# AUTOMATIC1111/stable-diffusion-webui

Measured on AMD Instinct MI355X. Metric: images/sec SD1.5 512x512 20-step Euler-a, batch 8 per GPU, higher is better.
Workload: dtype f16

## Files before the change

include/sdmi.h:

```cpp
#ifndef SDMI_H
#define SDMI_H

#include <stdint.h>

#ifdef __cplusplus
extern "C" {
#endif

#define SDMI_VERSION 100

enum { SDMI_F16 = 0, SDMI_F32 = 1 };

typedef struct sdmi_engine sdmi_engine;

int sdmi_version(void);
const char* sdmi_last_error(void);
int sdmi_device_ok(void);


int64_t sdmi_attention_workspace_bytes(int B, int H, int M, int D);
int sdmi_attention(const void* q, const void* k, const void* v, void* out,
                   int B, int H, int N, int M, int D,
                   int ldq, int ldk, int ldv, int ldo, float scale,
                   void* workspace, int64_t workspace_bytes, void* stream);

int64_t sdmi_attention_wide_workspace_bytes(int B, int N, int M, int D);
int sdmi_attention_wide(const void* q, const void* k, const void* v, void* out,
                        int B, int N, int M, int D,
                        int ldq, int ldk, int ldv, int ldo, float scale,
                        void* workspace, int64_t workspace_bytes, void* stream);

int sdmi_attention_vt(const void* q, const void* k, const void* vt, void* out,
                      int B, int H, int N, int M, int D,
                      int ldq, int ldk, int vt_ld, int ldo, float scale, int force_generic, void* stream);

typedef struct sdmi_conv_desc {
    const void* a0;
    const void* a1;
    const void* w;
    const void* bias;
    const void* rowbias;
    const void* resid;
    void* out;
    int32_t c0, c1, lda0, lda1;
    int32_t B, Hi, Wi, Ho, Wo;
    int32_t taps;
    int32_t stride;
    int32_t pad;
    int32_t up;
    int32_t N;
    int32_t n_real;
    int32_t ldo, ldr;
    int32_t flags;
    float alpha;
    int32_t batch;
    int64_t a_bs, w_bs, o_bs, r_bs;
    int32_t force_generic;
    int32_t reserved;
    void* splitk_workspace;
    int64_t splitk_workspace_bytes;
} sdmi_conv_desc;

enum {
    SDMI_EP_OUT_F32  = 1,
    SDMI_EP_GEGLU    = 2,
    SDMI_EP_NCHW     = 4,
    SDMI_EP_BIAS_ROW = 8,
    SDMI_EP_WRAP = 128,
    SDMI_EP_TRANSPOSE = 64
};
int sdmi_conv_gemm(const sdmi_conv_desc* d, void* stream);
int64_t sdmi_conv_splitk_workspace_bytes(int M, int N, int K, int batch);

int sdmi_pack_conv_weight(const void* w_oihw, int dtype, void* out_f16, int O, int I, int kh, int kw,
                          int O_pad, int I_pad, int geglu, void* stream);

int sdmi_groupnorm(const void* x0, const void* x1, int c0, int c1, const void* gamma_f32, const void* beta_f32,
                   void* out_f16, int B, int HW, int groups, float eps, int silu,
                   void* workspace_f32, int64_t workspace_bytes, void* stream);
int64_t sdmi_groupnorm_workspace_bytes(int B, int HW, int groups);

int sdmi_layernorm(const void* x, const void* gamma_f32, const void* beta_f32, void* out_f16,
                   int64_t rows, int C, float eps, void* stream);

int64_t sdmi_rowchain_ff_pack_bytes(int C, int hidden);
int sdmi_rowchain_ff_pack(const void* w1_f16, const void* b1_f32_or_null, const void* w2_f16, void* packs, int C, int hidden,
                          void* stream);
int sdmi_rowchain_ff(const void* x_f16, void* out_f16, const void* ln_gamma_f32, const void* ln_beta_f32, const void* packs,
                     const void* b2_f32_or_null, int64_t rows, int C, int hidden, float eps, void* stream);


int sdmi_philox_randn(void* out_f32, int64_t n, uint64_t seed, uint32_t offset, void* stream);

int sdmi_slerp(void* out_f32, const void* low_f32, const void* high_f32, float val, int C, int H, int W, void* scratch_f32,
               void* stream);


int sdmi_cfg_prepare_input(const void* x_f32, const void* c_in_f32, void* x_in, int out_dtype,
                           int B, int reps, int64_t chw, void* stream);

int sdmi_cfg_prepare_concat(const void* x_f32, const void* c_in_f32, const void* c_concat_f32, void* x_in, int out_dtype,
                            int B, int reps, int C, int Cc, int64_t hw, uint32_t zero_reps, void* stream);

int sdmi_cfg_combine(const void* x_f32, const void* eps_f32, const void* c_out_f32, float cond_scale, int mode,
                     const void* mask_f32, const void* nmask_f32, const void* init_latent_f32,
                     void* denoised_f32, int B, int64_t chw, void* stream);

int sdmi_cfg_combine_affine(const void* x_f32, const void* out_f32, const void* c_out_f32, const void* c_skip_f32,
                            float cond_scale, const void* mask_f32, const void* nmask_f32, const void* init_latent_f32,
                            void* denoised_f32, int B, int64_t chw, void* stream);

int sdmi_euler_step(void* x_f32, const void* denoised_f32, const void* noise_f32_or_null,
                    float sigma, float sigma_down, float sigma_up, float s_noise, int64_t n, void* stream);

int sdmi_dpmpp2m_step(void* x_f32, const void* denoised_f32, const void* old_denoised_f32_or_null,
                      float ratio, float em1, float c1, float c2, int64_t n, void* stream);

int sdmi_ddim_step(void* x_f32, const void* e_t_f32, const void* noise_f32_or_null, void* pred_x0_f32_or_null,
                   float a_t, float a_prev, float sigma_t, float sqrt_one_minus_at, int64_t n, void* stream);

int sdmi_axpby(void* y_f32, const void* x_f32, float a, const void* z_f32_or_null, float b, int64_t n, void* stream);

int sdmi_lincomb(void* out_f32, const void* const* terms_f32, const float* coefs, int n_terms, int64_t n, void* stream);

int sdmi_dpm_error_partials(const void* x_low_f32, const void* x_high_f32, const void* x_prev_f32, float atol, float rtol,
                            void* partial256_f32, int64_t n, void* stream);

int sdmi_latent_resize(const void* in_f32, void* out_f32, int planes, int hi, int wi, int ho, int wo, int mode, void* stream);

int sdmi_mask_blend(void* x_f32, const void* init_f32, const void* mask_f32, const void* nmask_f32, int64_t n, void* stream);

int sdmi_image_to_u8(const void* img_f32_nchw, void* out_u8_nhwc, int B, int C, int H, int W, void* stream);

typedef struct sdmi_unet_config {
    int32_t in_channels, out_channels, model_channels;
    int32_t num_levels;
    int32_t channel_mult[8];
    int32_t num_res_blocks;
    int32_t attn_level[8];
    int32_t transformer_depth[8];
    int32_t num_heads;
    int32_t num_head_channels;
    int32_t context_dim;
    int32_t adm_in_channels;
    int32_t reserved[4];
} sdmi_unet_config;

typedef struct sdmi_vae_config {
    int32_t ch, num_levels;
    int32_t ch_mult[8];
    int32_t num_res_blocks, in_channels, out_ch, z_channels;
    float scale_factor;
    int32_t reserved[4];
} sdmi_vae_config;

sdmi_engine* sdmi_engine_create(int device);
void sdmi_engine_destroy(sdmi_engine* e);

int sdmi_unet_configure(sdmi_engine* e, const sdmi_unet_config* cfg);
int sdmi_unet_load_tensor(sdmi_engine* e, const char* key, const void* data, int dtype, int ndim,
                          const int64_t* shape, int on_device);
int sdmi_unet_finalize(sdmi_engine* e);

int sdmi_unet_update_weight(sdmi_engine* e, const char* key, const void* data, int dtype, int ndim,
// ... 77 lines not shown
```

stable-diffusion-webui_amd/_lib.py:

```python
from __future__ import annotations

import ctypes as C
import os
import re

_HERE = os.path.dirname(os.path.abspath(__file__))
LIB_PATH = os.environ.get("SDMI_LIB") or os.path.join(_HERE, "lib", "libsdmi.so")
HEADER_PATH = os.path.join(os.path.dirname(_HERE), "include", "sdmi.h")

F16, F32 = 0, 1
EP_OUT_F32, EP_GEGLU, EP_NCHW, EP_BIAS_ROW = 1, 2, 4, 8
EP_TRANSPOSE = 64
EP_WRAP = 128


class SdmiError(RuntimeError):
    pass


class ConvDesc(C.Structure):
    _fields_ = [
        ("a0", C.c_void_p), ("a1", C.c_void_p), ("w", C.c_void_p), ("bias", C.c_void_p), ("rowbias", C.c_void_p),
        ("resid", C.c_void_p), ("out", C.c_void_p),
        ("c0", C.c_int32), ("c1", C.c_int32), ("lda0", C.c_int32), ("lda1", C.c_int32),
        ("B", C.c_int32), ("Hi", C.c_int32), ("Wi", C.c_int32), ("Ho", C.c_int32), ("Wo", C.c_int32),
        ("taps", C.c_int32), ("stride", C.c_int32), ("pad", C.c_int32), ("up", C.c_int32),
        ("N", C.c_int32), ("n_real", C.c_int32), ("ldo", C.c_int32), ("ldr", C.c_int32),
        ("flags", C.c_int32), ("alpha", C.c_float), ("batch", C.c_int32),
        ("a_bs", C.c_int64), ("w_bs", C.c_int64), ("o_bs", C.c_int64), ("r_bs", C.c_int64),
        ("force_generic", C.c_int32), ("reserved", C.c_int32),
        ("splitk_workspace", C.c_void_p), ("splitk_workspace_bytes", C.c_int64),
    ]


class UNetConfigC(C.Structure):
    _fields_ = [
        ("in_channels", C.c_int32), ("out_channels", C.c_int32), ("model_channels", C.c_int32),
        ("num_levels", C.c_int32), ("channel_mult", C.c_int32 * 8), ("num_res_blocks", C.c_int32),
        ("attn_level", C.c_int32 * 8), ("transformer_depth", C.c_int32 * 8),
        ("num_heads", C.c_int32), ("num_head_channels", C.c_int32), ("context_dim", C.c_int32),
        ("adm_in_channels", C.c_int32), ("reserved", C.c_int32 * 4),
    ]


class VAEConfigC(C.Structure):
    _fields_ = [
        ("ch", C.c_int32), ("num_levels", C.c_int32), ("ch_mult", C.c_int32 * 8),
        ("num_res_blocks", C.c_int32), ("in_channels", C.c_int32), ("out_ch", C.c_int32), ("z_channels", C.c_int32),
        ("scale_factor", C.c_float), ("reserved", C.c_int32 * 4),
    ]


class ClipConfigC(C.Structure):
    _fields_ = [("vocab_size", C.c_int32), ("max_positions", C.c_int32), ("hidden", C.c_int32), ("layers", C.c_int32),
                ("heads", C.c_int32), ("intermediate", C.c_int32), ("act", C.c_int32), ("eps", C.c_float)]


def declared_symbols() -> list:
    src = open(HEADER_PATH).read()
    src = re.sub(r"/\*.*?\*/", "", src, flags=re.S)
    return sorted(set(re.findall(r"\b(sdmi_[a-z0-9_]+)\s*\(", src)))


if not os.path.exists(LIB_PATH):
    raise ImportError(
        f"{LIB_PATH} is missing: build it with `python -c 'import __graft_entry__ as g; g.build()'` "
        "(hipcc --offload-arch=gfx950). There is no CPU fallback for the MI355X engine.")

lib = C.CDLL(LIB_PATH)

_vp, _i, _i64, _f, _u32 = C.c_void_p, C.c_int, C.c_int64, C.c_float, C.c_uint32
_SIGS = {
    "sdmi_version": (C.c_int, []),
    "sdmi_last_error": (C.c_char_p, []),
    "sdmi_device_ok": (C.c_int, []),
    "sdmi_attention_workspace_bytes": (_i64, [_i, _i, _i, _i]),
    "sdmi_attention": (_i, [_vp, _vp, _vp, _vp, _i, _i, _i, _i, _i, _i, _i, _i, _i, _f, _vp, _i64, _vp]),
    "sdmi_attention_wide_workspace_bytes": (_i64, [_i, _i, _i, _i]),
    "sdmi_attention_wide": (_i, [_vp, _vp, _vp, _vp, _i, _i, _i, _i, _i, _i, _i, _i, _f, _vp, _i64, _vp]),
    "sdmi_attention_vt": (_i, [_vp, _vp, _vp, _vp, _i, _i, _i, _i, _i, _i, _i, _i, _i, _f, _i, _vp]),
    "sdmi_conv_gemm": (_i, [C.POINTER(ConvDesc), _vp]),
    "sdmi_conv_splitk_workspace_bytes": (_i64, [_i, _i, _i, _i]),
    "sdmi_bench_conv_gemm": (_i, [C.POINTER(ConvDesc), _i, C.POINTER(C.c_float), _vp]),
    "sdmi_pack_conv_weight": (_i, [_vp, _i, _vp, _i, _i, _i, _i, _i, _i, _i, _vp]),
    "sdmi_groupnorm": (_i, [_vp, _vp, _i, _i, _vp, _vp, _vp, _i, _i, _i, _f, _i, _vp, _i64, _vp]),
    "sdmi_groupnorm_workspace_bytes": (_i64, [_i, _i, _i]),
    "sdmi_layernorm": (_i, [_vp, _vp, _vp, _vp, _i64, _i, _f, _vp]),
    "sdmi_rowchain_ff_pack_bytes": (_i64, [_i, _i]),
    "sdmi_rowchain_ff_pack": (_i, [_vp, _vp, _vp, _vp, _i, _i, _vp]),
    "sdmi_rowchain_ff": (_i, [_vp, _vp, _vp, _vp, _vp, _vp, _i64, _i, _i, _f, _vp]),
    "sdmi_philox_randn": (_i, [_vp, _i64, C.c_uint64, C.c_uint32, _vp]),
    "sdmi_slerp": (_i, [_vp, _vp, _vp, _f, _i, _i, _i, _vp, _vp]),
    "sdmi_cfg_prepare_input": (_i, [_vp, _vp, _vp, _i, _i, _i, _i64, _vp]),
    "sdmi_cfg_prepare_concat": (_i, [_vp, _vp, _vp, _vp, _i, _i, _i, _i, _i, _i64, _u32, _vp]),
    "sdmi_cfg_combine": (_i, [_vp, _vp, _vp, _f, _i, _vp, _vp, _vp, _vp, _i, _i64, _vp]),
    "sdmi_cfg_combine_affine": (_i, [_vp, _vp, _vp, _vp, _f, _vp, _vp, _vp, _vp, _i, _i64, _vp]),
    "sdmi_euler_step": (_i, [_vp, _vp, _vp, _f, _f, _f, _f, _i64, _vp]),
    "sdmi_dpmpp2m_step": (_i, [_vp, _vp, _vp, _f, _f, _f, _f, _i64, _vp]),
    "sdmi_ddim_step": (_i, [_vp, _vp, _vp, _vp, _f, _f, _f, _f, _i64, _vp]),
    "sdmi_axpby": (_i, [_vp, _vp, _f, _vp, _f, _i64, _vp]),
    "sdmi_dpm_error_partials": (_i, [_vp, _vp, _vp, _f, _f, _vp, _i64, _vp]),
    "sdmi_lincomb": (_i, [_vp, C.POINTER(_vp), C.POINTER(_f), _i, _i64, _vp]),
    "sdmi_mask_blend": (_i, [_vp, _vp, _vp, _vp, _i64, _vp]),
    "sdmi_latent_resize": (_i, [_vp, _vp, _i, _i, _i, _i, _i, _i, _vp]),
    "sdmi_image_to_u8": (_i, [_vp, _vp, _i, _i, _i, _i, _vp]),
    "sdmi_engine_create": (_vp, [_i]),
    "sdmi_engine_destroy": (None, [_vp]),
    "sdmi_unet_configure": (_i, [_vp, C.POINTER(UNetConfigC)]),
    "sdmi_unet_load_tensor": (_i, [_vp, C.c_char_p, _vp, _i, _i, C.POINTER(C.c_int64), _i]),
    "sdmi_unet_finalize": (_i, [_vp]),
    "sdmi_clip_configure": (_i, [_vp, _i, C.POINTER(ClipConfigC)]),
    "sdmi_clip_load_tensor": (_i, [_vp, _i, C.c_char_p, _vp, _i, _i, C.POINTER(C.c_int64), _i]),
    "sdmi_clip_finalize": (_i, [_vp, _i]),
    "sdmi_clip_forward": (_i, [_vp, _i, _vp, _vp, _i, _i, _i, _i, _vp, _vp, _vp]),
    "sdmi_unet_update_weight": (_i, [_vp, C.c_char_p, _vp, _i, _i, C.POINTER(C.c_int64), _i]),
    "sdmi_unet_hypernet_clear": (_i, [_vp]),
    "sdmi_unet_hypernet_begin": (_i, [_vp, _f]),
    "sdmi_unet_hypernet_linear": (_i, [_vp, _i, _i, _vp, _vp, _i, _i, _i, _i]),
    "sdmi_unet_hypernet_act": (_i, [_vp, _i, _i, _i]),
    "sdmi_unet_hypernet_layernorm": (_i, [_vp, _i, _i, _vp, _vp, _i, _i, _i]),
    "sdmi_unet_update_vector": (_i, [_vp, C.c_char_p, _vp, _i, _i64, _i]),
    "sdmi_lora_merge": (_i, [_vp, _vp, _i, _vp, _i, _vp, _i, _i, _i, _i, _f, _vp]),
    "sdmi_weight_hadamard": (_i, [_vp, _vp, _vp, _vp, _f, _i64, _vp]),
    "sdmi_weight_kron": (_i, [_vp, _vp, _vp, _vp, _i, _i, _i, _i, _i, _f, _vp]),
    "sdmi_weight_ia3": (_i, [_vp, _vp, _vp, _i, _i, _i, _f, _vp]),
    "sdmi_weight_dora": (_i, [_vp, _vp, _vp, _vp, _i, _i, _i, _f, _vp]),
    "sdmi_vae_configure": (_i, [_vp, C.POINTER(VAEConfigC)]),
    "sdmi_vae_load_tensor": (_i, [_vp, C.c_char_p, _vp, _i, _i, C.POINTER(C.c_int64), _i]),
    "sdmi_vae_finalize": (_i, [_vp]),
    "sdmi_unet_set_context": (_i, [_vp, _vp, _i, _i, _i, _vp]),
    "sdmi_unet_set_context_cached": (_i, [_vp, _vp, _i, _i, _i, _vp]),
    "sdmi_unet_forward": (_i, [_vp, _vp, _vp, _vp, _vp, _vp, _i, _i, _i, _i, _i, _vp]),
    "sdmi_unet_set_control": (_i, [_vp, _vp, _vp, _i, _i]),
    "sdmi_unet_forward_ex": (_i, [_vp, _vp, _vp, _vp, _vp, _vp, _i, _i, _i, _i, _i, _i, _vp]),
    "sdmi_vae_decode": (_i, [_vp, _vp, _i, _vp, _i, _i, _i, _vp]),
    "sdmi_vae_encode": (_i, [_vp, _vp, _i, _vp, _i, _i, _i, _vp]),
    "sdmi_debug_set": (_i, [C.c_char_p, _i]),
    "sdmi_debug_set_str": (_i, [C.c_char_p, C.c_char_p]),
    "sdmi_profile_begin": (_i, []),
    "sdmi_profile_end": (_i, [C.c_char_p, _i]),
    "sdmi_engine_arena_bytes": (_i64, [_vp]),
    "sdmi_engine_set_option": (_i, [_vp, C.c_char_p, _i]),
    "sdmi_engine_tap_count": (_i, [_vp]),
    "sdmi_engine_tap_info": (_i, [_vp, _i, C.c_char_p, _i, C.POINTER(C.c_int64)]),
    "sdmi_engine_tap_read": (_i, [_vp, _i, _vp, _vp]),
}
for _name, (_res, _args) in _SIGS.items():
    _fn = getattr(lib, _name)
    _fn.restype = _res
    _fn.argtypes = _args


def last_error() -> str:
    return (lib.sdmi_last_error() or b"").decode("utf-8", "replace")


def check(rc: int, what: str = "sdmi call"):
    if rc != 0:
        raise SdmiError(f"{what} failed: {last_error()}")


def device_ok() -> bool:
    return bool(lib.sdmi_device_ok())


def require_device():
    if not device_ok():
        raise SdmiError("no gfx950 (MI355X) device visible to HIP: the engine has no CPU path")


# ... 17 lines not shown
```

stable-diffusion-webui_amd/csrc/capi.cpp:

```cpp
#include "engine.h"
#include "prof.h"
#include <cstring>

namespace sdmi {
extern int g_vae_attn_rows;
int unet_forward(sdmi_engine* e, const void* x, const void* t, const void* ctx, const void* y, void* out, int io_dtype,
                 int Bn, int h, int w, int L, hipStream_t s);
int vae_decode(sdmi_engine* e, const void* z, int io_dtype, float* out, int B, int h, int w, hipStream_t s);
int vae_encode(sdmi_engine* e, const void* x, int io_dtype, float* out, int B, int H, int W, hipStream_t s);
int engine_load_unet_tensor(sdmi_engine* e, const char* key, const void* data, int dtype, int ndim, const int64_t* shape, int on_device);
int engine_load_vae_tensor(sdmi_engine* e, const char* key, const void* data, int dtype, int ndim, const int64_t* shape, int on_device);
int engine_unet_finalize(sdmi_engine* e);
int engine_clip_configure(sdmi_engine* e, int slot, const sdmi_clip_config* cfg);
int engine_clip_load_tensor(sdmi_engine* e, int slot, const char* key, const void* data, int dtype, int ndim, const int64_t* shape, int on_device);
int engine_clip_finalize(sdmi_engine* e, int slot);
int engine_clip_forward(sdmi_engine* e, int slot, const int* tokens, const float* inputs_embeds, int B, int L, int skip,
                        int apply_final_ln, float* out, float* pooled, hipStream_t s);
int engine_unet_update_weight(sdmi_engine* e, const char* key, const void* data, int dtype, int ndim, const int64_t* shape, int on_device);
int engine_vae_finalize(sdmi_engine* e);
int engine_hypernet_clear(sdmi_engine* e);
int engine_hypernet_begin(sdmi_engine* e, float multiplier);
int engine_hypernet_linear(sdmi_engine* e, int dim, int which, const void* w, const void* b, int dtype, int out_f, int in_f, int on_device);
int engine_hypernet_act(sdmi_engine* e, int dim, int which, int act);
int engine_hypernet_layernorm(sdmi_engine* e, int dim, int which, const void* g, const void* b, int dtype, int n, int on_device);
// ... 48 lines not shown
                   int ldk, int ldv, int ldo, float scale, void* workspace, int64_t workspace_bytes, void* stream) {
    API_GUARD_BEGIN
    SDMI_REQUIRE(workspace && workspace_bytes >= sdmi_attention_workspace_bytes(B, H, M, D), "attention workspace too small");
    const int mpad = (M + 63) / 64 * 64;
    if (launch_transpose_v((const half_t*)v, (half_t*)workspace, B, H, M, D, ldv, mpad, (hipStream_t)stream)) return 1;
    return sdmi_attention_vt(q, k, workspace, out, B, H, N, M, D, ldq, ldk, mpad, ldo, scale, 0, stream);
    API_GUARD_END
}

static constexpr int kWideRows = 4096;
int64_t sdmi_attention_wide_workspace_bytes(int B, int N, int M, int D) {
    if (B <= 0 || N <= 0 || M <= 0 || D <= 0) return 0;
    const int64_t mpad = (M + 63) / 64 * 64;
    const int64_t rows = N < kWideRows ? N : kWideRows;
    return (int64_t)B * D * mpad * (int64_t)sizeof(half_t) + rows * mpad * (int64_t)(sizeof(float) + sizeof(half_t));
}

int sdmi_attention_wide(const void* q, const void* k, const void* v, void* out, int B, int N, int M, int D, int ldq, int ldk,
                        int ldv, int ldo, float scale, void* workspace, int64_t workspace_bytes, void* stream) {
    API_GUARD_BEGIN
    SDMI_REQUIRE(q && k && v && out && B > 0 && N > 0 && M > 0, "sdmi_attention_wide: null pointer or empty problem");
    SDMI_REQUIRE(D > 0 && D % 64 == 0 && D <= 1024, "sdmi_attention_wide: D must be a multiple of 64, at most 1024");
    SDMI_REQUIRE(ldq % 8 == 0 && ldk % 8 == 0 && ldo % 8 == 0, "sdmi_attention_wide: row strides must be multiples of 8 elements");
    SDMI_REQUIRE(ldq >= D && ldk >= D && ldv >= D && ldo >= D, "sdmi_attention_wide: row strides must be at least D");
    SDMI_REQUIRE(workspace && workspace_bytes >= sdmi_attention_wide_workspace_bytes(B, N, M, D), "attention workspace too small");
    hipStream_t s = (hipStream_t)stream;
    const int mpad = (M + 63) / 64 * 64;
    const int rows_max = N < kWideRows ? N : kWideRows;
    half_t* vt = (half_t*)workspace;
    float* S = (float*)(vt + (size_t)B * D * mpad);
    half_t* P = (half_t*)(S + (size_t)rows_max * mpad);
    if (launch_transpose_v((const half_t*)v, vt, B, 1, M, D, ldv, mpad, s)) return 1;
    for (int b = 0; b < B; ++b)
        for (int r0 = 0; r0 < N; r0 += kWideRows) {
            const int rows = N - r0 < kWideRows ? N - r0 : kWideRows;
            GemmP p{};
            p.a0 = (const half_t*)q + ((size_t)b * N + r0) * ldq; p.c0 = D; p.cin = D; p.lda0 = ldq;
            p.w = (const half_t*)k + (size_t)b * M * ldk; p.ldw = ldk;
            p.out = S;
            p.Hi = rows; p.Wi = 1; p.Ho = rows; p.Wo = 1; p.taps = 1; p.stride = 1;
            p.M = rows; p.N = mpad; p.n_valid = M; p.K = D; p.ldo = mpad; p.rows_per_batch = rows; p.n_real = mpad;
            p.flags = EP_OUT_F32;
            p.alpha = scale;
            if (launch_gemm(p, 1, false, true, s)) return 1;
            if (launch_softmax_rows(S, P, rows, M, mpad, mpad, s)) return 1;
            GemmP g{};
            g.a0 = P; g.c0 = mpad; g.cin = mpad; g.lda0 = mpad;
            g.w = vt + (size_t)b * D * mpad; g.ldw = mpad;
            g.out = (half_t*)out + ((size_t)b * N + r0) * ldo;
            g.Hi = rows; g.Wi = 1; g.Ho = rows; g.Wo = 1; g.taps = 1; g.stride = 1;
            g.M = rows; g.N = D; g.K = mpad; g.ldo = ldo; g.rows_per_batch = rows; g.n_real = D;
            g.alpha = 1.f;
            if (launch_gemm(g, 1, false, true, s)) return 1;
        }
    return 0;
    API_GUARD_END
}

static int desc_to_p(const sdmi_conv_desc* d, GemmP* p) {
    SDMI_REQUIRE(d != nullptr, "null descriptor");
    *p = GemmP{};
    p->a0 = (const half_t*)d->a0; p->a1 = (const half_t*)d->a1; p->w = (const half_t*)d->w;
    p->bias = (const float*)d->bias; p->rowbias = (const float*)d->rowbias; p->resid = (const half_t*)d->resid;
    p->out = d->out;
    p->c0 = d->c0; p->c1 = d->a1 ? d->c1 : 0; p->cin = p->c0 + p->c1;
    p->lda0 = d->lda0 ? d->lda0 : d->c0; p->lda1 = d->lda1 ? d->lda1 : d->c1;
    p->Hi = d->Hi; p->Wi = d->Wi; p->Ho = d->Ho; p->Wo = d->Wo;
    p->taps = d->taps; p->stride = d->stride ? d->stride : 1; p->pad = d->pad; p->up = d->up;
    SDMI_REQUIRE(p->taps == 1 || p->taps == 9, "taps must be 1 or 9");
    p->M = d->B * d->Ho * d->Wo; p->N = d->N; p->K = p->taps * p->cin;
    p->ldo = d->ldo; p->ldr = d->ldr; p->ldw = p->K; p->ldrb = d->N;
    p->rows_per_batch = d->Ho * d->Wo;
    p->n_real = d->n_real ? d->n_real : d->N;
    p->flags = d->flags;
    p->alpha = d->alpha == 0.f ? 1.f : d->alpha;
    p->a_bs = d->a_bs; p->w_bs = d->w_bs; p->o_bs = d->o_bs; p->r_bs = d->r_bs;
    const size_t need = gemm_splitk_ws_bytes(p->M, p->N, p->K, d->batch > 0 ? d->batch : 1);
    if (d->splitk_workspace && need && (size_t)d->splitk_workspace_bytes >= need) p->splitk_ws = (float*)d->splitk_workspace;
    return 0;
}

int64_t sdmi_conv_splitk_workspace_bytes(int M, int N, int K, int batch) { return (int64_t)gemm_splitk_ws_bytes(M, N, K, batch); }

int sdmi_conv_gemm(const sdmi_conv_desc* d, void* stream) {
    API_GUARD_BEGIN
    GemmP p;
    if (desc_to_p(d, &p)) return 1;
    const char* env = getenv("SDMI_NO_GLDS");
    return launch_gemm(p, d->batch > 0 ? d->batch : 1, d->force_generic == 1, !(env && env[0] == '1') && d->force_generic != 2,
                       (hipStream_t)stream);
    API_GUARD_END
}

int sdmi_bench_conv_gemm(const sdmi_conv_desc* d, int iters, float* ms_out, void* stream) {
    API_GUARD_BEGIN
    GemmP p;
    if (desc_to_p(d, &p)) return 1;
    hipStream_t s = (hipStream_t)stream;
    hipEvent_t e0, e1;
    SDMI_CHECK_HIP(hipEventCreate(&e0));
    SDMI_CHECK_HIP(hipEventCreate(&e1));
    const bool glds = d->force_generic != 2;
    for (int i = 0; i < 2; ++i)
        if (launch_gemm(p, d->batch > 0 ? d->batch : 1, d->force_generic == 1, glds, s)) return 1;
    SDMI_CHECK_HIP(hipEventRecord(e0, s));
    for (int i = 0; i < iters; ++i)
        if (launch_gemm(p, d->batch > 0 ? d->batch : 1, d->force_generic == 1, glds, s)) return 1;
    SDMI_CHECK_HIP(hipEventRecord(e1, s));
    SDMI_CHECK_HIP(hipEventSynchronize(e1));
    float ms = 0.f;
    SDMI_CHECK_HIP(hipEventElapsedTime(&ms, e0, e1));
    *ms_out = ms / (float)iters;
    (void)hipEventDestroy(e0);
    (void)hipEventDestroy(e1);
    return 0;
    API_GUARD_END
}

int sdmi_pack_conv_weight(const void* w, int dtype, void* out, int O, int I, int kh, int kw, int O_pad, int I_pad, int geglu,
                          void* stream) {
    API_GUARD_BEGIN
    return launch_pack_conv_weight(w, dtype, (half_t*)out, O, I, kh, kw, O_pad, I_pad, geglu, (hipStream_t)stream);
    API_GUARD_END
}

int64_t sdmi_groupnorm_workspace_bytes(int B, int HW, int groups) { return groupnorm_ws_bytes(B, HW, groups); }

int sdmi_groupnorm(const void* x0, const void* x1, int c0, int c1, const void* gamma, const void* beta, void* out, int B, int HW,
                   int groups, float eps, int silu, void* ws, int64_t ws_bytes, void* stream) {
    API_GUARD_BEGIN
    SDMI_REQUIRE(ws && ws_bytes >= groupnorm_ws_bytes(B, HW, groups), "groupnorm workspace too small");
    return launch_groupnorm((const half_t*)x0, (const half_t*)x1, c0, x1 ? c1 : 0, (const float*)gamma, (const float*)beta,
                            (half_t*)out, B, HW, groups, eps, silu != 0, (float*)ws, (hipStream_t)stream);
    API_GUARD_END
}

int sdmi_layernorm(const void* x, const void* gamma, const void* beta, void* out, int64_t rows, int C, float eps, void* stream) {
    API_GUARD_BEGIN
    return launch_layernorm((const half_t*)x, (const float*)gamma, (const float*)beta, (half_t*)out, rows, C, eps, (hipStream_t)stream);
    API_GUARD_END
}

int64_t sdmi_rowchain_ff_pack_bytes(int C, int hidden) { return (int64_t)rowchain_ff_pack_bytes(C, hidden); }
int sdmi_rowchain_ff_pack(const void* w1, const void* b1, const void* w2, void* packs, int C, int hidden, void* stream) {
    API_GUARD_BEGIN
    SDMI_REQUIRE(w1 && w2 && packs, "null argument");
    return launch_rowchain_ff_pack((const half_t*)w1, (const float*)b1, (const half_t*)w2, packs, C, hidden, false, (hipStream_t)stream);
    API_GUARD_END
}
int sdmi_rowchain_ff(const void* x, void* out, const void* g, const void* b, const void* packs, const void* b2, int64_t rows, int C,
                     int hidden, float eps, void* stream) {
    API_GUARD_BEGIN
    SDMI_REQUIRE(x && out && g && b && packs, "null argument");
    return launch_rowchain_ff((const half_t*)x, (half_t*)out, (const float*)g, (const float*)b, packs, (const float*)b2, (long)rows, C,
                              hidden, eps, (hipStream_t)stream);
    API_GUARD_END
}


int sdmi_philox_randn(void* out, int64_t n, uint64_t seed, uint32_t offset, void* stream) {
    API_GUARD_BEGIN
    return launch_philox((float*)out, n, seed, offset, (hipStream_t)stream);
    API_GUARD_END
}

int sdmi_slerp(void* out, const void* low, const void* high, float val, int C, int H, int W, void* scratch, void* stream) {
    API_GUARD_BEGIN
    SDMI_REQUIRE(out && low && high && scratch && C > 0 && H > 0 && W > 0, "bad arguments");
    return launch_slerp((float*)out, (const float*)low, (const float*)high, val, C, H, W, (float*)scratch, (hipStream_t)stream);
    API_GUARD_END
}

int sdmi_cfg_prepare_input(const void* x, const void* c_in, void* x_in, int out_dtype, int B, int reps, int64_t chw, void* stream) {
    API_GUARD_BEGIN
    return launch_cfg_prepare((const float*)x, (const float*)c_in, x_in, out_dtype, B, reps, chw, (hipStream_t)stream);
    API_GUARD_END
}

int sdmi_cfg_prepare_concat(const void* x, const void* c_in, const void* c_concat, void* x_in, int out_dtype, int B, int reps,
                            int C, int Cc, int64_t hw, uint32_t zero_reps, void* stream) {
    API_GUARD_BEGIN
    SDMI_REQUIRE(x && c_concat && x_in, "null pointer");
    SDMI_REQUIRE(B > 0 && reps > 0 && reps <= 32 && C > 0 && Cc > 0 && hw > 0, "bad sizes");
    return launch_cfg_prepare_concat((const float*)x, (const float*)c_in, (const float*)c_concat, x_in, out_dtype, B, reps, C, Cc, hw,
                                     zero_reps, (hipStream_t)stream);
    API_GUARD_END
}

int sdmi_cfg_combine(const void* x, const void* eps, const void* c_out, float cond_scale, int mode, const void* mask,
                     const void* nmask, const void* init_latent, void* den, int B, int64_t chw, void* stream) {
    API_GUARD_BEGIN
    SDMI_REQUIRE(mode == 1 || (x && c_out), "sigma-space combine needs x and c_out");
    return launch_cfg_combine((const float*)x, (const float*)eps, (const float*)c_out, cond_scale, mode, (const float*)mask,
                              (const float*)nmask, (const float*)init_latent, (float*)den, B, chw, (hipStream_t)stream);
    API_GUARD_END
}

int sdmi_euler_step(void* x, const void* den, const void* noise, float sigma, float sigma_down, float sigma_up, float s_noise,
                    int64_t n, void* stream) {
    API_GUARD_BEGIN
    return launch_euler_step((float*)x, (const float*)den, (const float*)noise, sigma, sigma_down, sigma_up, s_noise, n,
                             (hipStream_t)stream);
    API_GUARD_END
}

int sdmi_dpmpp2m_step(void* x, const void* den, const void* old, float ratio, float em1, float c1, float c2, int64_t n,
                      void* stream) {
    API_GUARD_BEGIN
    return launch_dpmpp2m_step((float*)x, (const float*)den, (const float*)old, ratio, em1, c1, c2, n, (hipStream_t)stream);
    API_GUARD_END
}

int sdmi_ddim_step(void* x, const void* e_t, const void* noise, void* pred_x0, float a_t, float a_prev, float sigma_t,
                   float sqrt_one_minus_at, int64_t n, void* stream) {
    API_GUARD_BEGIN
    return launch_ddim_step((float*)x, (const float*)e_t, (const float*)noise, (float*)pred_x0, a_t, a_prev, sigma_t,
                            sqrt_one_minus_at, n, (hipStream_t)stream);
    API_GUARD_END
}

int sdmi_dpm_error_partials(const void* x_low, const void* x_high, const void* x_prev, float atol, float rtol, void* partial256_f32,
                            int64_t n, void* stream) {
// ... 206 lines not shown
    e->vae.cfg = *cfg;
    e->vae.ready = false;
    return 0;
    API_GUARD_END
}
int sdmi_vae_load_tensor(sdmi_engine* e, const char* key, const void* data, int dtype, int ndim, const int64_t* shape,
                         int on_device) {
    API_GUARD_BEGIN
    return engine_load_vae_tensor(e, key, data, dtype, ndim, shape, on_device);
    API_GUARD_END
}
int sdmi_vae_finalize(sdmi_engine* e) {
    API_GUARD_BEGIN
    return engine_vae_finalize(e);
    API_GUARD_END
}

int sdmi_unet_set_context(sdmi_engine* e, const void* context, int io_dtype, int Bn, int L, void* stream) {
    API_GUARD_BEGIN
    return engine_set_context(e, context, io_dtype, Bn, L, (hipStream_t)stream);
    API_GUARD_END
}
int sdmi_unet_set_context_cached(sdmi_engine* e, const void* context, int io_dtype, int Bn, int L, void* stream) {
    API_GUARD_BEGIN
    return engine_set_context(e, context, io_dtype, Bn, L, (hipStream_t)stream, true);
    API_GUARD_END
}
int sdmi_unet_forward(sdmi_engine* e, const void* x, const void* timesteps, const void* context, const void* y, void* out,
                      int io_dtype, int Bn, int h, int w, int L, void* stream) {
    API_GUARD_BEGIN
    return unet_forward(e, x, timesteps, context, y, out, io_dtype, Bn, h, w, L, (hipStream_t)stream);
    API_GUARD_END
}
int sdmi_unet_set_control(sdmi_engine* e, const void* const* tensors, const int64_t* numel, int n, int only_mid_control) {
    API_GUARD_BEGIN
    SDMI_REQUIRE(e != nullptr && n >= 0 && (n == 0 || (tensors && numel)), "null argument");
    e->control.assign(tensors, tensors + n);
    e->control_numel.assign(numel, numel + n);
    e->only_mid_control = only_mid_control != 0;
    for (int i = 0; i < n; ++i) SDMI_REQUIRE(tensors[i] != nullptr, "null control tensor");
    return 0;
    API_GUARD_END
}
int sdmi_unet_forward_ex(sdmi_engine* e, const void* x, const void* timesteps, const void* context, const void* y, void* out,
                         int io_dtype, int Bn, int h, int w, int L, int call_flags, void* stream) {
    API_GUARD_BEGIN
    SDMI_REQUIRE(e != nullptr, "null engine");
    struct Restore {
        sdmi_engine* e; bool uni, pairs, derive;
        ~Restore() { e->uniform_t = uni; e->cfg_pairs = pairs; e->auto_promises = derive; }
    } restore{e, e->uniform_t, e->cfg_pairs, e->auto_promises};
    e->uniform_t = (call_flags & SDMI_CALL_UNIFORM_T) != 0;
    e->cfg_pairs = (call_flags & SDMI_CALL_CFG_PAIRS) != 0;
    e->auto_promises = (call_flags & SDMI_CALL_DERIVE) != 0;
    return unet_forward(e, x, timesteps, context, y, out, io_dtype, Bn, h, w, L, (hipStream_t)stream);
    API_GUARD_END
}
int sdmi_vae_decode(sdmi_engine* e, const void* z, int io_dtype, void* out, int B, int h, int w, void* stream) {
    API_GUARD_BEGIN
    return vae_decode(e, z, io_dtype, (float*)out, B, h, w, (hipStream_t)stream);
    API_GUARD_END
}
int sdmi_vae_encode(sdmi_engine* e, const void* x, int io_dtype, void* out, int B, int H, int W, void* stream) {
    API_GUARD_BEGIN
    return vae_encode(e, x, io_dtype, (float*)out, B, H, W, (hipStream_t)stream);
    API_GUARD_END
}

int sdmi_debug_set(const char* name, int value) {
    API_GUARD_BEGIN
    SDMI_REQUIRE(name != nullptr, "null name");
    const std::string n(name);
    if (n == "gemm_cfg") g_force_gemm_cfg = value;
    else if (n == "gemm_shortk_cfg") g_shortk_gemm_cfg = value;
    else if (n == "vae_attn_rows") g_vae_attn_rows = value;
    else if (n == "gemm_shortk_maxk") g_shortk_max_k = value;
    else if (n == "gemm_geglu_cfg") g_geglu_gemm_cfg = value;
    else if (n == "vt_mode") g_vt_mode = value;
    else if (n == "tile_order") g_tile_order = value;
    else if (n == "conv_korder") g_conv_korder = value < 0 ? g_conv_korder_default : value;
    else if (n == "small_linear_lds") g_small_linear_lds = value;
    else if (n == "gn_fuse") g_gn_fuse = value;
    else if (n == "gn_small") g_gn_small = value;
    else if (n == "ep_wide") g_ep_wide = value;
    else if (n == "attn_kvt") g_attn_kvt = value;
    else if (n == "attn_occ") g_attn_occ = value;
    else if (n == "attn_lds_pad") g_attn_lds_pad = value;
    else if (n == "attn_fold_min_m") g_attn_fold_min_m = value;
    else if (n == "attn_tau") g_attn_tau = value;
    else if (n == "attn_dbg_lo") g_attn_dbg = (g_attn_dbg & 0xFFFFFFFF00000000ull) | (unsigned)value;
    else if (n == "attn_dbg_hi") g_attn_dbg = (g_attn_dbg & 0xFFFFFFFFull) | ((unsigned long long)(unsigned)value << 32);
    else if (n == "gemm_split") g_force_gemm_split = value;
    else if (n == "gemm_pipe") g_gemm_pipe = value < 0 ? g_gemm_pipe_default : value;
    else if (n == "gemm_lin") g_gemm_lin = value < 0 ? 1 : value;
    else if (n == "gn_apply_blocks") g_gn_apply_blocks = value < 0 ? 0 : value;
    else if (n == "gn_band_elems") g_gn_band_elems = value < 0 ? 0 : value;
    else if (n == "gemm_dbgflags") g_gemm_dbgflags = value & 0x1F00;
    else if (n == "gemm_dbg_lo") g_gemm_dbg = (g_gemm_dbg & 0xFFFFFFFF00000000ull) | (unsigned)value;
    else if (n == "gemm_dbg_hi") g_gemm_dbg = (g_gemm_dbg & 0xFFFFFFFFull) | ((unsigned long long)(unsigned)value << 32);
    else { set_error("unknown debug knob " + n); return 1; }
    return 0;
    API_GUARD_END
}

int sdmi_debug_set_str(const char* name, const char* value) {
    API_GUARD_BEGIN
    SDMI_REQUIRE(name != nullptr, "null name");
    if (std::string(name) == "gemm_override") {
        SDMI_REQUIRE(gemm_set_override(value) == 0, "gemm_override: expected M,N,K,taps,kind:cfg:split;...");
        return 0;
    }
    set_error(std::string("unknown debug knob ") + name);
    return 1;
    API_GUARD_END
}

int sdmi_profile_begin(void) {
    prof_begin();
    return 0;
}
int sdmi_profile_end(char* json_out, int capacity) {
    const std::string s = prof_end();
    if (!json_out || capacity <= (int)s.size()) {
        set_error("profile buffer too small");
        return 1;
    }
    std::memcpy(json_out, s.c_str(), s.size() + 1);
    return 0;
}

int64_t sdmi_engine_arena_bytes(sdmi_engine* e) { return e ? (int64_t)e->arena.cap : 0; }

int sdmi_engine_set_option(sdmi_engine* e, const char* name, int value) {
    API_GUARD_BEGIN
    SDMI_REQUIRE(e && name, "null argument");
    const std::string n(name);
    if (n == "force_generic") e->force_generic = value != 0;
    else if (n == "glds") e->use_glds = value != 0;
    else if (n == "trace") { e->trace = value != 0; e->taps.clear(); }
    else if (n == "tiling") e->tiling = value != 0;
    else if (n == "uniform_t") e->uniform_t = value != 0;
    else if (n == "cfg_pairs") e->cfg_pairs = value != 0;
    else if (n == "auto_promises") e->auto_promises = value != 0;
    else if (n == "ln_fold") e->ln_fold = value;
    else if (n == "fuse_rows") e->fuse_rows = value;
    else if (n == "residual_fp32") e->residual_fp32 = value != 0;
    else if (n == "arena_reuse") e->arena_reuse = value;
    else if (n == "streams") { if (value < 1 || value > 8) { sdmi::set_error("streams must be 1..8"); return 1; } e->n_streams = value; }
    else if (n == "vae_range_extend") e->vae_stream_scale = value ? 1.0f / 64.0f : 1.0f;
    else { set_error("unknown option " + n); return 1; }
    return 0;
    API_GUARD_END
}

int sdmi_engine_tap_count(sdmi_engine* e) { return e ? (int)e->taps.size() : 0; }
int sdmi_engine_tap_info(sdmi_engine* e, int index, char* name_out, int capacity, int64_t* dims_bhwc) {
    API_GUARD_BEGIN
    SDMI_REQUIRE(e && name_out && dims_bhwc && index >= 0 && index < (int)e->taps.size(), "bad tap index / null argument");
    const auto& t = e->taps[index];
    SDMI_REQUIRE((int)t.name.size() < capacity, "tap name buffer too small");
    std::memcpy(name_out, t.name.c_str(), t.name.size() + 1);
    dims_bhwc[0] = t.B; dims_bhwc[1] = t.H; dims_bhwc[2] = t.W; dims_bhwc[3] = t.C;
    return 0;
    API_GUARD_END
}
int sdmi_engine_tap_read(sdmi_engine* e, int index, void* out_f16_nhwc, void* stream) {
// ... 11 lines not shown
```

stable-diffusion-webui_amd/csrc/common.h:

```cpp
#pragma once
#include <hip/hip_runtime.h>
#include <stdint.h>
#include <string>

typedef _Float16 half_t;
typedef _Float16 h8 __attribute__((ext_vector_type(8)));
typedef _Float16 h4 __attribute__((ext_vector_type(4)));
typedef _Float16 h2 __attribute__((ext_vector_type(2)));
typedef float f4 __attribute__((ext_vector_type(4)));
typedef float f16v __attribute__((ext_vector_type(16)));

namespace sdmi {

#ifndef SDMI_GELU_SIG
#define SDMI_GELU_SIG 1
#endif
__device__ __forceinline__ float geglu_gate(float val, float g) {
    const float gc = fminf(fmaxf(g, -10.0f), 10.0f);
    const float g2 = gc * gc;
    float p = fmaf(1.01426306e-3f, g2, -0.106775724f);
    p = fmaf(p, g2, -2.30112135f);
    const float e = __builtin_amdgcn_exp2f(p * gc);
    return (val * g) * __builtin_amdgcn_rcpf(1.0f + e);
}
// ... 13 lines not shown
#define SDMI_REQUIRE(cond, msg)                                                                    \
    do {                                                                                           \
        if (!(cond)) {                                                                             \
            ::sdmi::set_error(std::string("requirement failed: ") + #cond + " — " + (msg));        \
            return 1;                                                                              \
        }                                                                                          \
    } while (0)

static inline int cdiv(int64_t a, int64_t b) { return (int)((a + b - 1) / b); }

struct PerDeviceOnce {
    int level[64] = {};
    bool need(int want = 1) {
        int d = 0;
        if (hipGetDevice(&d) != hipSuccess) d = 0;
        d &= 63;
        if (level[d] >= want) return false;
        level[d] = want;
        return true;
    }
};

constexpr int kZeroPageHalfs = 16384;
const half_t* zero_page();

struct GemmP {
    const half_t* a0;
    const half_t* a1;
    const half_t* w;
    const float* bias;
    const float* rowbias;
    const half_t* resid;
    void* out;
    const half_t* zero;
    int c0, c1, cin;
    int lda0, lda1;
    int Hi, Wi, Ho, Wo;
    int taps, stride, pad, up;
    int M, N, K;
    int ldo, ldr;
    int ldw;
    int ldrb;
    int rows_per_batch;
    int n_real;
    int n_valid;
    int flags;
    float alpha;
    long a_bs, w_bs, o_bs, r_bs;
    float* splitk_ws;
    int splitk;
    int splitk_steps;
    long long* dbg;
    float* stats_out;
    int stats_cpg;
    int stats_nchunk;
    int korder;
    int tile_order;
    float bias_scale;
    const int* gate;
    const float* ln_stats;
    const float* ln_s;
    int ln_np;
    float ln_inv_c, ln_eps;
    float* lnp_out;
    int lnp_np;
};

enum { EP_OUT_F32 = 1, EP_GEGLU = 2, EP_NCHW = 4, EP_BIAS_ROW = 8,
       EP_QUICK_GELU = 16, EP_GELU = 32,
       EP_TRANSPOSE = 64,
       EP_WRAP = 128,
       EP_DBG_NO_BAR_A = 0x100, EP_DBG_NO_BAR_B = 0x200, EP_DBG_NO_GLDS = 0x400, EP_DBG_NO_VMWAIT = 0x800,
       EP_DBG_NO_DSREAD = 0x1000,
       EP_LNFOLD = 0x4000,
       EP_HILO = 0x8000,
       EP_NARROW = 0x2000
     };

__host__ __device__ inline half_t* gemm_out_lo(const GemmP& p) {
    return (p.flags & EP_HILO) ? reinterpret_cast<half_t*>(const_cast<float*>(p.ln_stats)) : nullptr;
}
__host__ __device__ inline const half_t* gemm_resid_lo(const GemmP& p) { return (p.flags & EP_HILO) ? reinterpret_cast<const half_t*>(p.ln_s) : nullptr; }

int launch_gemm(const GemmP& p, int batch, bool force_generic, bool use_glds, hipStream_t s, int* stats_nchunk_out = nullptr,
                int* lnp_np_out = nullptr);
extern int g_ep_wide;
extern int g_small_linear_lds;
extern int g_gn_small;
extern int g_gn_fuse;
size_t gemm_splitk_ws_bytes(int M, int N, int K, int batch);
int gemm_set_override(const char* spec);
extern int g_force_gemm_cfg;
extern int g_shortk_gemm_cfg;
extern int g_shortk_max_k;
extern int g_geglu_gemm_cfg;
extern int g_conv_korder;
extern int g_conv_korder_default;
extern int g_tile_order;
extern int g_vt_mode;
extern long g_gn_band_elems;
extern int g_gn_apply_blocks;
extern int g_gemm_lin;
extern int g_gemm_pipe;
extern int g_gemm_pipe_default;
extern int g_force_gemm_split;
extern int g_attn_kvt;
extern int g_attn_occ;
extern int g_attn_lds_pad;
extern int g_attn_fold_min_m;
extern int g_attn_tau;
extern unsigned long long g_attn_dbg;
extern int g_gemm_dbgflags;
extern unsigned long long g_gemm_dbg;

struct AttnP {
    const half_t* q;
    const half_t* k;
    const half_t* vt;
    half_t* out;
    int B, H, N, M, D;
    int ldq, ldk, vt_ld, ldo;
    float scale_log2;
    int causal;
    long long* dbg;
    float tau;
};
int launch_attention(const AttnP& p, bool force_generic, hipStream_t s);
int launch_transpose_v(const half_t* v, half_t* vt, int B, int H, int M, int D, int ldv, int Mpad, hipStream_t s);

bool rowchain_supports(int C);
size_t rowchain_ff_pack_bytes(int C, int hidden);
int launch_rowchain_ff_pack(const half_t* w1, const float* b1, const half_t* w2, void* packs, int C, int hidden, bool permuted,
                            hipStream_t s);
int launch_rowchain_ff(const half_t* x, half_t* out, const float* gamma, const float* beta, const void* packs, const float* bias_out,
                       long rows, int C, int hidden, float eps, hipStream_t s);

int launch_groupnorm(const half_t* x0, const half_t* x1, int c0, int c1, const float* gamma, const float* beta,
                     half_t* out, int B, int HW, int groups, float eps, bool silu, float* ws, hipStream_t s, int pre_nchunk = 0,
                     const half_t* x0_lo = nullptr, const half_t* x1_lo = nullptr);
int64_t groupnorm_ws_bytes(int B, int HW, int groups);
int launch_layernorm(const half_t* x, const float* gamma, const float* beta, half_t* out, int64_t rows, int C,
                     float eps, hipStream_t s, const half_t* x_lo = nullptr);
int launch_ln_rowstats(const half_t* x, float* stats, int64_t rows, int C, float eps, hipStream_t s);
int launch_ln_fold_weights(const half_t* w, const float* gamma, const float* beta, const float* bias, half_t* wf, float* s_out,
                           float* c_out, int n_rows, int K, int C, hipStream_t s);

int launch_philox(float* out, int64_t n, uint64_t seed, uint32_t offset, hipStream_t s);
int launch_cfg_prepare(const float* x, const float* c_in, void* xin, int out_dtype, int B, int reps, int64_t chw, hipStream_t s);
int launch_slerp(float* out, const float* low, const float* high, float val, int C, int H, int W, float* scratch, hipStream_t s);
int launch_weight_hadamard(float* out, const float* w, const float* a, const float* b, float scale, int64_t n, hipStream_t s);
int launch_weight_kron(float* out, const float* w, const float* w1, const float* w2, int r1, int c1, int r2, int c2, int k, float scale,
                       hipStream_t s);
int launch_weight_ia3(float* out, const float* w, const float* v, int rows, int cols, int on_input, float scale, hipStream_t s);
int launch_weight_dora(float* out, const float* w, const float* delta, const float* dora_scale, int rows, int cin, int k, float mult,
                       hipStream_t s);
int launch_cfg_prepare_concat(const float* x, const float* c_in, const float* cond, void* xin, int out_dtype, int B, int reps,
                              int C, int Cc, int64_t hw, unsigned zero_reps, hipStream_t s);
int launch_cfg_combine(const float* x, const float* eps, const float* c_out, float cond_scale, int mode,
                       const float* mask, const float* nmask, const float* init_latent, float* den, int B,
                       int64_t chw, hipStream_t s);
int launch_euler_step(float* x, const float* den, const float* noise, float sigma, float sigma_down, float sigma_up,
                      float s_noise, int64_t n, hipStream_t s);
int launch_dpmpp2m_step(float* x, const float* den, const float* old, float ratio, float em1, float c1, float c2,
                        int64_t n, hipStream_t s);
int launch_ddim_step(float* x, const float* e, const float* noise, float* pred_x0, float a_t, float a_prev,
                     float sigma_t, float somat, int64_t n, hipStream_t s);
int launch_axpby(float* y, const float* x, float a, const float* z, float b, int64_t n, hipStream_t s);
int launch_dpm_error(const float* lo, const float* hi, const float* prev, float atol, float rtol, float* partial256, int64_t n,
                     hipStream_t s);
int launch_lincomb(float* out, const float* const* terms, const float* coefs, int n_terms, int64_t n, hipStream_t s);
int launch_lora_merge(float* out, const void* w, int w_dtype, const void* up, int up_dtype, const void* down, int down_dtype,
                      int rows, int cols, int rank, float scale, hipStream_t s);
int launch_clip_embed(const int* tokens, const void* tok_emb, int tok_dtype, const float* pos_emb, const float* inputs_embeds,
                      half_t* out, int B, int L, int C, int vocab, hipStream_t s);
int launch_clip_pool(const int* tokens, const half_t* hidden, float* pooled, int B, int L, int C, hipStream_t s);
int launch_latent_resize(const float* in, float* out, int planes, int hi, int wi, int ho, int wo, int mode, hipStream_t s);
int launch_cfg_combine_affine(const float* x, const float* out, const float* c_out, const float* c_skip, float cond_scale,
                              const float* mask, const float* nmask, const float* init_latent, float* den, int B, int64_t chw,
                              hipStream_t s);
int launch_act_f16(half_t* x, int64_t n, int kind, hipStream_t s);
int launch_axpy_f16(half_t* y, const half_t* x, const half_t* h, float a, int64_t n, hipStream_t s);
int launch_silu_f32(const float* x, float* y, int64_t n, hipStream_t s);
int launch_mask_blend(float* x, const float* init, const float* mask, const float* nmask, int64_t n, hipStream_t s);
int launch_image_to_u8(const float* img, uint8_t* out, int B, int C, int H, int W, hipStream_t s);

int launch_nchw_to_nhwc(const void* x, int dtype, half_t* out, int B, int C, int HW, int cpad, float scale,
                        const float* mix_w, const float* mix_b, hipStream_t s, bool lo_ch = false);
int launch_add_nchw_residual(const half_t* src, const half_t* src_lo, const void* ctrl, int dtype, half_t* dst, half_t* dst_lo, int B, int C,
                             int HW, hipStream_t s);
int launch_copy_out(const float* src, void* dst, int dtype, int64_t n, hipStream_t s);
int launch_convert_to_f16(const void* src, int dtype, half_t* dst, int64_t n, hipStream_t s);
int launch_convert_to_f32(const void* src, int dtype, float* dst, int64_t n, hipStream_t s);
int launch_ctx_compare(const void* src, int dtype, const half_t* cached, int B, int L, int Lpad, int C, int* gate, hipStream_t s);
int launch_ctx_update_gated(const void* src, int dtype, half_t* cached, int B, int L, int Lpad, int C, const int* gate, hipStream_t s);
int launch_timestep_embedding(const void* t, int dtype, float* out, int B, int dim, hipStream_t s);
int launch_small_linear(const float* a, const half_t* w, const float* bias, const float* add, float* out, int B,
                        int N, int K, int lda, int ldo, bool silu_in, bool silu_out, hipStream_t s);
int launch_softmax_rows(const float* in, half_t* out, int64_t rows, int cols, int ldi, int ldo, hipStream_t s);
int launch_pack_conv_weight(const void* w, int dtype, half_t* out, int O, int I, int kh, int kw, int O_pad,
                            int I_pad, int geglu, hipStream_t s);
int launch_pack_bias(const void* b, int dtype, float* out, int O, int O_pad, int geglu, hipStream_t s);

}
```

stable-diffusion-webui_amd/csrc/engine.cpp:

```cpp
#include "engine.h"

#include <algorithm>
#include <cmath>
#include <cstring>

namespace sdmi {

static thread_local std::string g_err;
void set_error(const std::string& m) { g_err = m; }
const char* get_error() { return g_err.c_str(); }

const half_t* zero_page() {
    static thread_local int cached_dev = -1;
    static thread_local half_t* cached = nullptr;
    static std::map<int, half_t*> pages;
    int dev = 0;
    if (hipGetDevice(&dev) != hipSuccess) return nullptr;
    if (dev == cached_dev) return cached;
    auto it = pages.find(dev);
    if (it == pages.end()) {
        void* p = nullptr;
        if (hipMalloc(&p, kZeroPageHalfs * sizeof(half_t)) != hipSuccess) return nullptr;
        if (hipMemset(p, 0, kZeroPageHalfs * sizeof(half_t)) != hipSuccess) return nullptr;
        it = pages.emplace(dev, (half_t*)p).first;
    }
    cached_dev = dev;
    cached = it->second;
    return cached;
}

static inline int rup(int x, int m) { return (x + m - 1) / m * m; }

struct Run {
    sdmi_engine* e;
    hipStream_t s;
    bool dry;
    Arena* ar;
    int b0 = 0, Btot = 0;
    Run(sdmi_engine* e_, hipStream_t s_, bool dry_, Arena* ar_ = nullptr, int b0_ = 0, int Btot_ = 0)
        : e(e_), s(s_), dry(dry_), ar(ar_ ? ar_ : &e_->arena), b0(b0_), Btot(Btot_) {}
    half_t* H(size_t n) { return (half_t*)ar->take(n * sizeof(half_t)); }
    bool acc() const { return e->residual_fp32 && !e->force_generic && e->use_glds; }
    half_t* S(size_t n) { return H(acc() ? 2 * n : n); }
    half_t* lo(const half_t* p, size_t n) const { return (acc() && p) ? const_cast<half_t*>(p) + n : nullptr; }
    bool reuse() const { return e->arena_reuse && !e->trace && !e->ln_fold && !acc(); }
    float* F(size_t n) { return (float*)ar->take(n * sizeof(float)); }
    void tap(const std::string& name, const half_t* p, int B, int H, int W, int C) {
        if (!dry && e->trace) e->taps.push_back({name, p, B, H, W, C});
    }
    const half_t* st_tensor = nullptr;
    float* st_ws = nullptr;
    int st_nchunk = 0;
    bool lnp_want = false;
    const half_t* lnp_tensor = nullptr;
    float* lnp_ws = nullptr;
    int lnp_np = 0;
};

#define TRY(x)                  \
    do {                        \
        if ((x) != 0) return 1; \
    } while (0)

static int dev_alloc(sdmi_engine* e, void** p, size_t bytes) {
    SDMI_CHECK_HIP(hipMalloc(p, std::max<size_t>(bytes, 256)));
    (e->alloc_sink ? *e->alloc_sink : e->owned).push_back(*p);
    return 0;
}

static const RawTensor* find_raw(const std::map<std::string, RawTensor>& m, const std::string& k) {
    auto it = m.find(k);
    return it == m.end() ? nullptr : &it->second;
}

static int pack_stack(sdmi_engine* e, const std::map<std::string, RawTensor>& m, const std::vector<std::string>& names,
                      bool pad64, bool geglu, ConvW* out, bool dup_in = false) {
    int cin = -1, taps = -1, total = 0;
    bool any_bias = false;
    for (auto& n : names) {
        const RawTensor* w = find_raw(m, n + ".weight");
        SDMI_REQUIRE(w != nullptr, "missing weight " + n + ".weight");
        SDMI_REQUIRE(w->shape.size() == 2 || w->shape.size() == 4, "weight must be 2-D or 4-D: " + n);
        const int I = (int)w->shape[1];
        const int t = w->shape.size() == 4 ? (int)(w->shape[2] * w->shape[3]) : 1;
        SDMI_REQUIRE(cin < 0 || (cin == I && taps == t), "stacked weights disagree in shape: " + n);
        cin = I; taps = t;
        total += (int)w->shape[0];
        if (find_raw(m, n + ".bias")) any_bias = true;
    }
    SDMI_REQUIRE(taps == 1 || taps == 9, "only 1x1 and 3x3 kernels");
    out->cin = cin;
    out->cin_pad = pad64 ? rup(cin, 64) : cin;
    out->cout = total;
    out->n_pad = pad64 ? rup(total, 64) : total;
    out->taps = taps;
    out->geglu = geglu;
    SDMI_REQUIRE(names.size() == 1 || (total == out->n_pad), "stacked outputs must be multiples of 64");
    const size_t wn = (size_t)out->n_pad * taps * out->cin_pad;
    TRY(dev_alloc(e, (void**)&out->w, wn * sizeof(half_t)));
    SDMI_CHECK_HIP(hipMemset(out->w, 0, wn * sizeof(half_t)));
    if (any_bias) {
        TRY(dev_alloc(e, (void**)&out->b, (size_t)out->n_pad * sizeof(float)));
        SDMI_CHECK_HIP(hipMemset(out->b, 0, (size_t)out->n_pad * sizeof(float)));
    }
    int row = 0;
    for (size_t i = 0; i < names.size(); ++i) {
        const RawTensor* w = find_raw(m, names[i] + ".weight");
        const int O = (int)w->shape[0];
        const int Opad = (names.size() == 1) ? out->n_pad : O;
        const int kh = taps == 9 ? 3 : 1;
        const int pflags = (geglu ? 1 : 0) | ((dup_in && 2 * cin <= out->cin_pad) ? 2 : 0);
        TRY(launch_pack_conv_weight(w->ptr, w->dtype, out->w + (size_t)row * taps * out->cin_pad, O, cin, kh, kh, Opad,
                                    out->cin_pad, pflags, 0));
        if (e->recording_unet_sites)
            e->unet_sites[names[i] + ".weight"].push_back({out->w + (size_t)row * taps * out->cin_pad, O, cin, kh, Opad,
                                                           out->cin_pad, pflags});
        const RawTensor* b = find_raw(m, names[i] + ".bias");
        if (b) TRY(launch_pack_bias(b->ptr, b->dtype, out->b + row, O, Opad, geglu ? 1 : 0, 0));
        if (b && e->recording_unet_sites) e->unet_vec_sites[names[i] + ".bias"].push_back({out->b + row, O, Opad, geglu ? 1 : 0});
        row += Opad;
    }
    return 0;
}
static int pack_one(sdmi_engine* e, const std::map<std::string, RawTensor>& m, const std::string& name, bool pad64,
                    bool geglu, ConvW* out, bool dup_in = false) {
    return pack_stack(e, m, {name}, pad64, geglu, out, dup_in);
}
static int pack_norm(sdmi_engine* e, const std::map<std::string, RawTensor>& m, const std::string& name, NormW* out) {
    const RawTensor* g = find_raw(m, name + ".weight");
    const RawTensor* b = find_raw(m, name + ".bias");
    SDMI_REQUIRE(g && b, "missing norm " + name);
    const int c = (int)g->shape[0];
    out->c = c;
    TRY(dev_alloc(e, (void**)&out->g, c * sizeof(float)));
    TRY(dev_alloc(e, (void**)&out->b, c * sizeof(float)));
    TRY(launch_convert_to_f32(g->ptr, g->dtype, out->g, c, 0));
    TRY(launch_convert_to_f32(b->ptr, b->dtype, out->b, c, 0));
    if (e->recording_unet_sites) {
        e->unet_vec_sites[name + ".weight"].push_back({out->g, c, c, 0});
// ... 144 lines not shown
            L.kind = UNetLayer::DOWN;
            TRY(pack_one(e, m, "input_blocks." + std::to_string(idx) + ".0.op", true, false, &L.conv));
            blk.push_back(L);
            u.input.push_back(blk);
            chans.push_back(ch);
            ++idx;
        }
    }
    TRY(add_res("middle_block.0", ch, ch, ch, 0, &u.middle));
    TRY(add_st("middle_block.1", ch, nlev - 1, &u.middle));
    TRY(add_res("middle_block.2", ch, ch, ch, 0, &u.middle));
    idx = 0;
    for (int level = nlev - 1; level >= 0; --level) {
        for (int i = 0; i <= c.num_res_blocks; ++i) {
            std::vector<UNetLayer> blk;
            const int ich = chans.back();
            chans.pop_back();
            const int cout = mc * c.channel_mult[level];
            const std::string base = "output_blocks." + std::to_string(idx);
            TRY(add_res(base + ".0", ch + ich, cout, ch, ich, &blk));
            ch = cout;
            int li = 1;
            if (c.attn_level[level]) { TRY(add_st(base + "." + std::to_string(li), ch, level, &blk)); ++li; }
            if (level && i == c.num_res_blocks) {
                UNetLayer L;
                L.kind = UNetLayer::UP;
                TRY(pack_one(e, m, base + "." + std::to_string(li) + ".conv", true, false, &L.conv));
                blk.push_back(L);
            }
            u.output.push_back(blk);
            ++idx;
        }
    }
    TRY(pack_norm(e, m, "out.0", &u.out_norm));
    TRY(pack_one(e, m, "out.2", true, false, &u.out_conv));
    TRY(pack_stack(e, m, emb_names, false, false, &u.emb_all));
    u.emb_cols = emb_cols;
    SDMI_CHECK_HIP(hipDeviceSynchronize());
    u.ready = true;
    return 0;
}

struct ConvArgs {
    const half_t* a0 = nullptr;
    const half_t* a1 = nullptr;
    int c0 = 0, c1 = 0;
    int B = 1, Hi = 1, Wi = 1, Ho = 1, Wo = 1;
    int stride = 1, pad = 0, up = 0;
    const float* rowbias = nullptr;
    int ldrb = 0;
    const half_t* resid = nullptr;
    const half_t* resid_lo = nullptr;
    half_t* out_lo = nullptr;
    int ldr = 0;
    void* out = nullptr;
    int ldo = 0;
    int flags = 0;
    int n_real = 0;
    float alpha = 1.f;
    float bias_scale = 1.f;
    int batch = 1;
    long a_bs = 0, w_bs = 0, o_bs = 0, r_bs = 0;
    const int* gate = nullptr;
    int stats_C = 0;
    bool no_split = false;
    float* stats_ws_pre = nullptr;
};

static int run_conv(Run& r, const ConvW& W, const ConvArgs& a) {
    float* splitk_ws = nullptr;
    if (!(a.flags & EP_NCHW) && !W.geglu && !a.no_split) {
        const size_t wsb = gemm_splitk_ws_bytes(a.B * a.Ho * a.Wo, W.n_pad, W.taps * (a.c0 + a.c1), a.batch);
        if (wsb) splitk_ws = r.F(wsb / sizeof(float));
    }
    float* stats_ws = nullptr;
    if (a.stats_C > 0 && W.n_pad == a.stats_C && a.stats_C % 32 == 0) stats_ws = a.stats_ws_pre ? a.stats_ws_pre : r.F((size_t)a.B * 64 * 32 * 2);
    r.st_tensor = nullptr; r.st_nchunk = 0;
    float* lnp_ws = nullptr;
    const bool want_lnp = r.lnp_want && W.taps == 1 && !W.geglu && !(a.flags & (EP_NCHW | EP_OUT_F32 | EP_TRANSPOSE));
    r.lnp_want = false;
    if (want_lnp) lnp_ws = r.F((size_t)a.B * a.Ho * a.Wo * (W.n_pad / 64) * 2);
    r.lnp_tensor = nullptr; r.lnp_np = 0;
    if (r.dry) return 0;
    GemmP p{};
    p.splitk_ws = splitk_ws;
    p.lnp_out = lnp_ws;
    p.a0 = a.a0; p.a1 = a.a1; p.w = W.w; p.bias = W.b; p.rowbias = a.rowbias; p.resid = a.resid; p.out = a.out;
    p.c0 = a.c0; p.c1 = a.c1; p.cin = a.c0 + a.c1; p.lda0 = a.c0; p.lda1 = a.c1;
    SDMI_REQUIRE(p.cin == W.cin_pad, "conv input channels do not match the packed weight");
    p.Hi = a.Hi; p.Wi = a.Wi; p.Ho = a.Ho; p.Wo = a.Wo;
    p.taps = W.taps; p.stride = a.stride; p.pad = a.pad; p.up = a.up;
    p.M = a.B * a.Ho * a.Wo; p.N = W.n_pad; p.K = W.taps * p.cin;
    p.ldo = a.ldo; p.ldr = a.ldr; p.ldw = p.K; p.ldrb = a.ldrb;
    p.rows_per_batch = a.Ho * a.Wo;
    p.n_real = a.n_real ? a.n_real : W.n_pad;
    p.flags = a.flags | (W.geglu ? EP_GEGLU : 0);
    if (a.out_lo || a.resid_lo) {
        p.flags |= EP_HILO;
        p.ln_stats = reinterpret_cast<const float*>(a.out_lo);
        p.ln_s = reinterpret_cast<const float*>(a.resid_lo);
    }
    if (r.e->tiling && W.taps == 9 && a.pad == 1) p.flags |= EP_WRAP;
    p.alpha = a.alpha;
    p.bias_scale = a.bias_scale;
    p.a_bs = a.a_bs; p.w_bs = a.w_bs; p.o_bs = a.o_bs; p.r_bs = a.r_bs;
    p.gate = a.gate;
    int nchunk = 0;
    if (stats_ws) { p.stats_out = stats_ws; p.stats_cpg = a.stats_C / 32; }
    int lnp_np = 0;
    TRY(launch_gemm(p, a.batch, r.e->force_generic, r.e->use_glds, r.s, &nchunk, &lnp_np));
    if (nchunk > 0) { r.st_tensor = (const half_t*)a.out; r.st_ws = stats_ws; r.st_nchunk = nchunk; }
    if (lnp_np > 0) { r.lnp_tensor = (const half_t*)a.out; r.lnp_ws = lnp_ws; r.lnp_np = lnp_np; }
    return 0;
}

static int run_linear(Run& r, const ConvW& W, const half_t* a, int rows, const half_t* resid, half_t* out, int ldo, float ss = 1.f,
                      bool no_split = false, const half_t* resid_lo = nullptr, half_t* out_lo = nullptr) {
    ConvArgs c;
    c.resid_lo = resid_lo; c.out_lo = out_lo;
    c.alpha = ss; c.bias_scale = ss;
    c.no_split = no_split;
    c.a0 = a; c.c0 = W.cin_pad;
    c.B = 1; c.Hi = rows; c.Wi = 1; c.Ho = rows; c.Wo = 1;
    c.resid = resid; c.ldr = ldo; c.out = out; c.ldo = ldo;
    return run_conv(r, W, c);
}

static int run_gn(Run& r, const NormW& n, const half_t* x0, const half_t* x1, int c0, int c1, int B, int HW, float eps,
                  bool silu, half_t* out, const half_t* x0_lo = nullptr, const half_t* x1_lo = nullptr) {
    float* ws = r.F(groupnorm_ws_bytes(B, HW, 32) / sizeof(float));
    if (r.dry) return 0;
    SDMI_REQUIRE(n.c == c0 + c1, "GroupNorm channel mismatch");
    if (x1 == nullptr && r.st_nchunk > 0 && r.st_tensor == x0)
        return launch_groupnorm(x0, nullptr, c0, 0, n.g, n.b, out, B, HW, 32, eps, silu, r.st_ws, r.s, r.st_nchunk, x0_lo, nullptr);
    return launch_groupnorm(x0, x1, c0, c1, n.g, n.b, out, B, HW, 32, eps, silu, ws, r.s, 0, x0_lo, x1_lo);
}
static int run_ln(Run& r, const NormW& n, const half_t* x, int64_t rows, half_t* out, const half_t* x_lo = nullptr) {
    if (r.dry) return 0;
    return launch_layernorm(x, n.g, n.b, out, rows, n.c, 1e-5f, r.s, x_lo);
}

struct LnStats { const float* ptr = nullptr; int np = 0; };
static int run_ln_stats(Run& r, const NormW& n, const half_t* x, int64_t rows, LnStats* out) {
    float* own = r.F((size_t)rows * 2);
    if (r.dry) { out->ptr = own; out->np = 0; return 0; }
    if (r.lnp_tensor == x && r.lnp_np > 0) { out->ptr = r.lnp_ws; out->np = r.lnp_np; return 0; }
    out->ptr = own; out->np = 0;
    return launch_ln_rowstats(x, own, rows, n.c, 1e-5f, r.s);
}
static int ensure_ln_fold(sdmi_engine* e, const ConvW& W, const NormW& n, hipStream_t s) {
    if (W.w_ln && W.fold_epoch == e->weights_epoch) return 0;
    SDMI_REQUIRE(W.taps == 1 && n.c <= W.cin_pad, "LayerNorm fold: linear layers only");
    if (!W.w_ln) {
        void* p = nullptr;
        SDMI_CHECK_HIP(hipMalloc(&p, (size_t)W.n_pad * W.cin_pad * sizeof(half_t))); e->owned.push_back(p); W.w_ln = (half_t*)p;
        SDMI_CHECK_HIP(hipMalloc(&p, (size_t)W.n_pad * sizeof(float))); e->owned.push_back(p); W.s_ln = (float*)p;
        SDMI_CHECK_HIP(hipMalloc(&p, (size_t)W.n_pad * sizeof(float))); e->owned.push_back(p); W.c_ln = (float*)p;
    }
    TRY(launch_ln_fold_weights(W.w, n.g, n.b, W.b, W.w_ln, W.s_ln, W.c_ln, W.n_pad, W.cin_pad, n.c, s));
    W.fold_epoch = e->weights_epoch;
    return 0;
}
static int run_linear_ln(Run& r, const ConvW& W, const NormW& n, const half_t* x, const LnStats& stats, int rows, half_t* out, int ldo) {
    if (!r.dry) TRY(ensure_ln_fold(r.e, W, n, r.s));
    float* splitk_ws = nullptr;
    if (!W.geglu) {
        const size_t wsb = gemm_splitk_ws_bytes(rows, W.n_pad, W.cin_pad, 1);
        if (wsb) splitk_ws = r.F(wsb / sizeof(float));
    }
    r.st_tensor = nullptr; r.st_nchunk = 0;
    if (r.dry) return 0;
    GemmP p{};
    p.splitk_ws = splitk_ws;
    p.a0 = x; p.w = W.w_ln; p.bias = W.c_ln; p.out = out;
    p.c0 = W.cin_pad; p.cin = W.cin_pad; p.lda0 = W.cin_pad;
    p.Hi = rows; p.Wi = 1; p.Ho = rows; p.Wo = 1;
    p.taps = 1; p.stride = 1; p.pad = 0; p.up = 0;
    p.M = rows; p.N = W.n_pad; p.K = W.cin_pad;
    p.ldo = ldo; p.ldw = p.K;
    p.rows_per_batch = rows; p.n_real = W.n_pad;
    p.flags = EP_LNFOLD | (W.geglu ? EP_GEGLU : 0);
    p.alpha = 1.f; p.bias_scale = 1.f;
    p.ln_stats = stats.ptr; p.ln_np = stats.np; p.ln_inv_c = 1.0f / (float)n.c; p.ln_eps = 1e-5f; p.ln_s = W.s_ln;
    return launch_gemm(p, 1, false, true, r.s);
}
static int run_vt_ln(Run& r, const ConvW& Wv, const NormW& n, const half_t* x, const LnStats& stats, int B, int tokens, int tokens_pad,
                     half_t* vt) {
    if (r.dry) return 0;
    TRY(ensure_ln_fold(r.e, Wv, n, r.s));
    GemmP p{};
    const int C = Wv.n_pad, K = Wv.cin_pad;
    p.a0 = x; p.c0 = K; p.cin = K; p.lda0 = K;
    p.w = Wv.w_ln; p.ldw = K;
    p.bias = Wv.c_ln;
    p.out = vt;
    p.Hi = tokens; p.Wi = 1; p.Ho = tokens; p.Wo = 1;
    p.taps = 1; p.stride = 1; p.pad = 0; p.up = 0;
    p.M = B * tokens; p.N = C; p.K = K; p.n_valid = C;
    p.ldo = tokens_pad; p.rows_per_batch = tokens; p.n_real = C;
    p.flags = EP_TRANSPOSE | EP_LNFOLD;
    p.alpha = 1.f; p.bias_scale = 1.f;
    p.ln_stats = stats.ptr; p.ln_np = stats.np; p.ln_inv_c = 1.0f / (float)n.c; p.ln_eps = 1e-5f; p.ln_s = Wv.s_ln;
    return launch_gemm(p, 1, false, true, r.s);
}

static int run_res(Run& r, const ResW& w, const half_t* x0, const half_t* x1, int c0, int c1, int B, int H, int Wd,
                   float eps, const float* embs, int emb_ld, half_t** out, float ss = 1.f, half_t* out_buf = nullptr, bool hilo = false,
                   size_t lo_rows = 0) {
    const int HW = H * Wd;
    const size_t M = (size_t)B * HW;
    const size_t LR = lo_rows ? lo_rows : M;
    const bool reuse = r.reuse();
    half_t* o_pre = reuse ? r.H(M * w.cout) : nullptr;
    float* st_pre = (reuse && ss == 1.f && w.cout % 32 == 0) ? r.F((size_t)B * 64 * 32 * 2) : nullptr;
    const size_t mk = r.ar->mark();
    const bool acc = hilo && r.acc() && ss == 1.f;
    const half_t* x0_lo = acc ? r.lo(x0, LR * c0) : nullptr;
    const half_t* x1_lo = (acc && x1) ? r.lo(x1, LR * c1) : nullptr;
    half_t* t1 = r.H(M * w.cin);
    TRY(run_gn(r, w.n1, x0, x1, c0, c1, B, HW, eps * ss * ss, true, t1, x0_lo, x1_lo));
    half_t* h1 = acc ? r.S(M * w.cout) : r.H(M * w.cout);
    {
        ConvArgs c;
        c.a0 = t1; c.c0 = w.cin; c.B = B; c.Hi = H; c.Wi = Wd; c.Ho = H; c.Wo = Wd; c.pad = 1;
        if (embs) { c.rowbias = embs + w.emb_off; c.ldrb = emb_ld; }
        c.out = h1; c.ldo = w.cout;
        c.out_lo = acc ? r.lo(h1, M * w.cout) : nullptr;
        c.stats_C = w.cout;
        TRY(run_conv(r, w.c1, c));
    }
    half_t* t2 = r.H(M * w.cout);
    TRY(run_gn(r, w.n2, h1, nullptr, w.cout, 0, B, HW, eps, true, t2, acc ? r.lo(h1, M * w.cout) : nullptr));
    const half_t* resid = x0;
    const half_t* resid_lo = x0_lo;
    if (w.has_skip) {
        half_t* sk = acc ? r.S(M * w.cout) : r.H(M * w.cout);
        ConvArgs c;
        c.a0 = x0; c.a1 = x1; c.c0 = c0; c.c1 = c1; c.B = B; c.Hi = H; c.Wi = Wd; c.Ho = H; c.Wo = Wd;
        c.out = sk; c.ldo = w.cout;
        c.resid_lo = nullptr;
        c.out_lo = acc ? r.lo(sk, M * w.cout) : nullptr;
        c.bias_scale = ss;
        TRY(run_conv(r, w.skip, c));
        resid = sk;
        resid_lo = c.out_lo;
    } else {
        SDMI_REQUIRE(x1 == nullptr, "identity skip with a concatenated input");
    }
    half_t* o = out_buf ? out_buf : (reuse ? o_pre : (acc ? r.S(M * w.cout) : r.H(M * w.cout)));
    {
        ConvArgs c;
        c.a0 = t2; c.c0 = w.cout; c.B = B; c.Hi = H; c.Wi = Wd; c.Ho = H; c.Wo = Wd; c.pad = 1;
        c.resid = resid; c.ldr = w.cout; c.out = o; c.ldo = w.cout;
        c.resid_lo = resid_lo; c.out_lo = acc ? r.lo(o, (out_buf ? LR : M) * w.cout) : nullptr;
        c.alpha = ss; c.bias_scale = ss;
        c.stats_C = ss == 1.f ? w.cout : 0;
        c.stats_ws_pre = st_pre;
        TRY(run_conv(r, w.c2, c));
    }
    if (reuse) r.ar->rewind(mk);
    *out = o;
    return 0;
}

static int run_attn(Run& r, const half_t* q, const half_t* k, const half_t* vt, half_t* out, int B, int H, int N, int M,
                    int D, int ldq, int ldk, int vt_ld, int ldo) {
    if (r.dry) return 0;
    AttnP p{};
    p.q = q; p.k = k; p.vt = vt; p.out = out;
    p.B = B; p.H = H; p.N = N; p.M = M; p.D = D;
    p.ldq = ldq; p.ldk = ldk; p.vt_ld = vt_ld; p.ldo = ldo;
    p.scale_log2 = (1.0f / sqrtf((float)D)) * 1.4426950408889634f;
    return launch_attention(p, r.e->force_generic, r.s);
}

static int run_vt(Run& r, const ConvW& Wv, const half_t* x, int ldx, int B, int tokens, int tokens_pad, half_t* vt,
                  bool bias_row, const int* gate = nullptr) {
    if (r.dry) return 0;
    GemmP p{};
    const int C = Wv.n_pad, K = Wv.cin_pad;
    if (g_vt_mode == 1 && tokens == tokens_pad && tokens % 4 == 0 && ldx == K && gate == nullptr) {
        p.a0 = x; p.c0 = K; p.cin = K; p.lda0 = ldx;
        p.w = Wv.w; p.ldw = K;
        p.bias = bias_row ? Wv.b : nullptr;
        p.out = vt;
        p.Hi = tokens; p.Wi = 1; p.Ho = tokens; p.Wo = 1;
        p.taps = 1; p.stride = 1; p.pad = 0; p.up = 0;
        p.M = B * tokens; p.N = C; p.K = K; p.n_valid = C;
        p.ldo = tokens_pad; p.rows_per_batch = tokens; p.n_real = C;
        p.flags = EP_TRANSPOSE;
        p.alpha = 1.f;
        return launch_gemm(p, 1, r.e->force_generic, r.e->use_glds, r.s);
    }
    p.a0 = Wv.w; p.c0 = K; p.cin = K; p.lda0 = K;
    p.w = x; p.ldw = ldx;
    p.bias = bias_row ? Wv.b : nullptr;
    p.out = vt;
    p.Hi = C; p.Wi = 1; p.Ho = C; p.Wo = 1;
    p.taps = 1; p.stride = 1; p.pad = 0; p.up = 0;
    p.M = C; p.N = tokens_pad; p.K = K; p.n_valid = tokens;
    p.ldo = tokens_pad; p.rows_per_batch = C; p.n_real = tokens_pad;
    p.flags = bias_row ? EP_BIAS_ROW : 0;
    p.alpha = 1.f;
    p.a_bs = 0; p.w_bs = (long)tokens * ldx;
    p.o_bs = (long)C * tokens_pad;
    p.gate = gate;
    return launch_gemm(p, B, r.e->force_generic, r.e->use_glds, r.s);
}

static bool hn_has_dim(const sdmi_engine* e, int dim) {
    for (const auto& n : e->hypernets)
        if (n.by_dim.count(dim)) return true;
    return false;
}

template <typename Alloc>
static int run_hn(Run& r, int dim, int which, const half_t* x, size_t rows, Alloc alloc, bool no_split, const half_t** out) {
    const half_t* cur = x;
    for (const HnNet& net : r.e->hypernets) {
        auto it = net.by_dim.find(dim);
        if (it == net.by_dim.end()) continue;
        const HnModule& mod = which ? it->second.second : it->second.first;
        const half_t* h = cur;
        int width = dim;
        half_t* y = nullptr;
        for (size_t i = 0; i < mod.ops.size(); ++i) {
            const HnOp& op = mod.ops[i];
            const bool last = i + 1 == mod.ops.size();
            if (op.kind == 0) {
                SDMI_REQUIRE(op.lin.cin_pad == width || r.dry, "hypernetwork layer widths do not chain");
                half_t* t = alloc(rows * (size_t)op.lin.n_pad);
                if (last) {
                    SDMI_REQUIRE(op.lin.n_pad == dim, "hypernetwork output width must equal its input width");
                    TRY(run_linear(r, op.lin, h, (int)rows, cur, t, op.lin.n_pad, net.multiplier, no_split));
                    y = t;
                } else {
                    TRY(run_linear(r, op.lin, h, (int)rows, nullptr, t, op.lin.n_pad, 1.f, no_split));
                }
                h = t;
                width = op.lin.n_pad;
            } else if (op.kind == 1) {
                if (!r.dry) TRY(launch_act_f16(const_cast<half_t*>(h), (int64_t)rows * width, op.act, r.s));
            } else {
                half_t* t = alloc(rows * (size_t)width);
                if (!r.dry) TRY(launch_layernorm(h, op.ln.g, op.ln.b, t, (int64_t)rows, width, 1e-5f, r.s));
                h = t;
            }
        }
        if (y == nullptr) {
            SDMI_REQUIRE(width == dim, "hypernetwork output width must equal its input width");
            y = alloc(rows * (size_t)dim);
            if (!r.dry) TRY(launch_axpy_f16(y, cur, h, net.multiplier, (int64_t)rows * dim, r.s));
        }
        cur = y;
    }
    *out = cur;
    return 0;
}

static int run_st(Run& r, const STW& st, const half_t* x, int B, int H, int Wd, int L, half_t** out,
                  const std::string& name = std::string(), int Bh = 0) {
    sdmi_engine* e = r.e;
    const int C = st.ch, HW = H * Wd;
    const size_t M = (size_t)B * HW;
    int B1 = Bh > 0 ? Bh : B;
    size_t M1 = (size_t)B1 * HW;
    const int Npad = rup(HW, 64);
    const bool reuse = r.reuse();
    half_t* o_pre = reuse ? r.H(M * C) : nullptr;
    half_t* cur_pre = reuse ? r.H(M * C) : nullptr;
    half_t* pp[2] = {reuse ? r.H(M * C) : nullptr, (reuse && st.blocks.size() > 1) ? r.H(M * C) : nullptr};
    const size_t mk = r.ar->mark();
    const bool acc = r.acc();
    const size_t MC = M * C;
    half_t* n0 = r.H(M * C);
    TRY(run_gn(r, st.norm, x, nullptr, C, 0, B1, HW, 1e-6f, false, n0, r.lo(x, MC)));
    half_t* cur = reuse ? cur_pre : r.S(M * C);
    const bool fold_any = e->ln_fold && !acc && !hn_has_dim(e, C) && !e->force_generic && e->use_glds && g_vt_mode == 1 && HW == Npad && HW % 4 == 0;
    r.lnp_want = fold_any && e->ln_fold >= 2;
    TRY(run_linear(r, st.proj_in, n0, (int)M1, nullptr, cur, C, 1.f, false, nullptr, r.lo(cur, MC)));
    if (reuse) r.ar->rewind(mk);
    int bi = 0, blk = 0;
    for (const TBlockW& b : st.blocks) {
        const std::string bname = name + ".transformer_blocks." + std::to_string(bi++);
        const bool fold = fold_any;
        half_t* a1 = nullptr;
        if (fold) {
            LnStats st1;
            TRY(run_ln_stats(r, b.ln1, cur, M, &st1));
            half_t* qk = r.H(M * 2 * C);
            TRY(run_linear_ln(r, b.qk1, b.ln1, cur, st1, (int)M, qk, 2 * C));
            half_t* vt = r.H((size_t)B * C * Npad);
            TRY(run_vt_ln(r, b.v1, b.ln1, cur, st1, B, HW, Npad, vt));
            a1 = r.H(M * C);
            TRY(run_attn(r, qk, qk + C, vt, a1, B, st.heads, HW, HW, st.dhead, 2 * C, 2 * C, Npad, C));
        }
        half_t* n1 = fold ? nullptr : r.H(M * C);
        if (!fold) TRY(run_ln(r, b.ln1, cur, M1, n1, r.lo(cur, MC)));
        if (fold) {
        } else if (!hn_has_dim(e, C)) {
            half_t* qk = r.H(M * 2 * C);
            TRY(run_linear(r, b.qk1, n1, (int)M1, nullptr, qk, 2 * C));
            half_t* vt = r.H((size_t)B * C * Npad);
            TRY(run_vt(r, b.v1, n1, C, B1, HW, Npad, vt, false));
            a1 = r.H(M * C);
            TRY(run_attn(r, qk, qk + C, vt, a1, B1, st.heads, HW, HW, st.dhead, 2 * C, 2 * C, Npad, C));
        } else {
            auto alloc = [&](size_t n) { return r.H(n); };
            const half_t *xk = nullptr, *xv = nullptr;
            TRY(run_hn(r, C, 0, n1, M, alloc, false, &xk));
            TRY(run_hn(r, C, 1, n1, M, alloc, false, &xv));
            ConvW wq = b.qk1, wk = b.qk1;
            wq.n_pad = wk.n_pad = C; wq.cout = wk.cout = C;
            wk.w = b.qk1.w + (size_t)C * b.qk1.cin_pad;
            if (b.qk1.b) wk.b = b.qk1.b + C;
            half_t* q = r.H(M * C);
            half_t* k = r.H(M * C);
            TRY(run_linear(r, wq, n1, (int)M, nullptr, q, C));
            TRY(run_linear(r, wk, xk, (int)M, nullptr, k, C));
            half_t* vt = r.H((size_t)B * C * Npad);
            TRY(run_vt(r, b.v1, xv, C, B, HW, Npad, vt, false));
            a1 = r.H(M * C);
            TRY(run_attn(r, q, k, vt, a1, B, st.heads, HW, HW, st.dhead, C, C, Npad, C));
        }
        half_t* x1 = r.S(M * C);
        r.lnp_want = fold && e->ln_fold >= 2;
        TRY(run_linear(r, b.o1, a1, (int)M1, cur, x1, C, 1.f, false, r.lo(cur, MC), r.lo(x1, MC)));
        if (B1 != B) {
            if (!r.dry) SDMI_CHECK_HIP(hipMemcpyAsync(x1 + M1 * C, x1, M1 * C * sizeof(half_t), hipMemcpyDeviceToDevice, r.s));
            if (!r.dry && acc) SDMI_CHECK_HIP(hipMemcpyAsync(x1 + MC + M1 * C, x1 + MC, M1 * C * sizeof(half_t), hipMemcpyDeviceToDevice, r.s));
            B1 = B; M1 = M;
        }
        r.tap(bname + ".attn1+x", x1, B, H, Wd, C);
        const bool chain_ok = !fold && !acc && !e->force_generic && e->use_glds && rowchain_supports(C) && HW % 128 == 0 && e->n_streams <= 1;
        half_t* x2 = nullptr;
        {
        half_t* q2 = nullptr;
        if (fold) {
            LnStats st2;
            TRY(run_ln_stats(r, b.ln2, x1, M, &st2));
            q2 = r.H(M * C);
            TRY(run_linear_ln(r, b.q2, b.ln2, x1, st2, (int)M, q2, C));
        } else {
            half_t* n2 = r.H(M * C);
            TRY(run_ln(r, b.ln2, x1, M, n2, r.lo(x1, MC)));
            q2 = r.H(M * C);
            TRY(run_linear(r, b.q2, n2, (int)M, nullptr, q2, C));
        }
        half_t* a2 = r.H(M * C);
        if (!r.dry) {
            SDMI_REQUIRE(e->ctx_valid && e->ctx_B == (r.Btot ? r.Btot : B), "context not set for this batch size");
            AttnP p{};
            p.q = q2; p.out = a2;
            p.k = e->ctx_k[b.ctx_slot] + (size_t)r.b0 * e->ctx_L * C;
            p.vt = e->ctx_vt[b.ctx_slot] + (size_t)r.b0 * C * e->ctx_Lpad;
            p.B = B; p.H = st.heads; p.N = HW; p.M = e->ctx_L; p.D = st.dhead;
            p.ldq = C; p.ldk = C; p.vt_ld = e->ctx_Lpad; p.ldo = C;
            p.scale_log2 = (1.0f / sqrtf((float)st.dhead)) * 1.4426950408889634f;
            TRY(launch_attention(p, e->force_generic, r.s));
        }
        x2 = r.S(M * C);
        r.lnp_want = fold && e->ln_fold >= 2;
        TRY(run_linear(r, b.o2, a2, (int)M, x1, x2, C, 1.f, false, r.lo(x1, MC), r.lo(x2, MC)));
        }
        r.tap(bname + ".attn2+x", x2, B, H, Wd, C);
        half_t* x3 = reuse ? pp[blk & 1] : r.S(M * C);
        if (chain_ok && (e->fuse_rows & 2) && b.ff1.geglu && b.ff1.n_pad % 64 == 0 && b.ff2.cin_pad * 2 == b.ff1.n_pad && b.ff1.cin_pad == C &&
            b.ff2.n_pad == C) {
            if (!r.dry) {
                const int hidden = b.ff2.cin_pad;
                if (!b.ff_packs) {
                    void* pk = nullptr;
                    SDMI_CHECK_HIP(hipMalloc(&pk, rowchain_ff_pack_bytes(C, hidden)));
                    e->owned.push_back(pk);
                    b.ff_packs = (char*)pk;
                }
                if (b.ff_epoch != e->weights_epoch) {
                    TRY(launch_rowchain_ff_pack(b.ff1.w, b.ff1.b, b.ff2.w, b.ff_packs, C, hidden, true, r.s));
                    b.ff_epoch = e->weights_epoch;
                }
                TRY(launch_rowchain_ff(x2, x3, b.ln3.g, b.ln3.b, b.ff_packs, b.ff2.b, (long)M, C, hidden, 1e-5f, r.s));
            }
        } else {
        half_t* g = nullptr;
        if (fold) {
            LnStats st3;
            TRY(run_ln_stats(r, b.ln3, x2, M, &st3));
            g = r.H(M * 4 * C);
            TRY(run_linear_ln(r, b.ff1, b.ln3, x2, st3, (int)M, g, 4 * C));
        } else {
            half_t* n3 = r.H(M * C);
            TRY(run_ln(r, b.ln3, x2, M, n3, r.lo(x2, MC)));
            g = r.H(M * 4 * C);
            TRY(run_linear(r, b.ff1, n3, (int)M, nullptr, g, 4 * C));
        }
        r.lnp_want = fold && e->ln_fold >= 2;
        TRY(run_linear(r, b.ff2, g, (int)M, x2, x3, C, 1.f, false, r.lo(x2, MC), r.lo(x3, MC)));
        }
        r.tap(bname, x3, B, H, Wd, C);
        cur = x3;
        ++blk;
        if (reuse) r.ar->rewind(mk);
    }
    half_t* o = reuse ? o_pre : r.S(M * C);
    TRY(run_linear(r, st.proj_out, cur, (int)M, x, o, C, 1.f, false, r.lo(x, MC), r.lo(o, MC)));
    *out = o;
    (void)L;
    return 0;
}

static void ctx_free(sdmi_engine* e) {
    for (void* p : e->ctx_owned) (void)hipFree(p);
    e->ctx_owned.clear(); e->ctx_k.clear(); e->ctx_vt.clear();
    e->ctx_f16 = nullptr; e->ctx_valid = false;
}

static void collect_st(const UNetW& u, std::vector<const STW*>* out) {
    for (auto& blk : u.input) for (auto& L : blk) if (L.kind == UNetLayer::ST) out->push_back(&L.st);
    for (auto& L : u.middle) if (L.kind == UNetLayer::ST) out->push_back(&L.st);
    for (auto& blk : u.output) for (auto& L : blk) if (L.kind == UNetLayer::ST) out->push_back(&L.st);
}

static int unet_set_context(sdmi_engine* e, const void* ctx, int dtype, int Bn, int L, hipStream_t s, bool conditional = false) {
    UNetW& u = e->unet;
    SDMI_REQUIRE(u.ready, "unet not finalized");
    const int cd = u.cfg.context_dim;
    const int Lpad = rup(L, 64);
    const int* gate = nullptr;
    if (conditional && e->ctx_valid && e->ctx_B == Bn && e->ctx_L == L && !e->ctx_k.empty() && !hn_has_dim(e, cd)) {
        if (!e->ctx_gate) {
            SDMI_CHECK_HIP(hipMalloc((void**)&e->ctx_gate, 256));
            e->owned.push_back(e->ctx_gate);
        }
// ... 5 lines not shown
        SDMI_CHECK_HIP(hipStreamSynchronize(s));
        ctx_free(e);
        void* p = nullptr;
        SDMI_CHECK_HIP(hipMalloc(&p, (size_t)Bn * Lpad * cd * sizeof(half_t)));
        e->ctx_owned.push_back(p);
        e->ctx_f16 = (half_t*)p;
        SDMI_CHECK_HIP(hipMemsetAsync(p, 0, (size_t)Bn * Lpad * cd * sizeof(half_t), s));
        std::vector<const STW*> sts;
        collect_st(u, &sts);
        e->ctx_k.assign(u.n_ctx_slots, nullptr);
        e->ctx_vt.assign(u.n_ctx_slots, nullptr);
        for (const STW* st : sts)
            for (const TBlockW& b : st->blocks) {
                SDMI_CHECK_HIP(hipMalloc(&p, (size_t)Bn * L * st->ch * sizeof(half_t)));
                e->ctx_owned.push_back(p);
                e->ctx_k[b.ctx_slot] = (half_t*)p;
                SDMI_CHECK_HIP(hipMalloc(&p, (size_t)Bn * st->ch * Lpad * sizeof(half_t)));
                e->ctx_owned.push_back(p);
                e->ctx_vt[b.ctx_slot] = (half_t*)p;
            }
        e->ctx_B = Bn; e->ctx_L = L; e->ctx_Lpad = Lpad;
    }
    if (gate) {
        TRY(launch_ctx_update_gated(ctx, dtype, e->ctx_f16, Bn, L, Lpad, cd, gate, s));
    } else {
        for (int b = 0; b < Bn; ++b) {
            const char* src = (const char*)ctx + (size_t)b * L * cd * (dtype == SDMI_F16 ? 2 : 4);
            TRY(launch_convert_to_f16(src, dtype, e->ctx_f16 + (size_t)b * Lpad * cd, (int64_t)L * cd, s));
        }
    }
    Run r{e, s, false};
    const half_t *ctx_k_src = e->ctx_f16, *ctx_v_src = e->ctx_f16;
    if (hn_has_dim(e, cd)) {
        SDMI_REQUIRE(gate == nullptr, "internal: gated context update with hypernetworks");
        const size_t rows = (size_t)Bn * Lpad;
        for (int pass = 0; pass < 2; ++pass) {
            size_t off = 0;
            const bool dry = pass == 0;
            auto alloc = [&](size_t n) {
                const size_t a = (off + 255) & ~size_t(255);
                off = a + n * sizeof(half_t);
                return (half_t*)(dry ? (char*)0x1000 + a : e->hn_ctx_scratch + a);
            };
            Run rr{e, s, dry};
            TRY(run_hn(rr, cd, 0, e->ctx_f16, rows, alloc, true, &ctx_k_src));
            TRY(run_hn(rr, cd, 1, e->ctx_f16, rows, alloc, true, &ctx_v_src));
            if (dry && off > e->hn_ctx_scratch_bytes) {
                SDMI_CHECK_HIP(hipStreamSynchronize(s));
                if (e->hn_ctx_scratch) (void)hipFree(e->hn_ctx_scratch);
                SDMI_CHECK_HIP(hipMalloc((void**)&e->hn_ctx_scratch, off + 256));
                e->hn_ctx_scratch_bytes = off;
            }
        }
    }
    std::vector<const STW*> sts;
    collect_st(u, &sts);
    for (const STW* st : sts)
        for (const TBlockW& b : st->blocks) {
            ConvArgs c;
            c.a0 = ctx_k_src; c.c0 = cd; c.B = 1; c.Hi = L; c.Wi = 1; c.Ho = L; c.Wo = 1;
            c.out = e->ctx_k[b.ctx_slot]; c.ldo = st->ch;
            c.batch = Bn; c.a_bs = (long)Lpad * cd; c.o_bs = (long)L * st->ch;
            c.gate = gate;
            c.no_split = true;
            TRY(run_conv(r, b.k2, c));
            TRY(run_vt(r, b.v2, ctx_v_src, cd, Bn, Lpad, Lpad, e->ctx_vt[b.ctx_slot], false, gate));
        }
    e->ctx_valid = true;
    return 0;
}

struct Act {
    half_t* p;
    int C, H, W;
};

static int unet_run(Run& r, const void* x, const void* t, const void* y, void* out, int io_dtype, int Bn, int h, int w,
                    int L) {
    sdmi_engine* e = r.e;
    UNetW& u = e->unet;
    const sdmi_unet_config& c = u.cfg;
    const int mc = c.model_channels, ted = mc * 4;
    r.ar->reset();
    float* sinus = r.F((size_t)Bn * mc);
    float* e1 = r.F((size_t)Bn * ted);
    float* emb = r.F((size_t)Bn * ted);
    float* embs = r.F((size_t)Bn * u.emb_cols);
    float* emb_act = r.F((size_t)Bn * ted);
    float* yf = c.adm_in_channels > 0 ? r.F((size_t)Bn * c.adm_in_channels) : nullptr;
    float* l1 = c.adm_in_channels > 0 ? r.F((size_t)Bn * ted) : nullptr;
    const int Be = (r.e->uniform_t && c.adm_in_channels == 0) ? 1 : Bn;
    const int emb_ld = Be == 1 ? 0 : u.emb_cols;
    if (!r.dry) {
        TRY(launch_timestep_embedding(t, io_dtype, sinus, Be, mc, r.s));
        TRY(launch_small_linear(sinus, u.te0.w, u.te0.b, nullptr, e1, Be, ted, mc, mc, ted, false, true, r.s));
        TRY(launch_small_linear(e1, u.te2.w, u.te2.b, nullptr, emb, Be, ted, ted, ted, ted, false, false, r.s));
        if (c.adm_in_channels > 0) {
            SDMI_REQUIRE(y != nullptr, "this UNet needs the vector conditioning y");
            TRY(launch_convert_to_f32(y, io_dtype, yf, (int64_t)Bn * c.adm_in_channels, r.s));
            TRY(launch_small_linear(yf, u.le0.w, u.le0.b, nullptr, l1, Bn, ted, c.adm_in_channels, c.adm_in_channels,
                                    ted, false, true, r.s));
            TRY(launch_small_linear(l1, u.le2.w, u.le2.b, emb, emb, Bn, ted, ted, ted, ted, false, false, r.s));
        }
        TRY(launch_silu_f32(emb, emb_act, (int64_t)Be * ted, r.s));
        TRY(launch_small_linear(emb_act, u.emb_all.w, u.emb_all.b, nullptr, embs, Be, u.emb_cols, ted, ted, u.emb_cols,
                                false, false, r.s));
    }
    const ConvW& cin_w = u.input[0][0].conv;
    half_t* xin = r.H((size_t)Bn * h * w * cin_w.cin_pad);
    const bool xin_lo = r.acc() && io_dtype != SDMI_F16 && 2 * c.in_channels <= cin_w.cin_pad;
    if (!r.dry) TRY(launch_nchw_to_nhwc(x, io_dtype, xin, Bn, c.in_channels, h * w, cin_w.cin_pad, 1.0f, nullptr, nullptr, r.s, xin_lo));

    std::vector<Act> hs;
    Act cur{nullptr, 0, h, w};
    const bool pairs = e->cfg_pairs && c.adm_in_channels == 0 && Bn % 2 == 0 && Bn >= 2 && !e->trace && !e->ln_fold && !r.reuse() &&
                       e->hypernets.empty() && (r.Btot == 0 || r.Btot == Bn);
    const int Bh = Bn / 2;
    bool shared = pairs;
    auto dup = [&](const Act& a) -> int {
        const size_t n = (size_t)Bh * a.H * a.W * a.C;
        if (!r.dry) SDMI_CHECK_HIP(hipMemcpyAsync((half_t*)a.p + n, a.p, n * sizeof(half_t), hipMemcpyDeviceToDevice, r.s));
        if (!r.dry && r.acc())
            SDMI_CHECK_HIP(hipMemcpyAsync((half_t*)a.p + 3 * n, a.p + 2 * n, n * sizeof(half_t), hipMemcpyDeviceToDevice, r.s));
        return 0;
    };
    auto run_block = [&](const std::vector<UNetLayer>& blk, const Act* skip, const std::string& bname) -> int {
        bool first = true;
        int li = 0;
        for (const UNetLayer& Lr : blk) {
            const std::string lname = bname + "." + std::to_string(li++);
            if (shared && (Lr.kind == UNetLayer::DOWN || Lr.kind == UNetLayer::UP || (Lr.kind == UNetLayer::RES && skip && first))) {
                TRY(dup(cur));
                shared = false;
            }
            switch (Lr.kind) {
                case UNetLayer::CONV_IN: {
                    half_t* o = r.S((size_t)Bn * cur.H * cur.W * Lr.conv.n_pad);
                    if (shared) {
                        ConvArgs a;
                        a.a0 = xin; a.c0 = Lr.conv.cin_pad; a.B = Bh; a.Hi = cur.H; a.Wi = cur.W; a.Ho = cur.H; a.Wo = cur.W;
                        a.pad = 1; a.out = o; a.ldo = Lr.conv.n_pad;
                        a.out_lo = r.lo(o, (size_t)Bn * cur.H * cur.W * Lr.conv.n_pad);
                        TRY(run_conv(r, Lr.conv, a));
                        cur = Act{o, Lr.conv.cout, cur.H, cur.W};
                        break;
                    }
                    ConvArgs a;
                    a.a0 = xin; a.c0 = Lr.conv.cin_pad; a.B = Bn; a.Hi = cur.H; a.Wi = cur.W; a.Ho = cur.H; a.Wo = cur.W;
                    a.pad = 1; a.out = o; a.ldo = Lr.conv.n_pad;
                    a.out_lo = r.lo(o, (size_t)Bn * cur.H * cur.W * Lr.conv.n_pad);
                    TRY(run_conv(r, Lr.conv, a));
                    cur = Act{o, Lr.conv.cout, cur.H, cur.W};
                    break;
                }
                case UNetLayer::RES: {
                    half_t* o = nullptr;
                    if (skip && first) {
                        SDMI_REQUIRE(Lr.c0 == cur.C && Lr.c1 == skip->C, "skip concat channel mismatch");
                        SDMI_REQUIRE(cur.H == skip->H && cur.W == skip->W, "skip connection spatial mismatch");
                        TRY(run_res(r, Lr.res, cur.p, skip->p, cur.C, skip->C, Bn, cur.H, cur.W, 1e-5f, embs, emb_ld, &o, 1.f, nullptr, true));
                    } else if (shared) {
                        half_t* full = r.S((size_t)Bn * cur.H * cur.W * Lr.res.cout);
                        TRY(run_res(r, Lr.res, cur.p, nullptr, cur.C, 0, Bh, cur.H, cur.W, 1e-5f, embs, emb_ld, &o, 1.f, full, true,
                                    (size_t)Bn * cur.H * cur.W));
                    } else {
                        TRY(run_res(r, Lr.res, cur.p, nullptr, cur.C, 0, Bn, cur.H, cur.W, 1e-5f, embs, emb_ld, &o, 1.f, nullptr, true));
                    }
                    cur = Act{o, Lr.res.cout, cur.H, cur.W};
                    break;
                }
                case UNetLayer::ST: {
                    half_t* o = nullptr;
                    if (shared) TRY(dup(cur));
                    TRY(run_st(r, Lr.st, cur.p, Bn, cur.H, cur.W, L, &o, lname, shared ? Bh : 0));
                    shared = false;
                    cur.p = o;
                    break;
                }
                case UNetLayer::DOWN: {
                    const int Ho = (cur.H + 2 - 3) / 2 + 1, Wo = (cur.W + 2 - 3) / 2 + 1;
                    half_t* o = r.S((size_t)Bn * Ho * Wo * cur.C);
                    ConvArgs a;
                    a.a0 = cur.p; a.c0 = cur.C; a.B = Bn; a.Hi = cur.H; a.Wi = cur.W; a.Ho = Ho; a.Wo = Wo;
                    a.stride = 2; a.pad = 1; a.out = o; a.ldo = cur.C;
                    a.out_lo = r.lo(o, (size_t)Bn * Ho * Wo * cur.C);
                    TRY(run_conv(r, Lr.conv, a));
                    cur = Act{o, cur.C, Ho, Wo};
                    break;
                }
                case UNetLayer::UP: {
                    const int Ho = cur.H * 2, Wo = cur.W * 2;
                    half_t* o = r.S((size_t)Bn * Ho * Wo * cur.C);
                    ConvArgs a;
                    a.a0 = cur.p; a.c0 = cur.C; a.B = Bn; a.Hi = cur.H; a.Wi = cur.W; a.Ho = Ho; a.Wo = Wo;
                    a.up = 1; a.pad = 1; a.out = o; a.ldo = cur.C;
                    a.out_lo = r.lo(o, (size_t)Bn * Ho * Wo * cur.C);
                    TRY(run_conv(r, Lr.conv, a));
                    cur = Act{o, cur.C, Ho, Wo};
                    break;
                }
            }
            first = false;
            r.tap(lname, cur.p, Bn, cur.H, cur.W, cur.C);
        }
        return 0;
    };
    if (!r.dry) e->taps.clear();
    const bool have_ctl = !e->control.empty();
    const size_t n_ctl = e->control.size();
    if (have_ctl) SDMI_REQUIRE(n_ctl == u.input.size() + 1, "control: one tensor per input block output and one for the middle block");
    auto add_control = [&](Act a, size_t idx, Act* out) -> int {
        const size_t n = (size_t)Bn * a.H * a.W * a.C;
        half_t* o = r.S(n);
        if (!r.dry) {
            const size_t full = (size_t)(r.Btot ? r.Btot : Bn) * a.C * a.H * a.W;
            SDMI_REQUIRE((size_t)e->control_numel[idx] == full, "control tensor " + std::to_string(idx) + " does not have the shape of the activation it is added to");
            const size_t elt = io_dtype == SDMI_F16 ? 2 : 4;
            const char* src = (const char*)e->control[idx] + (size_t)r.b0 * a.C * a.H * a.W * elt;
            TRY(launch_add_nchw_residual(a.p, r.lo(a.p, n), src, io_dtype, o, r.lo(o, n), Bn, a.C, a.H * a.W, r.s));
        }
        *out = Act{o, a.C, a.H, a.W};
        return 0;
    };
    int bidx = 0;
    for (auto& blk : u.input) {
        TRY(run_block(blk, nullptr, "input_blocks." + std::to_string(bidx++)));
        if (shared) TRY(dup(cur));
        Act sk = cur;
        if (have_ctl && !e->only_mid_control) TRY(add_control(cur, hs.size(), &sk));
        hs.push_back(sk);
    }
    shared = false;
    TRY(run_block(u.middle, nullptr, "middle_block"));
    if (have_ctl) TRY(add_control(cur, n_ctl - 1, &cur));
    bidx = 0;
    for (auto& blk : u.output) {
        Act sk = hs.back();
        hs.pop_back();
        TRY(run_block(blk, &sk, "output_blocks." + std::to_string(bidx++)));
    }
    const size_t M = (size_t)Bn * cur.H * cur.W;
    half_t* tn = r.H(M * cur.C);
    TRY(run_gn(r, u.out_norm, cur.p, nullptr, cur.C, 0, Bn, cur.H * cur.W, 1e-5f, true, tn, r.lo(cur.p, M * cur.C)));
    float* eps = r.F((size_t)Bn * c.out_channels * cur.H * cur.W);
    {
        ConvArgs a;
        a.a0 = tn; a.c0 = cur.C; a.B = Bn; a.Hi = cur.H; a.Wi = cur.W; a.Ho = cur.H; a.Wo = cur.W; a.pad = 1;
        a.out = eps; a.flags = EP_NCHW; a.n_real = c.out_channels;
        TRY(run_conv(r, u.out_conv, a));
    }
    if (!r.dry) TRY(launch_copy_out(eps, out, io_dtype, (int64_t)Bn * c.out_channels * cur.H * cur.W, r.s));
    return 0;
}

static int ensure_arena(Arena& ar, size_t need, hipStream_t s) {
    if (need <= ar.cap) return 0;
    SDMI_CHECK_HIP(hipStreamSynchronize(s));
    if (ar.base) SDMI_CHECK_HIP(hipFree(ar.base));
    ar.base = nullptr; ar.cap = 0;
    const size_t cap = need + (need >> 4) + (1 << 20);
    SDMI_CHECK_HIP(hipMalloc((void**)&ar.base, cap));
    ar.cap = cap;
    return 0;
}
static int ensure_arena(sdmi_engine* e, size_t need, hipStream_t s) { return ensure_arena(e->arena, need, s); }

static int unet_forward_slice(sdmi_engine* e, Arena& ar, const void* x, const void* t, const void* y, void* out, int io_dtype,
                              int Bn, int b0, int Btot, int h, int w, int L, hipStream_t s) {
    Run dry(e, s, true, &ar, b0, Btot);
    ar.dry = true; ar.high = 0;
    TRY(unet_run(dry, x, t, y, out, io_dtype, Bn, h, w, L));
    ar.dry = false;
    TRY(ensure_arena(ar, ar.high, s));
    Run run(e, s, false, &ar, b0, Btot);
    return unet_run(run, x, t, y, out, io_dtype, Bn, h, w, L);
}

int unet_forward(sdmi_engine* e, const void* x, const void* t, const void* ctx, const void* y, void* out, int io_dtype,
                 int Bn, int h, int w, int L, hipStream_t s) {
    SDMI_REQUIRE(e->unet.ready, "unet not finalized");
    SDMI_CHECK_HIP(hipSetDevice(e->device));
    const char* cpv = getenv("SDMI_CHECK_PROMISES");
    const bool check_promises = cpv && atoi(cpv) != 0;
    if (check_promises && (e->cfg_pairs || e->uniform_t)) {
        const size_t elt = io_dtype == SDMI_F16 ? 2 : 4;
        SDMI_CHECK_HIP(hipStreamSynchronize(s));
        if (e->uniform_t && Bn > 1) {
            std::vector<char> th((size_t)Bn * elt);
            SDMI_CHECK_HIP(hipMemcpy(th.data(), t, th.size(), hipMemcpyDeviceToHost));
            for (int b = 1; b < Bn; ++b)
                SDMI_REQUIRE(memcmp(th.data(), th.data() + (size_t)b * elt, elt) == 0, "option uniform_t is set but the timesteps of the call differ");
        }
        if (e->cfg_pairs && Bn % 2 == 0 && Bn >= 2) {
            const size_t half_bytes = (size_t)(Bn / 2) * e->unet.cfg.in_channels * h * w * elt;
            std::vector<char> xh(2 * half_bytes), th((size_t)Bn * elt);
            SDMI_CHECK_HIP(hipMemcpy(xh.data(), x, xh.size(), hipMemcpyDeviceToHost));
            SDMI_CHECK_HIP(hipMemcpy(th.data(), t, th.size(), hipMemcpyDeviceToHost));
            SDMI_REQUIRE(memcmp(xh.data(), xh.data() + half_bytes, half_bytes) == 0,
                         "option cfg_pairs is set but rows [Bn/2, Bn) of x do not repeat rows [0, Bn/2)");
            SDMI_REQUIRE(memcmp(th.data(), th.data() + th.size() / 2, th.size() / 2) == 0,
                         "option cfg_pairs is set but the timesteps of the two halves differ");
        }
    }
    struct Restore {
        sdmi_engine* e; bool pairs, uni, on;
        ~Restore() { if (on) { e->cfg_pairs = pairs; e->uniform_t = uni; } }
    } restore{e, e->cfg_pairs, e->uniform_t, e->auto_promises};
    if (e->auto_promises) {
        const size_t elt = io_dtype == SDMI_F16 ? 2 : 4;
        const size_t half_bytes = (size_t)(Bn / 2) * e->unet.cfg.in_channels * h * w * elt;
        std::vector<char> th((size_t)Bn * elt), xh(Bn % 2 == 0 && Bn >= 2 ? 2 * half_bytes : 0);
        SDMI_CHECK_HIP(hipStreamSynchronize(s));
        SDMI_CHECK_HIP(hipMemcpy(th.data(), t, th.size(), hipMemcpyDeviceToHost));
        bool uni = true;
        for (int b = 1; b < Bn && uni; ++b) uni = memcmp(th.data(), th.data() + (size_t)b * elt, elt) == 0;
        bool pairs = uni && !xh.empty();
        if (pairs) {
            SDMI_CHECK_HIP(hipMemcpy(xh.data(), x, xh.size(), hipMemcpyDeviceToHost));
            pairs = memcmp(xh.data(), xh.data() + half_bytes, half_bytes) == 0;
        }
        e->uniform_t = uni;
        e->cfg_pairs = pairs;
    }
    struct ClearControl {
        sdmi_engine* e;
        ~ClearControl() { e->control.clear(); e->control_numel.clear(); e->only_mid_control = false; }
    } clear_control{e};
    if (ctx) TRY(unet_set_context(e, ctx, io_dtype, Bn, L, s));
    const int ns = (e->n_streams > 1 && !e->trace && Bn % e->n_streams == 0) ? e->n_streams : 1;
    SDMI_REQUIRE(!(ns > 1 && e->ln_fold), "engine options ln_fold and streams > 1 cannot be combined");
    if (ns == 1) return unet_forward_slice(e, e->arena, x, t, y, out, io_dtype, Bn, 0, Bn, h, w, L, s);
    const sdmi_unet_config& c = e->unet.cfg;
    while ((int)e->aux_streams.size() < ns - 1) {
// ... 662 lines not shown
```

stable-diffusion-webui_amd/csrc/gemm.hip:

```cpp
#include "common.h"
#include "prof.h"
#include <algorithm>
#include <cmath>
#include <cstdlib>
#include <map>

namespace sdmi {

typedef const __attribute__((address_space(1))) void* gptr_t;
typedef __attribute__((address_space(3))) void* lptr_t;

struct RowInfo {
    int b, yo, xo;
    bool ok;
};

struct GRow {
    int yb, xb;
    int pixbase;
    bool ok;
};

__device__ __forceinline__ float gelu_erf(float g) {
    const float x = fabsf(g) * 0.70710678118654752f;
// ... 2046 lines not shown

int g_force_gemm_split = 0;
int g_shortk_gemm_cfg = [] { const char* e = getenv("SDMI_SHORTK_CFG"); return e ? atoi(e) : -1; }();
int g_shortk_max_k = [] { const char* e = getenv("SDMI_SHORTK_MAXK"); return e ? atoi(e) : 448; }();
int g_geglu_gemm_cfg = [] { const char* e = getenv("SDMI_GEGLU_CFG"); return e ? atoi(e) : -1; }();
int g_conv_korder_default = [] { const char* e = getenv("SDMI_CONV_KORDER"); return e ? atoi(e) : 2; }();
int g_conv_korder = g_conv_korder_default;
int g_ep_wide = [] { const char* e = getenv("SDMI_EP_WIDE"); return e ? atoi(e) : 1; }();
int g_gn_fuse = [] { const char* e = getenv("SDMI_GN_FUSE"); return e ? atoi(e) : 1; }();
int g_tile_order = [] { const char* e = getenv("SDMI_TILE_ORDER"); return e ? atoi(e) : -1; }();
int g_vt_mode = [] { const char* e = getenv("SDMI_VT_MODE"); return e ? atoi(e) : 1; }();
int g_gemm_pipe_default = [] { const char* e = getenv("SDMI_GEMM_PIPE"); return e ? atoi(e) : 4; }();
int g_gemm_pipe = g_gemm_pipe_default;

static bool cfg_valid(int cfg, const GemmP& p) {
    if (cfg < 0 || cfg >= CFG_COUNT) return false;
    if (p.N % kCfgBN[cfg]) return false;
    if (cfg == CFG_256x64) return false;
    if ((p.flags & EP_GEGLU) && (cfg == CFG_256x320 || cfg == CFG_128x320 || cfg == CFG_128x160 || cfg == CFG_256x128 || cfg == CFG_128x160_R4 || cfg == CFG_128x160_R3)) return false;
    if (cfg >= CFG_128x160_R4 && (p.korder || (p.flags & EP_LNFOLD))) return false;
    return true;
}

static const int kCfgOcc[CFG_COUNT] = {2, 2, 4, 3, 1, 1, 1, 3, 1, 2, 1, 1, 2, 1};

static float cfg_score(const GemmP& p, int batch, int cfg, int split) {
    const float tiles = (float)((long)cdiv(p.M, kCfgBM[cfg]) * (p.N / kCfgBN[cfg]) * batch * split);
    const float cus = 256.f, cap = cus * kCfgOcc[cfg];
    float fill;
    if (tiles <= cus) fill = 0.8f * tiles / cus;
    else if (tiles <= cap) fill = 0.8f + 0.2f * (tiles - cus) / (cap - cus + 1e-3f);
    else { const float w = tiles / cap; fill = w / ceilf(w); }
    if (kCfgOcc[cfg] == 1 && tiles <= cus) fill = tiles / cus;
    float score = kCfgEff[cfg] * fill;
    const int ksteps = p.K / 64 / split;
    if (ksteps < 8 && kCfgOcc[cfg] == 1) score *= 0.9f;
    if (split > 1) {
        const double flops = 2.0 * p.M * (double)p.N * p.K * batch;
        const double t_mma = flops / (1.0e15 * (score > 0.05f ? score : 0.05f));
        const double slab_bytes = (double)split * p.M * p.N * batch * 4.0;
        const double bw = slab_bytes < 128.0e6 ? 6.0e12 : 3.0e12;
        const double t_red = 2.0 * slab_bytes / bw + 3.0e-6;
        score = (float)(score * t_mma / (t_mma + t_red));
    }
    return score;
}

struct ShapeKey { int M, N, K, taps, kind; };
struct ShapeChoice { ShapeKey k; int cfg, split; };
static std::vector<ShapeChoice> g_gemm_override;
static const ShapeChoice kTunedShapes[] = {
#include "gemm_tuned_shapes.inc"
    {{0, 0, 0, 0, 0}, -1, 1}
};
int gemm_set_override(const char* spec) {
    g_gemm_override.clear();
    if (!spec) return 0;
    const char* c = spec;
    while (*c) {
        ShapeChoice sc{};
        int n = 0;
        if (sscanf(c, "%d,%d,%d,%d,%d:%d:%d%n", &sc.k.M, &sc.k.N, &sc.k.K, &sc.k.taps, &sc.k.kind, &sc.cfg, &sc.split, &n) != 7) return 1;
        if (sc.split > 8) sc.split = 8;
        g_gemm_override.push_back(sc);
        c += n;
        if (*c == ';') ++c;
    }
    return 0;
}
static const ShapeChoice* find_shape(const GemmP& p) {
    const int base_kind = (p.flags & EP_GEGLU) ? 1 : (p.flags & EP_TRANSPOSE) ? 2 : 0;
    for (int kind : {(p.flags & EP_HILO) ? base_kind + 4 : base_kind, base_kind}) {
        for (const ShapeChoice& sc : g_gemm_override)
            if (sc.k.M == p.M && sc.k.N == p.N && sc.k.K == p.K && sc.k.taps == p.taps && sc.k.kind == kind) return &sc;
        for (const ShapeChoice& sc : kTunedShapes)
            if (sc.cfg >= 0 && sc.k.M == p.M && sc.k.N == p.N && sc.k.K == p.K && sc.k.taps == p.taps && sc.k.kind == kind) return &sc;
    }
    return nullptr;
}

static int pick_cfg(const GemmP& p, int batch, int* split_out, bool allow_split) {
    *split_out = 1;
    if (g_force_gemm_cfg >= 0 && cfg_valid(g_force_gemm_cfg, p)) {
        if (allow_split && g_force_gemm_split > 1 && p.K / 64 / g_force_gemm_split >= 4) *split_out = std::min(g_force_gemm_split, 8);
        return g_force_gemm_cfg;
    }
    if (g_force_gemm_split == 1) allow_split = false;
    if (g_shortk_gemm_cfg >= 0 && p.taps == 1 && p.K <= g_shortk_max_k && !(p.flags & EP_GEGLU) && cfg_valid(g_shortk_gemm_cfg, p))
        return g_shortk_gemm_cfg;
    if (g_geglu_gemm_cfg >= 0 && (p.flags & EP_GEGLU) && cfg_valid(g_geglu_gemm_cfg, p)) return g_geglu_gemm_cfg;
    if (batch == 1) {
        if (const ShapeChoice* sc = find_shape(p)) {
            if (cfg_valid(sc->cfg, p) && (sc->split <= 1 || (allow_split && p.K / 64 / sc->split >= 2))) {
                *split_out = sc->split > 1 ? sc->split : 1;
                return sc->cfg;
            }
        }
    }
    const int cands[] = {CFG_256x320, CFG_256x256, CFG_128x320, CFG_128x128_K32, CFG_128x128, CFG_128x64, CFG_64x64};
    int best = -1;
    float best_score = -1.f;
    const int nk = p.K / 64;
    for (int cfg : cands) {
        if (!cfg_valid(cfg, p)) continue;
        for (int split : {1, 2, 3, 4, 6, 8}) {
            if (split > 1 && (!allow_split || nk / split < 12)) break;
            const float sc = cfg_score(p, batch, cfg, split);
            if (sc > best_score * 1.03f) { best_score = sc; best = cfg; *split_out = split; }
        }
    }
    return best >= 0 ? best : CFG_64x64;
}

size_t gemm_splitk_ws_bytes(int M, int N, int K, int batch) {
    if (K < 64 * 16 || N % 64) return 0;
    if ((long)cdiv(M, 128) * cdiv(N, 128) * batch >= 512) return 0;
    return (size_t)8 * M * N * batch * sizeof(float);
}

int launch_gemm(const GemmP& p_in, int batch, bool force_generic, bool use_glds, hipStream_t s, int* stats_nchunk_out, int* lnp_np_out) {
    GemmP p = p_in;
    p.stats_nchunk = 0;
    p.lnp_np = 0;
    if (stats_nchunk_out) *stats_nchunk_out = 0;
    if (lnp_np_out) *lnp_np_out = 0;
    p.flags |= g_gemm_dbgflags;
    if (p.n_valid <= 0 || p.n_valid > p.N) p.n_valid = p.N;
    if (p.bias_scale == 0.f) p.bias_scale = 1.f;
    p.korder = (p.taps == 9 && g_conv_korder == 1 && !p.up && !(p.flags & EP_WRAP)) ? 1 : 0;
    p.zero = zero_page();
    SDMI_REQUIRE(p.zero != nullptr, "zero page allocation failed");
    SDMI_REQUIRE(p.M > 0 && p.N > 0 && p.K > 0, "empty GEMM");
    SDMI_REQUIRE(p.cin % 8 == 0, "Cin must be a multiple of 8 (pad channels)");
    const double pf_flops = 2.0 * p.M * (double)p.N * p.K * batch;
    const double pf_in = (p.taps == 9 ? (double)p.M / (p.stride * p.stride) * (p.up ? 0.25 : 1.0) : (double)p.M) * p.cin * 2.0;
    const double pf_bytes = (pf_in + (double)p.N * p.K * 2.0 + (double)p.M * p.N * ((p.flags & EP_OUT_F32) ? 4.0 : 2.0)) * batch;
    if (p.flags & EP_LNFOLD) {
        SDMI_REQUIRE(p.ln_stats && p.ln_s && p.taps == 1 && !p.a1 && !p.stats_out && !(p.flags & (EP_NCHW | EP_OUT_F32 | EP_BIAS_ROW)),
                     "EP_LNFOLD: 1x1 / linear layers with fp16 row-major (or transposed) output only");
        SDMI_REQUIRE(!force_generic && use_glds && gemm_mfma_supported(p), "EP_LNFOLD runs on the LDS-direct MFMA kernels only");
    }
    if (force_generic || !gemm_mfma_supported(p)) {
        SDMI_REQUIRE(!(p.flags & EP_HILO), "(hi, lo) stream tensors need the MFMA kernels (shape not supported / force_generic)");
        const bool geglu = p.flags & EP_GEGLU;
        const long total = (long)p.M * (geglu ? p.N / 2 : p.N);
        int blocks = (int)std::min<long>((total + 255) / 256, 65535L * 8);
        ProfScope ps("gemm_generic", pf_flops, pf_bytes, s);
        hipLaunchKernelGGL(gemm_generic_kernel, dim3(blocks, 1, batch), dim3(256), 0, s, p);
        SDMI_CHECK_HIP(hipGetLastError());
        return 0;
    }
    {
        auto al16 = [](const void* q) { return ((uintptr_t)q & 15) == 0; };
        bool wide = g_ep_wide != 0 && al16(p.out) && p.ldo % 8 == 0 && p.o_bs % 8 == 0 && p.N % 8 == 0;
        if (p.resid) wide = wide && al16(p.resid) && p.ldr % 8 == 0 && p.r_bs % 8 == 0;
        if (p.flags & EP_TRANSPOSE) wide = wide && p.rows_per_batch % 8 == 0 && p.M % 8 == 0;
        if (!wide) p.flags |= EP_NARROW;
    }
    const bool hilo = (p.flags & EP_HILO) != 0;
    if (hilo) {
        SDMI_REQUIRE(!force_generic && !(p.flags & (EP_GEGLU | EP_NCHW | EP_TRANSPOSE | EP_OUT_F32 | EP_LNFOLD | EP_BIAS_ROW | EP_QUICK_GELU | EP_GELU)) &&
                         (gemm_resid_lo(p) == nullptr || p.resid != nullptr),
                     "(hi, lo) stream tensors: plain fp16 row-major epilogue on the MFMA kernels only");
        auto al16 = [](const void* q) { return ((uintptr_t)q & 15) == 0; };
        if (!al16(gemm_out_lo(p)) || !al16(gemm_resid_lo(p))) p.flags |= EP_NARROW;
        p.lnp_out = nullptr;
    }
    int split = 1;
    const bool can_split = p.splitk_ws != nullptr && !(p.flags & (EP_GEGLU | EP_NCHW | EP_TRANSPOSE)) && p.N % 4 == 0;
    SDMI_REQUIRE(!(p.flags & EP_TRANSPOSE) || (p.rows_per_batch % 4 == 0 && p.M % 4 == 0 && !(p.flags & (EP_GEGLU | EP_NCHW | EP_OUT_F32 | EP_BIAS_ROW)) &&
                                               !p.resid && !p.rowbias),
                 "EP_TRANSPOSE: rows per image must be a multiple of 4; no residual / GEGLU / fp32 output");
    const int cfg_picked = pick_cfg(p, batch, &split, can_split);
    const int cfg = cfg_picked;
    const bool phase = use_glds && (g_gemm_pipe == 3 || g_gemm_pipe == 4) &&
                       (cfg == CFG_256x320 || cfg == CFG_256x256 || cfg == CFG_256x128 || (cfg == CFG_128x320 && g_gemm_pipe == 4)) && p.n_valid == p.N &&
                       p.cin + 64 <= kZeroPageHalfs &&
                       ((p.taps == 1 && p.stride == 1 && !p.up && p.Ho == p.Hi && p.Wo == p.Wi) ||
                        (p.M / p.rows_per_batch < 128 && (p.up ? 2 : 1) * p.Hi < 2040 && (p.up ? 2 : 1) * p.Wi < 2040 &&
                         p.stride * p.Ho < 2040 && p.stride * p.Wo < 2040));
    const bool dxwalk = g_conv_korder == 2 && phase && p.taps == 9 && p.stride == 1 && p.pad == 1 && !p.up &&
                        !(p.flags & (EP_WRAP | EP_GEGLU | EP_TRANSPOSE | EP_LNFOLD)) && p.Ho == p.Hi && p.Wo == p.Wi && p.Wo % 16 == 0 &&
                        kCfgBM[cfg] % p.Wo == 0 && p.Wi < 2040 && p.Hi < 2040 && !p.lnp_out && !(g_gemm_dbg && p.stats_nchunk == 0);
    if (dxwalk) p.korder = 2;
    if (split > 1) {
        const int nk = p.K / (cfg == CFG_128x128_K32 ? 32 : 64);
        p.splitk_steps = cdiv(nk, split);
        if (dxwalk) p.splitk_steps = cdiv(p.splitk_steps, 3) * 3;
        p.splitk = cdiv(nk, p.splitk_steps);
        if (p.splitk <= 1) { p.splitk = 0; split = 1; }
    } else {
        p.splitk = 0;
    }
    {
        const int BMc = kCfgBM[cfg], BNc = kCfgBN[cfg];
        const long tiles_m = cdiv(p.M, BMc), tiles_n = p.N / BNc;
        const double run = std::max(1.0, (double)tiles_m * tiles_n / 8.0);
        const double a_panel = (double)BMc * p.cin * 2.0 * (p.taps == 9 ? 1.3 : 1.0) / ((p.taps == 9 && p.up) ? 2.0 : 1.0);
        const double w_panel = (double)BNc * p.K * 2.0 / (split > 1 ? split : 1);
        const double n_first = std::ceil(run / tiles_n) * a_panel + std::min<double>(run, tiles_n) * w_panel;
        const double m_first = std::ceil(run / tiles_m) * w_panel + std::min<double>(run, tiles_m) * a_panel;
        p.tile_order = g_tile_order >= 0 ? g_tile_order : (m_first < 0.8 * n_first ? 1 : 0);
        if (tiles_n == 1 || tiles_m == 1) p.tile_order = 0;
    }
    if (p.stats_out && g_gn_fuse && use_glds && split <= 1 && batch == 1 && !(p.flags & (EP_GEGLU | EP_TRANSPOSE | EP_NCHW | EP_OUT_F32 | EP_BIAS_ROW | EP_QUICK_GELU | EP_GELU)) && p.stats_cpg > 0) {
        const int BMc = kCfgBM[cfg], BNc = kCfgBN[cfg];
        if (p.rows_per_batch % BMc == 0 && BNc % p.stats_cpg == 0 && p.N % p.stats_cpg == 0 && p.rows_per_batch / BMc <= 64 &&
            p.M % p.rows_per_batch == 0 && (!hilo || (cfg != CFG_64x64 && cfg != CFG_256x320 && !(p.flags & EP_NARROW)))) {
            p.stats_nchunk = p.rows_per_batch / BMc;
            if (stats_nchunk_out) *stats_nchunk_out = p.stats_nchunk;
        }
    }
    if (p.lnp_out && !hilo && use_glds && split <= 1 && batch == 1 && p.stats_nchunk == 0 &&
        !(p.flags & (EP_NARROW | EP_GEGLU | EP_TRANSPOSE | EP_NCHW | EP_OUT_F32 | EP_BIAS_ROW | EP_QUICK_GELU | EP_GELU | EP_LNFOLD)) &&
        kCfgBM[cfg] % 32 == 0 && cfg != CFG_64x64 && (phase || kCfgBM[cfg] < 256)) {
        p.lnp_np = p.N / kCfgBN[cfg];
        if (lnp_np_out) *lnp_np_out = p.lnp_np;
    }
    std::string pname;
    if (prof_enabled()) {
        pname = std::string(kCfgName[cfg]) + (phase ? "pp" : "") + (split > 1 ? "_splitk" + std::to_string(p.splitk) : "") + (p.taps == 9 ? "_conv3x3" : "_1x1") +
                ((p.flags & EP_GEGLU) ? "_geglu" : "") + ((p.flags & EP_TRANSPOSE) ? "_tr" : "") + ((p.flags & EP_HILO) ? "_hl" : "") + (p.tile_order ? "_mf" : "") + (p.stats_nchunk ? "_gn" : "") + (p.korder == 2 ? "_dx" : "") + " M" + std::to_string(p.M) + " N" + std::to_string(p.N) + " K" + std::to_string(p.K) +
                ((p.flags & EP_LNFOLD) ? " ln" : "") + (batch > 1 ? " x" + std::to_string(batch) : "");
    }
    ProfScope ps(pname.c_str(), pf_flops, pf_bytes, s);
    struct Reduce {
        const GemmP& p; int batch; hipStream_t s; bool on;
        int run() const {
            if (!on) return 0;
            const long total = (long)p.M * (p.N / 4);
            const dim3 grid((unsigned)std::min<long>((total + 255) / 256, 8192));
            if (p.flags & EP_LNFOLD) hipLaunchKernelGGL(splitk_reduce_kernel<true>, grid, dim3(256), 0, s, p, batch);
            else hipLaunchKernelGGL(splitk_reduce_kernel<false>, grid, dim3(256), 0, s, p, batch);
            SDMI_CHECK_HIP(hipGetLastError());
            return 0;
        }
    } reduce{p, batch, s, split > 1};
#define SDMI_CASE(ID, BM, BN, WR, WC, BK)                                                                       \
    case ID:                                                                                                    \
        if (use_glds ? launch_cfg<BM, BN, WR, WC, BK, true>(p, batch, s) : launch_cfg<BM, BN, WR, WC, BK, false>(p, batch, s)) \
            return 1;                                                                                           \
        return reduce.run();
    if (phase) {
        int rc = 1;
        switch (cfg) {
            case CFG_256x320: rc = launch_pingpong<256, 320>(p, batch, s); break;
            case CFG_256x256: rc = launch_pingpong<256, 256>(p, batch, s); break;
            case CFG_256x128: rc = launch_pingpong<256, 128>(p, batch, s); break;
            case CFG_128x320: rc = launch_pingpong<128, 320>(p, batch, s); break;
            default: break;
        }
        if (rc) return 1;
        return reduce.run();
    }
    switch (cfg) {
        SDMI_CASE(CFG_128x128, 128, 128, 2, 2, 64)
        SDMI_CASE(CFG_64x64, 64, 64, 4, 1, 64)
        SDMI_CASE(CFG_128x128_K32, 128, 128, 2, 2, 32)
        SDMI_CASE(CFG_256x256, 256, 256, 4, 2, 64)
        SDMI_CASE(CFG_256x128, 256, 128, 4, 2, 64)
        SDMI_CASE(CFG_256x320, 256, 320, 4, 2, 64)
        SDMI_CASE(CFG_128x64, 128, 64, 4, 1, 64)
        SDMI_CASE(CFG_128x320, 128, 320, 2, 4, 64)
        SDMI_CASE(CFG_128x160, 128, 160, 2, 2, 64)
        case CFG_128x160_R4: if (use_glds ? launch_ring<128, 160, 2, 2, 4>(p, batch, s) : launch_cfg<128, 160, 2, 2, 64, false>(p, batch, s)) return 1; return reduce.run();
        case CFG_128x160_R3: if (use_glds ? launch_ring<128, 160, 2, 2, 3>(p, batch, s) : launch_cfg<128, 160, 2, 2, 64, false>(p, batch, s)) return 1; return reduce.run();
        case CFG_128x128_R4: if (use_glds ? launch_ring<128, 128, 2, 2, 4>(p, batch, s) : launch_cfg<128, 128, 2, 2, 64, false>(p, batch, s)) return 1; return reduce.run();
        case CFG_128x64_R3: if (use_glds ? launch_ring<128, 64, 4, 1, 3>(p, batch, s) : launch_cfg<128, 64, 4, 1, 64, false>(p, batch, s)) return 1; return reduce.run();
    }
#undef SDMI_CASE
    set_error("bad gemm config");
    return 1;
}

}
```

stable-diffusion-webui_amd/csrc/norm.hip:

```cpp
#include "common.h"
#include "prof.h"
#include <algorithm>
#include <cstdio>
#include <cstdlib>

namespace sdmi {

static constexpr int GN_MAX_C = 4096;

template <bool HILO = false>
__global__ __launch_bounds__(256) void gn_stats_kernel(const half_t* x0, const half_t* x1, int c0, int c1, int HW,
                                                       int groups, int rows_per_chunk, float* partial, const half_t* l0 = nullptr,
                                                       const half_t* l1 = nullptr) {
    __shared__ float s_sum[GN_MAX_C];
    __shared__ float s_sq[GN_MAX_C];
    const int C = c0 + c1, VP = C / 8;
    const int chunk = blockIdx.x, b = blockIdx.y, nchunk = gridDim.x;
    const int tid = threadIdx.x;
    const int TP = VP < 256 ? VP : 256;
    const int R = 256 / TP;
    const int p_begin = chunk * rows_per_chunk;
    const int p_end = min(HW, p_begin + rows_per_chunk);
    if (tid < TP * R) {
        const int tr = tid / TP, tc = tid - tr * TP;
        for (int cv = tc; cv < VP; cv += TP) {
            const int c = cv * 8;
            const half_t* src;
            int cc, ld;
            if (c < c0) { src = x0; cc = c; ld = c0; } else { src = x1; cc = c - c0; ld = c1; }
            const half_t* base = src + (long)b * HW * ld + cc;
            [[maybe_unused]] const half_t* lbase = HILO ? (c < c0 ? l0 : l1) + (long)b * HW * ld + cc : nullptr;
            float a[8], q[8], k[8];
#pragma unroll
            for (int e = 0; e < 8; ++e) { a[e] = 0.f; q[e] = 0.f; k[e] = 0.f; }
            int pix = p_begin + tr;
            const int n_t = pix < p_end ? (p_end - pix + R - 1) / R : 0;
            if (pix < p_end) {
                const h8 v = *reinterpret_cast<const h8*>(base + (long)pix * ld);
                h8 lv = {0, 0, 0, 0, 0, 0, 0, 0};
                if constexpr (HILO) lv = *reinterpret_cast<const h8*>(lbase + (long)pix * ld);
#pragma unroll
                for (int e = 0; e < 8; ++e) k[e] = HILO ? (float)v[e] + (float)lv[e] : (float)v[e];
                pix += R;
            }
            for (; pix + 3 * R < p_end; pix += 4 * R) {
                h8 v[4];
#pragma unroll
                for (int u = 0; u < 4; ++u) v[u] = *reinterpret_cast<const h8*>(base + (long)(pix + u * R) * ld);
#pragma unroll
                for (int u = 0; u < 4; ++u) {
                    h8 lv = {0, 0, 0, 0, 0, 0, 0, 0};
                    if constexpr (HILO) lv = *reinterpret_cast<const h8*>(lbase + (long)(pix + u * R) * ld);
#pragma unroll
                    for (int e = 0; e < 8; ++e) { const float f = (HILO ? (float)v[u][e] + (float)lv[e] : (float)v[u][e]) - k[e]; a[e] += f; q[e] = fmaf(f, f, q[e]); }
                }
            }
            for (; pix < p_end; pix += R) {
                const h8 v = *reinterpret_cast<const h8*>(base + (long)pix * ld);
                h8 lv = {0, 0, 0, 0, 0, 0, 0, 0};
                if constexpr (HILO) lv = *reinterpret_cast<const h8*>(lbase + (long)pix * ld);
#pragma unroll
                for (int e = 0; e < 8; ++e) { const float f = (HILO ? (float)v[e] + (float)lv[e] : (float)v[e]) - k[e]; a[e] += f; q[e] = fmaf(f, f, q[e]); }
            }
            const float inv = n_t > 0 ? 1.0f / (float)n_t : 0.f;
#pragma unroll
            for (int e = 0; e < 8; ++e) { s_sum[tr * C + c + e] = fmaf(a[e], inv, k[e]); s_sq[tr * C + c + e] = fmaxf(q[e] - a[e] * a[e] * inv, 0.f); }
        }
    }
    __syncthreads();
    {
        const int g = tid >> 3, l8 = tid & 7;
        const int cpg = C / groups, n = R * cpg;
        const int np = max(p_end - p_begin, 0);
        const float pv = g < groups ? s_sum[g * cpg] : 0.f;
        float a = 0.f;
        if (g < groups)
            for (int i = l8; i < n; i += 8) {
                const int r = i / cpg, c = g * cpg + (i - r * cpg);
                a = fmaf((float)max((np - r + R - 1) / R, 0), s_sum[r * C + c] - pv, a);
            }
        for (int off = 4; off > 0; off >>= 1) a += __shfl_xor(a, off);
        const float mean = np > 0 ? pv + a / ((float)np * (float)cpg) : 0.f;
        float q = 0.f;
        if (g < groups)
            for (int i = l8; i < n; i += 8) {
                const int r = i / cpg, c = g * cpg + (i - r * cpg);
                const float d = s_sum[r * C + c] - mean;
// ... 37 lines not shown
#pragma unroll
    for (int u = 1; u < U; ++u) {
        iv[u] = iv[u - 1] + (unsigned)stride;
        pix_u[u] = pix_u[u - 1] + sp; cv_u[u] = cv_u[u - 1] + sr;
        if (cv_u[u] >= VP) { cv_u[u] -= VP; ++pix_u[u]; }
    }
    const half_t* x0b = x0 + (long)b * HW * c0;
    const half_t* x1b = x1 ? x1 + (long)b * HW * c1 : nullptr;
    [[maybe_unused]] const half_t* l0b = HILO ? l0 + (long)b * HW * c0 : nullptr;
    [[maybe_unused]] const half_t* l1b = (HILO && l1) ? l1 + (long)b * HW * c1 : nullptr;
    half_t* outb = out + (long)b * HW * C;
    h8 v[U];
    [[maybe_unused]] h8 lv[HILO ? U : 1];
    int cs[U];
    bool ok[U];
    auto request = [&]() {
#pragma unroll
        for (int u = 0; u < U; ++u) {
            ok[u] = pix_u[u] < HW;
            const unsigned pix = ok[u] ? (unsigned)pix_u[u] : 0u;
            const int c = (ok[u] ? cv_u[u] : 0) * 8;
            cs[u] = c;
            const half_t* src;
            unsigned cc, ld;
            if (c < c0) { src = x0b; cc = (unsigned)c; ld = (unsigned)c0; } else { src = x1b; cc = (unsigned)(c - c0); ld = (unsigned)c1; }
            v[u] = *reinterpret_cast<const h8*>(src + (__umul24(pix, ld) + cc));
            if constexpr (HILO) lv[u] = *reinterpret_cast<const h8*>((c < c0 ? l0b : l1b) + (__umul24(pix, ld) + cc));
        }
    };
    request();
    {
        const int g = tid >> 3, l8 = tid & 7;
        float n = 0.f, mean = 0.f, m2 = 0.f;
        if (g < groups)
            for (int ch = l8; ch < nchunk; ch += 8) {
                const float* src = partial + (((long)b * nchunk + ch) * groups + g) * 2;
                const int j = ch % chunk_period;
                gn_merge(n, mean, m2, (float)(max(min(chunk_rows, HW - j * chunk_rows), 0) * cpg), src[0], src[1]);
            }
        for (int off = 4; off > 0; off >>= 1) {
            const float nb = __shfl_xor(n, off), mb = __shfl_xor(mean, off), qb = __shfl_xor(m2, off);
            gn_merge(n, mean, m2, nb, mb, qb);
        }
        if (g < groups && l8 == 0) {
            s_mean[g] = mean;
            s_rstd[g] = rsqrtf(m2 / n + eps);
        }
    }
    __syncthreads();
    for (int c = tid; c < C; c += 256) {
        const int g = c / cpg;
        const float sc = s_rstd[g] * gamma[c];
        s_scale[c] = sc;
        s_shift[c] = beta[c] - s_mean[g] * sc;
    }
    __syncthreads();
    while (true) {
#pragma unroll
        for (int u = 0; u < U; ++u) {
            if (!ok[u]) continue;
            const f4 sa = *reinterpret_cast<const f4*>(&s_scale[cs[u]]), sb = *reinterpret_cast<const f4*>(&s_scale[cs[u] + 4]);
            const f4 ha = *reinterpret_cast<const f4*>(&s_shift[cs[u]]), hb = *reinterpret_cast<const f4*>(&s_shift[cs[u] + 4]);
            h8 o;
#pragma unroll
            for (int e = 0; e < 8; ++e) {
                const float sc = e < 4 ? sa[e] : sb[e - 4], sh = e < 4 ? ha[e] : hb[e - 4];
                float y = fmaf(HILO ? (float)v[u][e] + (float)lv[HILO ? u : 0][e] : (float)v[u][e], sc, sh);
                if (silu) y = y * __builtin_amdgcn_rcpf(1.0f + __expf(-y));
                o[e] = (half_t)y;
            }
            *reinterpret_cast<h8*>(outb + iv[u] * 8u) = o;
        }
#pragma unroll
        for (int u = 0; u < U; ++u) {
            iv[u] += (unsigned)(U * stride);
            pix_u[u] += spU; cv_u[u] += srU;
            if (cv_u[u] >= VP) { cv_u[u] -= VP; ++pix_u[u]; }
        }
        if (pix_u[0] >= HW) break;
        request();
    }
}

template <int NVT, bool HILO = false>
__global__ __launch_bounds__(256) void gn_fused_small_kernel(const half_t* x0, const half_t* x1, int c0, int c1, int HW, int groups,
                                                             const float* gamma, const float* beta, half_t* out, float eps, int silu,
                                                             const half_t* l0 = nullptr, const half_t* l1 = nullptr) {
    __shared__ float red[2][4];
    const int C = c0 + c1, cpg = C / groups, VW = cpg / 8;
    const int g = blockIdx.x, b = blockIdx.y, tid = threadIdx.x;
    const int cbase = g * cpg;
    const half_t* x0b = x0 + (long)b * HW * c0;
    const half_t* x1b = x1 ? x1 + (long)b * HW * c1 : nullptr;
    h8 v[NVT];
    [[maybe_unused]] h8 vl[HILO ? NVT : 1];
    [[maybe_unused]] const half_t* l0b = HILO ? l0 + (long)b * HW * c0 : nullptr;
    [[maybe_unused]] const half_t* l1b = (HILO && l1) ? l1 + (long)b * HW * c1 : nullptr;
    int off[NVT], cch[NVT];
    float s = 0.f;
    const int sp = 256 / VW, sr = 256 - sp * VW;
    int pix = tid / VW, vc = tid - pix * VW;
#pragma unroll
    for (int k = 0; k < NVT; ++k) {
        const bool ok = pix < HW;
        const int pp = ok ? pix : 0;
        const int c = cbase + vc * 8;
        off[k] = ok ? pp * C + c : -1;
        cch[k] = c;
        const half_t* src = c < c0 ? x0b + (long)pp * c0 + c : x1b + (long)pp * c1 + (c - c0);
        h8 z = {0, 0, 0, 0, 0, 0, 0, 0};
        v[k] = ok ? *reinterpret_cast<const h8*>(src) : z;
        if constexpr (HILO) {
            const half_t* srcl = c < c0 ? l0b + (long)pp * c0 + c : l1b + (long)pp * c1 + (c - c0);
            vl[k] = ok ? *reinterpret_cast<const h8*>(srcl) : z;
        }
        pix += sp; vc += sr;
        if (vc >= VW) { vc -= VW; ++pix; }
    }
#pragma unroll
    for (int k = 0; k < NVT; ++k)
#pragma unroll
        for (int e = 0; e < 8; ++e) s += HILO ? (float)v[k][e] + (float)vl[HILO ? k : 0][e] : (float)v[k][e];
    for (int o = 32; o > 0; o >>= 1) s += __shfl_xor(s, o);
    if ((tid & 63) == 0) red[0][tid >> 6] = s;
    __syncthreads();
    const float n = (float)cpg * (float)HW;
    const float mean = ((red[0][0] + red[0][1]) + (red[0][2] + red[0][3])) / n;
    float q = 0.f;
#pragma unroll
    for (int k = 0; k < NVT; ++k)
        if (off[k] >= 0) {
#pragma unroll
            for (int e = 0; e < 8; ++e) { const float d = (HILO ? (float)v[k][e] + (float)vl[HILO ? k : 0][e] : (float)v[k][e]) - mean; q = fmaf(d, d, q); }
        }
    for (int o = 32; o > 0; o >>= 1) q += __shfl_xor(q, o);
    if ((tid & 63) == 0) red[1][tid >> 6] = q;
    __syncthreads();
    const float rstd = rsqrtf(((red[1][0] + red[1][1]) + (red[1][2] + red[1][3])) / n + eps);
    half_t* outb = out + (long)b * HW * C;
#pragma unroll
    for (int k = 0; k < NVT; ++k) {
        if (off[k] < 0) continue;
        const int c = cch[k];
        const f4 g0 = *reinterpret_cast<const f4*>(gamma + c), g1 = *reinterpret_cast<const f4*>(gamma + c + 4);
        const f4 b0 = *reinterpret_cast<const f4*>(beta + c), b1 = *reinterpret_cast<const f4*>(beta + c + 4);
        h8 o;
#pragma unroll
        for (int e = 0; e < 8; ++e) {
            const float gm = e < 4 ? g0[e] : g1[e - 4], bt = e < 4 ? b0[e] : b1[e - 4];
            float y = fmaf(((HILO ? (float)v[k][e] + (float)vl[HILO ? k : 0][e] : (float)v[k][e]) - mean) * rstd, gm, bt);
            if (silu) y = y * __builtin_amdgcn_rcpf(1.0f + __expf(-y));
            o[e] = (half_t)y;
        }
        *reinterpret_cast<h8*>(outb + off[k]) = o;
    }
}

int g_gn_apply_blocks = 0;
int g_gn_small = [] { const char* e = getenv("SDMI_GN_SMALL"); return e ? atoi(e) : 1; }();

static inline int gn_chunks(int B, int HW) {
    int n = (1024 + B - 1) / B;
    if (n > HW / 32) n = HW / 32;
    if (n > 64) n = 64;
    if (n < 1) n = 1;
    return n;
}

long g_gn_band_elems = 0;
static inline long gn_band_limit() { return g_gn_band_elems > 0 ? g_gn_band_elems : (1L << 31); }
static inline int gn_row_limit() { return g_gn_band_elems > 0 ? (1 << 30) : (1 << 24); }
static int gn_bands(int HW, int C) {
    if ((long)HW * C < gn_band_limit() && HW < gn_row_limit()) return 1;
    for (int nb = 2; nb <= 8192; nb *= 2)
        if (HW % nb == 0 && (long)(HW / nb) * C < gn_band_limit() && HW / nb < gn_row_limit()) return nb;
    return 0;
}

int64_t groupnorm_ws_bytes(int B, int HW, int groups) {
    int64_t chunks = gn_chunks(B, HW);
    if ((long)HW * GN_MAX_C >= gn_band_limit() || HW >= gn_row_limit()) {
        int nb = 2;
        while (nb < 8192 && !((long)(HW / nb) * GN_MAX_C < gn_band_limit() && HW / nb < gn_row_limit())) nb *= 2;
        chunks = std::max<int64_t>(chunks, (int64_t)nb * 64);
    }
    return (int64_t)B * chunks * groups * 2 * sizeof(float);
}

static int groupnorm_banded(const half_t* x0, const half_t* x1, int c0, int c1, const float* gamma, const float* beta, half_t* out, int B,
                            int HW, int groups, float eps, bool silu, float* ws, hipStream_t s, int nb) {
    const int C = c0 + c1, HWb = HW / nb;
    const int nchunk_b = gn_chunks(1, HWb), rows = cdiv(HWb, nchunk_b), nchunk = nb * nchunk_b;
    SDMI_REQUIRE((int64_t)B * nchunk * groups * 2 * (int64_t)sizeof(float) <= groupnorm_ws_bytes(B, HW, groups),
                 "banded GroupNorm: partial sums exceed the workspace groupnorm_ws_bytes provisions");
    char pname[64];
    snprintf(pname, sizeof pname, "groupnorm_silu_banded B%d HW%d C%d x%d", B, HW, C, nb);
    ProfScope ps(pname, 0.0, 3.0 * B * (double)HW * C * 2.0, s);
    const long per_image = (long)nchunk * groups * 2;
    for (int b = 0; b < B; ++b)
        for (int k = 0; k < nb; ++k) {
            const long row0 = (long)b * HW + (long)k * HWb;
            hipLaunchKernelGGL(gn_stats_kernel<false>, dim3(nchunk_b, 1), dim3(256), 0, s, x0 + row0 * c0, x1 ? x1 + row0 * c1 : nullptr, c0, c1, HWb,
                               groups, rows, ws + b * per_image + (long)k * nchunk_b * groups * 2, nullptr, nullptr);
            SDMI_CHECK_HIP(hipGetLastError());
        }
    const long nvec = (long)HWb * (C / 8);
    const long trips = std::max<long>(1, cdiv(nvec, 2048L * 2048));
    int blocks = (int)std::max<long>(1, cdiv(nvec, 2048 * trips));
    if (g_gn_apply_blocks > 0) blocks = g_gn_apply_blocks;
    const size_t smem = (size_t)2 * C * sizeof(float);
    for (int b = 0; b < B; ++b)
        for (int k = 0; k < nb; ++k) {
            const long row0 = (long)b * HW + (long)k * HWb;
            hipLaunchKernelGGL((gn_apply_kernel<false, 8>), dim3(blocks, 1), dim3(256), smem, s, x0 + row0 * c0, x1 ? x1 + row0 * c1 : nullptr, c0, c1,
                               HWb, groups, nchunk, rows, nchunk_b, ws + b * per_image, gamma, beta, out + row0 * C, eps, silu ? 1 : 0, nullptr, nullptr);
            SDMI_CHECK_HIP(hipGetLastError());
        }
    return 0;
}


int launch_groupnorm(const half_t* x0, const half_t* x1, int c0, int c1, const float* gamma, const float* beta,
                     half_t* out, int B, int HW, int groups, float eps, bool silu, float* ws, hipStream_t s, int pre_nchunk,
                     const half_t* x0_lo, const half_t* x1_lo) {
    const int C = c0 + c1;
    const bool hilo = x0_lo != nullptr;
    SDMI_REQUIRE(!hilo || (x1 == nullptr) == (x1_lo == nullptr), "GroupNorm (hi, lo) input: both sources as pairs");
    SDMI_REQUIRE(C % 8 == 0 && c0 % 8 == 0, "GroupNorm channels must be multiples of 8");
    SDMI_REQUIRE(C <= GN_MAX_C && groups <= 32 && C % groups == 0, "GroupNorm: C <= 4096, groups <= 32, C % groups == 0");
    if (const int nb = gn_bands(HW, C); nb != 1) {
        SDMI_REQUIRE(nb > 1, "GroupNorm: an image of 2^31 elements or more must split into equal power-of-two bands of rows below that limit");
        SDMI_REQUIRE(!hilo && pre_nchunk <= 0, "GroupNorm beyond 2^31 elements per image: fp16 input with its own statistics pass only");
        return groupnorm_banded(x0, x1, c0, c1, gamma, beta, out, B, HW, groups, eps, silu, ws, s, nb);
    }
    char pname[64];
    {
        const int cpg = C / groups;
        const long nv = (long)HW * (cpg / 8);
        if (pre_nchunk <= 0 && g_gn_small && cpg % 8 == 0 && nv <= (hilo ? 6 : 12) * 256) {
            snprintf(pname, sizeof pname, "groupnorm_silu_fused B%d HW%d C%d", B, HW, C);
            ProfScope ps(pname, 0.0, (hilo ? 3.0 : 2.0) * B * (double)HW * C * 2.0, s);
            const dim3 grid(groups, B);
#define SDMI_GNS(NVT, HL) hipLaunchKernelGGL((gn_fused_small_kernel<NVT, HL>), grid, dim3(256), 0, s, x0, x1, c0, c1, HW, groups, gamma, beta, out, eps, silu ? 1 : 0, x0_lo, x1_lo)
            if (hilo) { if (nv <= 2 * 256) SDMI_GNS(2, true); else SDMI_GNS(6, true); }
            else if (nv <= 4 * 256) SDMI_GNS(4, false);
            else SDMI_GNS(12, false);
#undef SDMI_GNS
            SDMI_CHECK_HIP(hipGetLastError());
            return 0;
        }
    }
    const int nchunk = pre_nchunk > 0 ? pre_nchunk : gn_chunks(B, HW);
    const int rows = cdiv(HW, nchunk);
    snprintf(pname, sizeof pname, pre_nchunk > 0 ? "groupnorm_silu_apply B%d HW%d C%d" : "groupnorm_silu B%d HW%d C%d", B, HW, C);
    ProfScope ps(pname, 0.0, (pre_nchunk > 0 ? 2.0 : 3.0) * B * (double)HW * C * 2.0, s);
    if (pre_nchunk <= 0) {
        if (hilo) hipLaunchKernelGGL(gn_stats_kernel<true>, dim3(nchunk, B), dim3(256), 0, s, x0, x1, c0, c1, HW, groups, rows, ws, x0_lo, x1_lo);
        else hipLaunchKernelGGL(gn_stats_kernel<false>, dim3(nchunk, B), dim3(256), 0, s, x0, x1, c0, c1, HW, groups, rows, ws, nullptr, nullptr);
        SDMI_CHECK_HIP(hipGetLastError());
    }
    const long nvec = (long)HW * (C / 8);
    const long cap = std::max(1, 2048 / B);
    const long trips = std::max<long>(1, cdiv(nvec, 2048 * cap));
    int blocks = (int)std::max<long>(1, cdiv(nvec, 2048 * trips));
    if (g_gn_apply_blocks > 0) blocks = g_gn_apply_blocks;
    const size_t smem = (size_t)2 * C * sizeof(float);
    if (hilo)
        hipLaunchKernelGGL((gn_apply_kernel<true, 4>), dim3(blocks, B), dim3(256), smem, s, x0, x1, c0, c1, HW, groups, nchunk, rows, nchunk, ws, gamma,
                           beta, out, eps, silu ? 1 : 0, x0_lo, x1_lo);
    else
        hipLaunchKernelGGL((gn_apply_kernel<false, 8>), dim3(blocks, B), dim3(256), smem, s, x0, x1, c0, c1, HW, groups, nchunk, rows, nchunk, ws, gamma,
                           beta, out, eps, silu ? 1 : 0, nullptr, nullptr);
    SDMI_CHECK_HIP(hipGetLastError());
    return 0;
}

#define LN_VAL(r, k, e) (HILO ? (float)v[r][k][e] + (float)vl[HILO ? (r) : 0][HILO ? (k) : 0][e] : (float)v[r][k][e])
template <int K, int RPW, bool HILO = false>
__global__ __launch_bounds__(256) void layernorm_kernel(const half_t* x, const float* gamma, const float* beta,
                                                        half_t* out, long rows, int C, float eps, const half_t* xlo = nullptr) {
    const int lane = threadIdx.x & 63, wave = threadIdx.x >> 6;
    const long row0 = ((long)blockIdx.x * 4 + wave) * RPW;
    if (row0 >= rows) return;
    const int VP = C / 8;
    const float inv_c = 1.0f / (float)C;
    h8 v[RPW][K];
    [[maybe_unused]] h8 vl[HILO ? RPW : 1][HILO ? K : 1];
    float sum[RPW];
#pragma unroll
    for (int r = 0; r < RPW; ++r) {
        const long row = min(row0 + r, rows - 1);
        const half_t* src = x + row * C;
#pragma unroll
        for (int k = 0; k < K; ++k) {
            const int cv = lane + k * 64;
            h8 z = {0, 0, 0, 0, 0, 0, 0, 0};
            v[r][k] = cv < VP ? *reinterpret_cast<const h8*>(src + cv * 8) : z;
            if constexpr (HILO) vl[r][k] = cv < VP ? *reinterpret_cast<const h8*>(xlo + row * C + cv * 8) : z;
        }
    }
#pragma unroll
    for (int r = 0; r < RPW; ++r) {
        float a = 0.f;
#pragma unroll
        for (int k = 0; k < K; ++k)
#pragma unroll
            for (int e = 0; e < 8; ++e) a += LN_VAL(r, k, e);
        sum[r] = a;
    }
    for (int off = 32; off > 0; off >>= 1)
#pragma unroll
        for (int r = 0; r < RPW; ++r) sum[r] += __shfl_xor(sum[r], off);
    float mean[RPW], sq[RPW];
#pragma unroll
    for (int r = 0; r < RPW; ++r) {
        mean[r] = sum[r] * inv_c;
        float q = 0.f;
#pragma unroll
        for (int k = 0; k < K; ++k) {
            const int cv = lane + k * 64;
            if (cv < VP) {
#pragma unroll
                for (int e = 0; e < 8; ++e) { const float d = LN_VAL(r, k, e) - mean[r]; q = fmaf(d, d, q); }
            }
        }
        sq[r] = q;
// ... 165 lines not shown
```

stable-diffusion-webui_amd/ops.py:

```python
from __future__ import annotations

import ctypes as C
from typing import Optional

import torch

from . import _lib
from ._lib import lib, check, ptr, stream_ptr, ConvDesc, F16, F32, EP_OUT_F32, EP_GEGLU, EP_NCHW, EP_BIAS_ROW


def _rup(x, m):
    return (x + m - 1) // m * m


def attention(q: torch.Tensor, k: torch.Tensor, v: torch.Tensor, heads: int, scale: Optional[float] = None) -> torch.Tensor:
    _lib.require_device()
    assert q.dtype == torch.float16 and k.dtype == torch.float16 and v.dtype == torch.float16
    b, n, c = q.shape
    m = k.shape[1]
    d = c // heads
    q, k, v = [t if t.stride(-1) == 1 and t.stride(0) == t.shape[1] * t.stride(1) else t.contiguous() for t in (q, k, v)]
    out = torch.empty((b, n, c), dtype=torch.float16, device=q.device)
    scale = d ** -0.5 if scale is None else scale
    if heads == 1 and d > 160 and d % 64 == 0:
# ... 30 lines not shown
    check(lib.sdmi_pack_conv_weight(ptr(w), _lib.dtype_code(w), ptr(out), o, i, kh, kw, o_pad, i_pad, 1 if geglu else 0,
                                    stream_ptr()), "pack_conv_weight")
    return out


def pack_bias(b: Optional[torch.Tensor], n_pad: int, geglu: bool = False) -> Optional[torch.Tensor]:
    if b is None:
        return None
    bf = b.float()
    if geglu:
        o = bf.shape[0]
        half = o // 2
        idx = torch.arange(o, device=bf.device)
        g, r = idx // 64, idx % 64
        src = torch.where(r < 32, g * 32 + r, half + g * 32 + (r - 32))
        bf = bf[src]
    out = torch.zeros(n_pad, dtype=torch.float32, device=b.device)
    out[: bf.shape[0]] = bf
    return out


def conv_gemm(a0: torch.Tensor, w_packed: torch.Tensor, *, a1: Optional[torch.Tensor] = None, bias=None, rowbias=None,
              resid=None, taps: int = 9, stride: int = 1, pad: int = 1, up: bool = False, Ho=None, Wo=None,
              geglu: bool = False, out_f32: bool = False, nchw_real: int = 0, bias_row: bool = False, alpha: float = 1.0,
              impl: str = "mfma", transpose: bool = False, wrap: bool = False) -> torch.Tensor:
    _lib.require_device()
    assert a0.dtype == torch.float16 and a0.is_contiguous()
    b, hi, wi, c0 = a0.shape
    c1 = a1.shape[3] if a1 is not None else 0
    n = w_packed.shape[0]
    if Ho is None:
        if up:
            Ho, Wo = 2 * hi, 2 * wi
        elif taps == 9:
            p2 = 2 if pad else 1
            Ho, Wo = (hi + p2 - 3) // stride + 1, (wi + p2 - 3) // stride + 1
        else:
            Ho, Wo = hi, wi
    d = ConvDesc()
    d.a0, d.a1, d.w = a0.data_ptr(), (a1.data_ptr() if a1 is not None else None), w_packed.data_ptr()
    d.bias = bias.data_ptr() if bias is not None else None
    d.rowbias = rowbias.data_ptr() if rowbias is not None else None
    d.resid = resid.data_ptr() if resid is not None else None
    d.c0, d.c1, d.lda0, d.lda1 = c0, c1, c0, c1
    d.B, d.Hi, d.Wi, d.Ho, d.Wo = b, hi, wi, Ho, Wo
    d.taps, d.stride, d.pad, d.up = taps, stride, pad if taps == 9 else 0, 1 if up else 0
    d.N = n
    flags = 0
    n_out = n
    if geglu:
        flags |= EP_GEGLU
        n_out = n // 2
    if bias_row:
        flags |= EP_BIAS_ROW
    if wrap:
        flags |= _lib.EP_WRAP
    if nchw_real:
        flags |= EP_NCHW
        out = torch.empty((b, nchw_real, Ho, Wo), dtype=torch.float32, device=a0.device)
        d.n_real = nchw_real
    elif out_f32:
        flags |= EP_OUT_F32
        out = torch.empty((b, Ho, Wo, n_out), dtype=torch.float32, device=a0.device)
    elif transpose:
        flags |= _lib.EP_TRANSPOSE
        out = torch.empty((b, n_out, Ho * Wo), dtype=torch.float16, device=a0.device)
    else:
        out = torch.empty((b, Ho, Wo, n_out), dtype=torch.float16, device=a0.device)
    d.out = out.data_ptr()
    d.ldo = Ho * Wo if transpose else n_out
    d.ldr = resid.shape[-1] if resid is not None else 0
    d.flags = flags
    d.alpha = alpha
    d.batch = 1
    d.force_generic = {"mfma": 0, "generic": 1, "mfma_reg": 2}[impl]
    wsb = lib.sdmi_conv_splitk_workspace_bytes(b * Ho * Wo, n, taps * (c0 + c1), 1)
    if wsb and not geglu and not nchw_real:
        ws = torch.empty(wsb, dtype=torch.uint8, device=a0.device)
        d.splitk_workspace, d.splitk_workspace_bytes = ws.data_ptr(), wsb
    check(lib.sdmi_conv_gemm(C.byref(d), stream_ptr()), "sdmi_conv_gemm")
    return out


def groupnorm(x0: torch.Tensor, gamma: torch.Tensor, beta: torch.Tensor, *, x1: Optional[torch.Tensor] = None,
              groups: int = 32, eps: float = 1e-5, silu: bool = True) -> torch.Tensor:
    _lib.require_device()
    b, h, w, c0 = x0.shape
    c1 = x1.shape[3] if x1 is not None else 0
    out = torch.empty((b, h, w, c0 + c1), dtype=torch.float16, device=x0.device)
    wsb = lib.sdmi_groupnorm_workspace_bytes(b, h * w, groups)
    ws = torch.empty(max(wsb, 16), dtype=torch.uint8, device=x0.device)
    check(lib.sdmi_groupnorm(ptr(x0), ptr(x1), c0, c1, ptr(gamma.float().contiguous()), ptr(beta.float().contiguous()),
                             ptr(out), b, h * w, groups, float(eps), 1 if silu else 0, ptr(ws), wsb, stream_ptr()), "sdmi_groupnorm")
    return out


def layernorm(x: torch.Tensor, gamma: torch.Tensor, beta: torch.Tensor, eps: float = 1e-5) -> torch.Tensor:
    _lib.require_device()
    c = x.shape[-1]
    x = x.contiguous()
    out = torch.empty_like(x)
    check(lib.sdmi_layernorm(ptr(x), ptr(gamma.float().contiguous()), ptr(beta.float().contiguous()), ptr(out),
                             x.numel() // c, c, float(eps), stream_ptr()), "sdmi_layernorm")
    return out


def rowchain_ff_pack(w1: torch.Tensor, b1, w2: torch.Tensor) -> torch.Tensor:
    _lib.require_device()
    hidden, c = w2.shape[1], w2.shape[0]
    w1, w2 = w1.half().contiguous(), w2.half().contiguous()
    b1 = b1.float().contiguous() if b1 is not None else None
    packs = torch.empty(int(lib.sdmi_rowchain_ff_pack_bytes(c, hidden)), dtype=torch.uint8, device=w1.device)
    check(lib.sdmi_rowchain_ff_pack(ptr(w1), ptr(b1) if b1 is not None else None, ptr(w2), ptr(packs), c, hidden, stream_ptr()),
          "sdmi_rowchain_ff_pack")
    return packs


def rowchain_ff(x: torch.Tensor, gamma, beta, packs: torch.Tensor, b2, hidden: int, eps: float = 1e-5) -> torch.Tensor:
    _lib.require_device()
    c = x.shape[-1]
    x = x.contiguous()
    out = torch.empty_like(x)
    b2 = b2.float().contiguous() if b2 is not None else None
    check(lib.sdmi_rowchain_ff(ptr(x), ptr(out), ptr(gamma.float().contiguous()), ptr(beta.float().contiguous()), ptr(packs),
                               ptr(b2) if b2 is not None else None, x.numel() // c, c, hidden, float(eps), stream_ptr()), "sdmi_rowchain_ff")
    return out


def philox_randn(shape, seed: int, offset: int, device) -> torch.Tensor:
    _lib.require_device()
    out = torch.empty(tuple(shape), dtype=torch.float32, device=device)
    check(lib.sdmi_philox_randn(ptr(out), out.numel(), C.c_uint64(seed & 0xFFFFFFFFFFFFFFFF), C.c_uint32(offset), stream_ptr()),
          "sdmi_philox_randn")
    return out


def lincomb(out: torch.Tensor, terms, coefs) -> torch.Tensor:
    _lib.require_device()
    n = len(terms)
    assert 1 <= n <= 6 and len(coefs) == n
    for t in terms:
        assert t.dtype == torch.float32 and t.is_contiguous() and t.numel() == out.numel()
    assert out.dtype == torch.float32 and out.is_contiguous()
    tarr = (C.c_void_p * n)(*[t.data_ptr() for t in terms])
    carr = (C.c_float * n)(*[float(c) for c in coefs])
    check(lib.sdmi_lincomb(ptr(out), tarr, carr, n, out.numel(), stream_ptr()), "sdmi_lincomb")
    return out


def mask_blend(x: torch.Tensor, init: torch.Tensor, mask: torch.Tensor, nmask: torch.Tensor) -> torch.Tensor:
    _lib.require_device()
    m = mask.to(x.device, torch.float32).expand_as(x).contiguous()
    nm = nmask.to(x.device, torch.float32).expand_as(x).contiguous()
    init = init.to(x.device, torch.float32).expand_as(x).contiguous()
    check(lib.sdmi_mask_blend(ptr(x), ptr(init), ptr(m), ptr(nm), x.numel(), stream_ptr()), "sdmi_mask_blend")
    return x


def latent_resize(x: torch.Tensor, size, mode: str = "bilinear", antialias: bool = False) -> torch.Tensor:
    _lib.require_device()
    x = x.float().contiguous()
    b, c, hi, wi = x.shape
    ho, wo = int(size[0]), int(size[1])
    out = torch.empty((b, c, ho, wo), dtype=torch.float32, device=x.device)
    code = {"nearest": 0, "nearest-exact": 1, "bilinear": 2, "bicubic": 3}[mode]
    if antialias:
# ... 15 lines not shown
```

Baseline: 21.72.

## Fuse split-K reduction of 3x3 convs into following GroupNorm kernel

The split-K reduction pass of a 3x3 conv GEMM is deferred, and when the next op is an eligible GroupNorm on that output, the reduction (alpha, bias, rowbias, residual) is done inside the small fused GroupNorm kernel. When the pre-norm tensor is not needed later, it is not written back at all. This removes one kernel launch and a round trip of the conv output through memory. The cost is deferred-state bookkeeping: every other op entry point must flush the pending reduce first, which is easy to get wrong. The forced split-K selection rule is also relaxed to allow smaller K per split.

```diff
diff --git a/include/sdmi.h b/include/sdmi.h
--- a/include/sdmi.h
+++ b/include/sdmi.h
@@ -80,6 +80,10 @@
                    void* workspace_f32, int64_t workspace_bytes, void* stream);
 int64_t sdmi_groupnorm_workspace_bytes(int B, int HW, int groups);
 
+int sdmi_conv_gemm_groupnorm(const sdmi_conv_desc* d, const void* x1, int c1, const void* gamma_f32, const void* beta_f32, int groups,
+                             float eps, int silu, void* y_f16, void* workspace, int64_t workspace_bytes, int* fused, void* stream);
+int64_t sdmi_conv_gemm_groupnorm_workspace_bytes(int M, int N, int B, int HW, int groups);
+
 int sdmi_layernorm(const void* x, const void* gamma_f32, const void* beta_f32, void* out_f16,
                    int64_t rows, int C, float eps, void* stream);
 
diff --git a/stable-diffusion-webui_amd/_lib.py b/stable-diffusion-webui_amd/_lib.py
--- a/stable-diffusion-webui_amd/_lib.py
+++ b/stable-diffusion-webui_amd/_lib.py
@@ -86,6 +86,8 @@
     "sdmi_groupnorm": (_i, [_vp, _vp, _i, _i, _vp, _vp, _vp, _i, _i, _i, _f, _i, _vp, _i64, _vp]),
     "sdmi_groupnorm_workspace_bytes": (_i64, [_i, _i, _i]),
     "sdmi_layernorm": (_i, [_vp, _vp, _vp, _vp, _i64, _i, _f, _vp]),
+    "sdmi_conv_gemm_groupnorm": (_i, [C.POINTER(ConvDesc), _vp, _i, _vp, _vp, _i, _f, _i, _vp, _vp, _i64, C.POINTER(C.c_int), _vp]),
+    "sdmi_conv_gemm_groupnorm_workspace_bytes": (_i64, [_i, _i, _i, _i, _i]),
     "sdmi_rowchain_ff_pack_bytes": (_i64, [_i, _i]),
     "sdmi_rowchain_ff_pack": (_i, [_vp, _vp, _vp, _vp, _i, _i, _vp]),
     "sdmi_rowchain_ff": (_i, [_vp, _vp, _vp, _vp, _vp, _vp, _i64, _i, _i, _f, _vp]),
diff --git a/stable-diffusion-webui_amd/csrc/capi.cpp b/stable-diffusion-webui_amd/csrc/capi.cpp
--- a/stable-diffusion-webui_amd/csrc/capi.cpp
+++ b/stable-diffusion-webui_amd/csrc/capi.cpp
@@ -154,8 +154,18 @@
 
 int64_t sdmi_conv_splitk_workspace_bytes(int M, int N, int K, int batch) { return (int64_t)gemm_splitk_ws_bytes(M, N, K, batch); }
 
+static SplitKDesc g_api_pend{};
+static hipStream_t g_api_pend_stream = nullptr;
+static int api_flush() {
+    if (g_api_pend.splitk <= 1) return 0;
+    const SplitKDesc d = g_api_pend;
+    g_api_pend.splitk = 0;
+    return launch_splitk_reduce(d, g_api_pend_stream);
+}
+
 int sdmi_conv_gemm(const sdmi_conv_desc* d, void* stream) {
     API_GUARD_BEGIN
+    if (api_flush()) return 1;
     GemmP p;
     if (desc_to_p(d, &p)) return 1;
     const char* env = getenv("SDMI_NO_GLDS");
@@ -201,6 +211,7 @@
 int sdmi_groupnorm(const void* x0, const void* x1, int c0, int c1, const void* gamma, const void* beta, void* out, int B, int HW,
                    int groups, float eps, int silu, void* ws, int64_t ws_bytes, void* stream) {
     API_GUARD_BEGIN
+    if (api_flush()) return 1;
     SDMI_REQUIRE(ws && ws_bytes >= groupnorm_ws_bytes(B, HW, groups), "groupnorm workspace too small");
     return launch_groupnorm((const half_t*)x0, (const half_t*)x1, c0, x1 ? c1 : 0, (const float*)gamma, (const float*)beta,
                             (half_t*)out, B, HW, groups, eps, silu != 0, (float*)ws, (hipStream_t)stream);
@@ -209,7 +220,58 @@
 
 int sdmi_layernorm(const void* x, const void* gamma, const void* beta, void* out, int64_t rows, int C, float eps, void* stream) {
     API_GUARD_BEGIN
+    if (api_flush()) return 1;
     return launch_layernorm((const half_t*)x, (const float*)gamma, (const float*)beta, (half_t*)out, rows, C, eps, (hipStream_t)stream);
+    API_GUARD_END
+}
+
+static size_t cgg_slab_bytes(int64_t M, int64_t N) { return (size_t)8 * M * N * sizeof(float); }
+static size_t cgg_pre_bytes(int64_t M, int64_t N) { return ((size_t)M * N * sizeof(half_t) + 255) / 256 * 256; }
+int64_t sdmi_conv_gemm_groupnorm_workspace_bytes(int M, int N, int B, int HW, int groups) {
+    return (int64_t)(cgg_slab_bytes(M, N) + cgg_pre_bytes(M, N)) + groupnorm_ws_bytes(B, HW, groups);
+}
+
+int sdmi_conv_gemm_groupnorm(const sdmi_conv_desc* d, const void* x1, int c1, const void* gamma, const void* beta, int groups, float eps,
+                             int silu, void* y, void* workspace, int64_t workspace_bytes, int* fused, void* stream) {
+    API_GUARD_BEGIN
+    if (api_flush()) return 1;
+    GemmP p;
+    if (desc_to_p(d, &p)) return 1;
+    hipStream_t s = (hipStream_t)stream;
+    SDMI_REQUIRE(fused != nullptr, "sdmi_conv_gemm_groupnorm: fused must point to an int");
+    *fused = 0;
+    SDMI_REQUIRE(d->batch <= 1 && p.flags == 0, "sdmi_conv_gemm_groupnorm: one batch element, plain fp16 row-major epilogue");
+    SDMI_REQUIRE(d->out == nullptr || d->ldo == d->N, "sdmi_conv_gemm_groupnorm: a kept pre-norm tensor has dense rows (ldo == N)");
+    const int B = d->B, HW = d->Ho * d->Wo;
+    if (x1 == nullptr) c1 = 0;
+    SDMI_REQUIRE(workspace && workspace_bytes >= sdmi_conv_gemm_groupnorm_workspace_bytes(p.M, p.N, B, HW, groups),
+                 "sdmi_conv_gemm_groupnorm: workspace too small");
+    p.splitk_ws = (float*)workspace;
+    half_t* pre = (half_t*)((char*)workspace + cgg_slab_bytes(p.M, p.N));
+    float* gn_ws = (float*)((char*)pre + cgg_pre_bytes(p.M, p.N));
+    const bool keep = d->out != nullptr;
+    if (!keep) { p.out = pre; p.ldo = p.N; }
+    const char* env = getenv("SDMI_NO_GLDS");
+    SplitKDesc pd{};
+    if (launch_gemm(p, 1, d->force_generic == 1, !(env && env[0] == '1') && d->force_generic != 2, s, nullptr, nullptr,
+                    g_gn_splitk_fuse ? &pd : nullptr))
+        return 1;
+    if (gamma == nullptr) {
+        SDMI_REQUIRE(keep, "sdmi_conv_gemm_groupnorm without a norm needs d->out");
+        if (pd.splitk > 1) { g_api_pend = pd; g_api_pend_stream = s; *fused = 1; }
+        return 0;
+    }
+    SDMI_REQUIRE(beta && y, "null argument");
+    if (pd.splitk > 1) {
+        if (groupnorm_splitk_eligible(pd, (const half_t*)x1, c1, B, HW, groups)) {
+            *fused = 1;
+            return launch_groupnorm_splitk(pd, keep, (const half_t*)x1, c1, (const float*)gamma, (const float*)beta, (half_t*)y, B, HW, groups, eps,
+                                           silu != 0, s);
+        }
+        if (launch_splitk_reduce(pd, s)) return 1;
+    }
+    return launch_groupnorm((const half_t*)p.out, (const half_t*)x1, p.N, c1, (const float*)gamma, (const float*)beta, (half_t*)y, B, HW, groups,
+                            eps, silu != 0, gn_ws, s);
     API_GUARD_END
 }
 
@@ -582,6 +644,7 @@
     else if (n == "small_linear_lds") g_small_linear_lds = value;
     else if (n == "gn_fuse") g_gn_fuse = value;
     else if (n == "gn_small") g_gn_small = value;
+    else if (n == "gn_splitk_fuse") g_gn_splitk_fuse = value < 0 ? 1 : value;
     else if (n == "ep_wide") g_ep_wide = value;
     else if (n == "attn_kvt") g_attn_kvt = value;
     else if (n == "attn_occ") g_attn_occ = value;
diff --git a/stable-diffusion-webui_amd/csrc/common.h b/stable-diffusion-webui_amd/csrc/common.h
--- a/stable-diffusion-webui_amd/csrc/common.h
+++ b/stable-diffusion-webui_amd/csrc/common.h
@@ -119,8 +119,24 @@
 }
 __host__ __device__ inline const half_t* gemm_resid_lo(const GemmP& p) { return (p.flags & EP_HILO) ? reinterpret_cast<const half_t*>(p.ln_s) : nullptr; }
 
+struct SplitKDesc {
+    const float* ws;
+    int splitk, M, N, rows_per_batch;
+    float alpha;
+    const float* bias;
+    float bias_scale;
+    const float* rowbias;
+    int ldrb;
+    const half_t* resid;
+    int ldr;
+    half_t* out;
+    int ldo;
+};
+
 int launch_gemm(const GemmP& p, int batch, bool force_generic, bool use_glds, hipStream_t s, int* stats_nchunk_out = nullptr,
-                int* lnp_np_out = nullptr);
+                int* lnp_np_out = nullptr,
+                SplitKDesc* defer = nullptr);
+int launch_splitk_reduce(const SplitKDesc& d, hipStream_t s);
 extern int g_ep_wide;
 extern int g_small_linear_lds;
 extern int g_gn_small;
@@ -176,6 +192,10 @@
                      half_t* out, int B, int HW, int groups, float eps, bool silu, float* ws, hipStream_t s, int pre_nchunk = 0,
                      const half_t* x0_lo = nullptr, const half_t* x1_lo = nullptr);
 int64_t groupnorm_ws_bytes(int B, int HW, int groups);
+extern int g_gn_splitk_fuse;
+bool groupnorm_splitk_eligible(const SplitKDesc& d, const half_t* x1, int c1, int B, int HW, int groups);
+int launch_groupnorm_splitk(const SplitKDesc& d, bool keep, const half_t* x1, int c1, const float* gamma, const float* beta, half_t* out, int B,
+                            int HW, int groups, float eps, bool silu, hipStream_t s);
 int launch_layernorm(const half_t* x, const float* gamma, const float* beta, half_t* out, int64_t rows, int C,
                      float eps, hipStream_t s, const half_t* x_lo = nullptr);
 int launch_ln_rowstats(const half_t* x, float* stats, int64_t rows, int C, float eps, hipStream_t s);
diff --git a/stable-diffusion-webui_amd/csrc/engine.cpp b/stable-diffusion-webui_amd/csrc/engine.cpp
--- a/stable-diffusion-webui_amd/csrc/engine.cpp
+++ b/stable-diffusion-webui_amd/csrc/engine.cpp
@@ -55,6 +55,14 @@
     const half_t* lnp_tensor = nullptr;
     float* lnp_ws = nullptr;
     int lnp_np = 0;
+    bool gn_splitk = false;
+    SplitKDesc pend{};
+    int flush() {
+        if (pend.splitk <= 1) return 0;
+        const SplitKDesc d = pend;
+        pend.splitk = 0;
+        return launch_splitk_reduce(d, s);
+    }
 };
 
 #define TRY(x)                  \
@@ -365,6 +373,7 @@
     if (want_lnp) lnp_ws = r.F((size_t)a.B * a.Ho * a.Wo * (W.n_pad / 64) * 2);
     r.lnp_tensor = nullptr; r.lnp_np = 0;
     if (r.dry) return 0;
+    TRY(r.flush());
     GemmP p{};
     p.splitk_ws = splitk_ws;
     p.lnp_out = lnp_ws;
@@ -391,7 +400,7 @@
     int nchunk = 0;
     if (stats_ws) { p.stats_out = stats_ws; p.stats_cpg = a.stats_C / 32; }
     int lnp_np = 0;
-    TRY(launch_gemm(p, a.batch, r.e->force_generic, r.e->use_glds, r.s, &nchunk, &lnp_np));
+    TRY(launch_gemm(p, a.batch, r.e->force_generic, r.e->use_glds, r.s, &nchunk, &lnp_np, (r.gn_splitk && W.taps == 9) ? &r.pend : nullptr));
     if (nchunk > 0) { r.st_tensor = (const half_t*)a.out; r.st_ws = stats_ws; r.st_nchunk = nchunk; }
     if (lnp_np > 0) { r.lnp_tensor = (const half_t*)a.out; r.lnp_ws = lnp_ws; r.lnp_np = lnp_np; }
     return 0;
@@ -410,16 +419,25 @@
 }
 
 static int run_gn(Run& r, const NormW& n, const half_t* x0, const half_t* x1, int c0, int c1, int B, int HW, float eps,
-                  bool silu, half_t* out, const half_t* x0_lo = nullptr, const half_t* x1_lo = nullptr) {
+                  bool silu, half_t* out, const half_t* x0_lo = nullptr, const half_t* x1_lo = nullptr, bool x0_dead = false) {
     float* ws = r.F(groupnorm_ws_bytes(B, HW, 32) / sizeof(float));
     if (r.dry) return 0;
     SDMI_REQUIRE(n.c == c0 + c1, "GroupNorm channel mismatch");
+    if (r.pend.splitk > 1) {
+        if (r.pend.out == x0 && r.pend.N == c0 && !x0_lo && groupnorm_splitk_eligible(r.pend, x1, c1, B, HW, 32)) {
+            const SplitKDesc d = r.pend;
+            r.pend.splitk = 0;
+            return launch_groupnorm_splitk(d, !x0_dead, x1, c1, n.g, n.b, out, B, HW, 32, eps, silu, r.s);
+        }
+        TRY(r.flush());
+    }
     if (x1 == nullptr && r.st_nchunk > 0 && r.st_tensor == x0)
         return launch_groupnorm(x0, nullptr, c0, 0, n.g, n.b, out, B, HW, 32, eps, silu, r.st_ws, r.s, r.st_nchunk, x0_lo, nullptr);
     return launch_groupnorm(x0, x1, c0, c1, n.g, n.b, out, B, HW, 32, eps, silu, ws, r.s, 0, x0_lo, x1_lo);
 }
 static int run_ln(Run& r, const NormW& n, const half_t* x, int64_t rows, half_t* out, const half_t* x_lo = nullptr) {
     if (r.dry) return 0;
+    TRY(r.flush());
     return launch_layernorm(x, n.g, n.b, out, rows, n.c, 1e-5f, r.s, x_lo);
 }
 
@@ -427,6 +445,7 @@
 static int run_ln_stats(Run& r, const NormW& n, const half_t* x, int64_t rows, LnStats* out) {
     float* own = r.F((size_t)rows * 2);
     if (r.dry) { out->ptr = own; out->np = 0; return 0; }
+    TRY(r.flush());
     if (r.lnp_tensor == x && r.lnp_np > 0) { out->ptr = r.lnp_ws; out->np = r.lnp_np; return 0; }
     out->ptr = own; out->np = 0;
     return launch_ln_rowstats(x, own, rows, n.c, 1e-5f, r.s);
@@ -453,6 +472,7 @@
     }
     r.st_tensor = nullptr; r.st_nchunk = 0;
     if (r.dry) return 0;
+    TRY(r.flush());
     GemmP p{};
     p.splitk_ws = splitk_ws;
     p.a0 = x; p.w = W.w_ln; p.bias = W.c_ln; p.out = out;
@@ -470,6 +490,7 @@
 static int run_vt_ln(Run& r, const ConvW& Wv, const NormW& n, const half_t* x, const LnStats& stats, int B, int tokens, int tokens_pad,
                      half_t* vt) {
     if (r.dry) return 0;
+    TRY(r.flush());
     TRY(ensure_ln_fold(r.e, Wv, n, r.s));
     GemmP p{};
     const int C = Wv.n_pad, K = Wv.cin_pad;
@@ -513,7 +534,7 @@
         TRY(run_conv(r, w.c1, c));
     }
     half_t* t2 = r.H(M * w.cout);
-    TRY(run_gn(r, w.n2, h1, nullptr, w.cout, 0, B, HW, eps, true, t2, acc ? r.lo(h1, M * w.cout) : nullptr));
+    TRY(run_gn(r, w.n2, h1, nullptr, w.cout, 0, B, HW, eps, true, t2, acc ? r.lo(h1, M * w.cout) : nullptr, nullptr, true));
     const half_t* resid = x0;
     const half_t* resid_lo = x0_lo;
     if (w.has_skip) {
@@ -549,6 +570,7 @@
 static int run_attn(Run& r, const half_t* q, const half_t* k, const half_t* vt, half_t* out, int B, int H, int N, int M,
                     int D, int ldq, int ldk, int vt_ld, int ldo) {
     if (r.dry) return 0;
+    TRY(r.flush());
     AttnP p{};
     p.q = q; p.k = k; p.vt = vt; p.out = out;
     p.B = B; p.H = H; p.N = N; p.M = M; p.D = D;
@@ -560,6 +582,7 @@
 static int run_vt(Run& r, const ConvW& Wv, const half_t* x, int ldx, int B, int tokens, int tokens_pad, half_t* vt,
                   bool bias_row, const int* gate = nullptr) {
     if (r.dry) return 0;
+    TRY(r.flush());
     GemmP p{};
     const int C = Wv.n_pad, K = Wv.cin_pad;
     if (g_vt_mode == 1 && tokens == tokens_pad && tokens % 4 == 0 && ldx == K && gate == nullptr) {
@@ -710,6 +733,7 @@
         r.lnp_want = fold && e->ln_fold >= 2;
         TRY(run_linear(r, b.o1, a1, (int)M1, cur, x1, C, 1.f, false, r.lo(cur, MC), r.lo(x1, MC)));
         if (B1 != B) {
+            if (!r.dry) TRY(r.flush());
             if (!r.dry) SDMI_CHECK_HIP(hipMemcpyAsync(x1 + M1 * C, x1, M1 * C * sizeof(half_t), hipMemcpyDeviceToDevice, r.s));
             if (!r.dry && acc) SDMI_CHECK_HIP(hipMemcpyAsync(x1 + MC + M1 * C, x1 + MC, M1 * C * sizeof(half_t), hipMemcpyDeviceToDevice, r.s));
             B1 = B; M1 = M;
@@ -732,6 +756,7 @@
         }
         half_t* a2 = r.H(M * C);
         if (!r.dry) {
+            TRY(r.flush());
             SDMI_REQUIRE(e->ctx_valid && e->ctx_B == (r.Btot ? r.Btot : B), "context not set for this batch size");
             AttnP p{};
             p.q = q2; p.out = a2;
@@ -903,6 +928,9 @@
     const sdmi_unet_config& c = u.cfg;
     const int mc = c.model_channels, ted = mc * 4;
     r.ar->reset();
+    r.gn_splitk = g_gn_splitk_fuse != 0 && !e->trace && !e->force_generic && e->use_glds && !r.acc() && e->n_streams <= 1 &&
+                  (r.Btot == 0 || r.Btot == Bn) && !r.reuse();
+    r.pend.splitk = 0;
     float* sinus = r.F((size_t)Bn * mc);
     float* e1 = r.F((size_t)Bn * ted);
     float* emb = r.F((size_t)Bn * ted);
@@ -940,6 +968,7 @@
     bool shared = pairs;
     auto dup = [&](const Act& a) -> int {
         const size_t n = (size_t)Bh * a.H * a.W * a.C;
+        if (!r.dry) TRY(r.flush());
         if (!r.dry) SDMI_CHECK_HIP(hipMemcpyAsync((half_t*)a.p + n, a.p, n * sizeof(half_t), hipMemcpyDeviceToDevice, r.s));
         if (!r.dry && r.acc())
             SDMI_CHECK_HIP(hipMemcpyAsync((half_t*)a.p + 3 * n, a.p + 2 * n, n * sizeof(half_t), hipMemcpyDeviceToDevice, r.s));
@@ -1034,6 +1063,7 @@
         const size_t n = (size_t)Bn * a.H * a.W * a.C;
         half_t* o = r.S(n);
         if (!r.dry) {
+            TRY(r.flush());
             const size_t full = (size_t)(r.Btot ? r.Btot : Bn) * a.C * a.H * a.W;
             SDMI_REQUIRE((size_t)e->control_numel[idx] == full, "control tensor " + std::to_string(idx) + " does not have the shape of the activation it is added to");
             const size_t elt = io_dtype == SDMI_F16 ? 2 : 4;
@@ -1070,6 +1100,7 @@
         a.out = eps; a.flags = EP_NCHW; a.n_real = c.out_channels;
         TRY(run_conv(r, u.out_conv, a));
     }
+    if (!r.dry) TRY(r.flush());
     if (!r.dry) TRY(launch_copy_out(eps, out, io_dtype, (int64_t)Bn * c.out_channels * cur.H * cur.W, r.s));
     return 0;
 }
diff --git a/stable-diffusion-webui_amd/csrc/gemm.hip b/stable-diffusion-webui_amd/csrc/gemm.hip
--- a/stable-diffusion-webui_amd/csrc/gemm.hip
+++ b/stable-diffusion-webui_amd/csrc/gemm.hip
@@ -2152,7 +2152,9 @@
 static int pick_cfg(const GemmP& p, int batch, int* split_out, bool allow_split) {
     *split_out = 1;
     if (g_force_gemm_cfg >= 0 && cfg_valid(g_force_gemm_cfg, p)) {
-        if (allow_split && g_force_gemm_split > 1 && p.K / 64 / g_force_gemm_split >= 4) *split_out = std::min(g_force_gemm_split, 8);
+        int fs = std::min(g_force_gemm_split, 8);
+        while (fs > 1 && p.K / 64 / fs < 2) --fs;
+        if (allow_split && fs > 1) *split_out = fs;
         return g_force_gemm_cfg;
     }
     if (g_force_gemm_split == 1) allow_split = false;
@@ -2188,12 +2190,37 @@
     return (size_t)8 * M * N * batch * sizeof(float);
 }
 
-int launch_gemm(const GemmP& p_in, int batch, bool force_generic, bool use_glds, hipStream_t s, int* stats_nchunk_out, int* lnp_np_out) {
+static void splitk_reduce_grid(const GemmP& p, int batch, hipStream_t s) {
+    const long total = (long)p.M * (p.N / 4);
+    const dim3 grid((unsigned)std::min<long>((total + 255) / 256, 8192));
+    if (p.flags & EP_LNFOLD) hipLaunchKernelGGL(splitk_reduce_kernel<true>, grid, dim3(256), 0, s, p, batch);
+    else hipLaunchKernelGGL(splitk_reduce_kernel<false>, grid, dim3(256), 0, s, p, batch);
+}
+
+int launch_splitk_reduce(const SplitKDesc& d, hipStream_t s) {
+    SDMI_REQUIRE(d.splitk > 1 && d.ws && d.out, "launch_splitk_reduce: no pending split-K launch");
+    GemmP p{};
+    p.splitk_ws = const_cast<float*>(d.ws); p.splitk = d.splitk;
+    p.M = d.M; p.N = d.N; p.rows_per_batch = d.rows_per_batch;
+    p.alpha = d.alpha; p.bias = d.bias; p.bias_scale = d.bias_scale;
+    p.rowbias = d.rowbias; p.ldrb = d.ldrb; p.resid = d.resid; p.ldr = d.ldr;
+    p.out = d.out; p.ldo = d.ldo;
+    char pname[64];
+    snprintf(pname, sizeof pname, "splitk_reduce M%d N%d", d.M, d.N);
+    ProfScope ps(pname, 0.0, ((double)d.splitk * 4.0 + 2.0) * d.M * (double)d.N, s);
+    splitk_reduce_grid(p, 1, s);
+    SDMI_CHECK_HIP(hipGetLastError());
+    return 0;
+}
+
+int launch_gemm(const GemmP& p_in, int batch, bool force_generic, bool use_glds, hipStream_t s, int* stats_nchunk_out, int* lnp_np_out,
+                SplitKDesc* defer) {
     GemmP p = p_in;
     p.stats_nchunk = 0;
     p.lnp_np = 0;
     if (stats_nchunk_out) *stats_nchunk_out = 0;
     if (lnp_np_out) *lnp_np_out = 0;
+    if (defer) defer->splitk = 0;
     p.flags |= g_gemm_dbgflags;
     if (p.n_valid <= 0 || p.n_valid > p.N) p.n_valid = p.N;
     if (p.bias_scale == 0.f) p.bias_scale = 1.f;
@@ -2294,18 +2321,19 @@
                 ((p.flags & EP_LNFOLD) ? " ln" : "") + (batch > 1 ? " x" + std::to_string(batch) : "");
     }
     ProfScope ps(pname.c_str(), pf_flops, pf_bytes, s);
+    const bool deferred = defer && split > 1 && batch == 1 && !p.gate && !(p.flags & ~EP_NARROW);
+    if (deferred)
+        *defer = SplitKDesc{p.splitk_ws, p.splitk, p.M, p.N, p.rows_per_batch, p.alpha, p.bias, p.bias_scale, p.rowbias, p.ldrb,
+                            p.resid, p.ldr, (half_t*)p.out, p.ldo};
     struct Reduce {
         const GemmP& p; int batch; hipStream_t s; bool on;
         int run() const {
             if (!on) return 0;
-            const long total = (long)p.M * (p.N / 4);
-            const dim3 grid((unsigned)std::min<long>((total + 255) / 256, 8192));
-            if (p.flags & EP_LNFOLD) hipLaunchKernelGGL(splitk_reduce_kernel<true>, grid, dim3(256), 0, s, p, batch);
-            else hipLaunchKernelGGL(splitk_reduce_kernel<false>, grid, dim3(256), 0, s, p, batch);
+            splitk_reduce_grid(p, batch, s);
             SDMI_CHECK_HIP(hipGetLastError());
             return 0;
         }
-    } reduce{p, batch, s, split > 1};
+    } reduce{p, batch, s, split > 1 && !deferred};
 #define SDMI_CASE(ID, BM, BN, WR, WC, BK)                                                                       \
     case ID:                                                                                                    \
         if (use_glds ? launch_cfg<BM, BN, WR, WC, BK, true>(p, batch, s) : launch_cfg<BM, BN, WR, WC, BK, false>(p, batch, s)) \
diff --git a/stable-diffusion-webui_amd/csrc/norm.hip b/stable-diffusion-webui_amd/csrc/norm.hip
--- a/stable-diffusion-webui_amd/csrc/norm.hip
+++ b/stable-diffusion-webui_amd/csrc/norm.hip
@@ -3,6 +3,7 @@
 #include <algorithm>
 #include <cstdio>
 #include <cstdlib>
+#include <type_traits>
 
 namespace sdmi {
 
@@ -206,13 +207,23 @@
     }
 }
 
-template <int NVT, bool HILO = false>
+template <int NVT, bool HILO = false, bool SK = false>
 __global__ __launch_bounds__(256) void gn_fused_small_kernel(const half_t* x0, const half_t* x1, int c0, int c1, int HW, int groups,
                                                              const float* gamma, const float* beta, half_t* out, float eps, int silu,
-                                                             const half_t* l0 = nullptr, const half_t* l1 = nullptr) {
+                                                             const half_t* l0 = nullptr, const half_t* l1 = nullptr,
+                                                             std::conditional_t<SK, SplitKDesc, int> sk = {}, int xcd_group = 0) {
+    static_assert(!(SK && HILO), "the split-K source is a plain fp16 stream");
     __shared__ float red[2][4];
     const int C = c0 + c1, cpg = C / groups, VW = cpg / 8;
-    const int g = blockIdx.x, b = blockIdx.y, tid = threadIdx.x;
+    int g = blockIdx.x, b = blockIdx.y;
+    const int tid = threadIdx.x;
+    if constexpr (SK) {
+        if (xcd_group) {
+            const int total = (int)(gridDim.x * gridDim.y), L = (int)(blockIdx.y * gridDim.x + blockIdx.x);
+            const int logical = (L & 7) * (total >> 3) + (L >> 3);
+            b = logical / (int)gridDim.x; g = logical - b * (int)gridDim.x;
+        }
+    }
     const int cbase = g * cpg;
     const half_t* x0b = x0 + (long)b * HW * c0;
     const half_t* x1b = x1 ? x1 + (long)b * HW * c1 : nullptr;
@@ -233,7 +244,46 @@
         cch[k] = c;
         const half_t* src = c < c0 ? x0b + (long)pp * c0 + c : x1b + (long)pp * c1 + (c - c0);
         h8 z = {0, 0, 0, 0, 0, 0, 0, 0};
-        v[k] = ok ? *reinterpret_cast<const h8*>(src) : z;
+        if constexpr (SK) {
+            if (c < c0) {
+                v[k] = z;
+                if (ok) {
+                    const long m = (long)b * HW + pp, slab = (long)sk.M * sk.N;
+                    const float* w = sk.ws + m * sk.N + c;
+                    f4 a0 = {0.f, 0.f, 0.f, 0.f}, a1 = {0.f, 0.f, 0.f, 0.f};
+#pragma unroll 4
+                    for (int sl = 0; sl < sk.splitk; ++sl) {
+                        a0 += *reinterpret_cast<const f4*>(w + sl * slab);
+                        a1 += *reinterpret_cast<const f4*>(w + sl * slab + 4);
+                    }
+#pragma unroll
+                    for (int e = 0; e < 4; ++e) { a0[e] *= sk.alpha; a1[e] *= sk.alpha; }
+                    if (sk.bias) {
+                        const f4 b0 = *reinterpret_cast<const f4*>(sk.bias + c), b1 = *reinterpret_cast<const f4*>(sk.bias + c + 4);
+#pragma unroll
+                        for (int e = 0; e < 4; ++e) { a0[e] = fmaf(b0[e], sk.bias_scale, a0[e]); a1[e] = fmaf(b1[e], sk.bias_scale, a1[e]); }
+                    }
+                    if (sk.rowbias) {
+                        a0 += *reinterpret_cast<const f4*>(sk.rowbias + (long)b * sk.ldrb + c);
+                        a1 += *reinterpret_cast<const f4*>(sk.rowbias + (long)b * sk.ldrb + c + 4);
+                    }
+                    if (sk.resid) {
+                        const h8 rr = *reinterpret_cast<const h8*>(sk.resid + m * sk.ldr + c);
+#pragma unroll
+                        for (int e = 0; e < 4; ++e) { a0[e] += (float)rr[e]; a1[e] += (float)rr[e + 4]; }
+                    }
+                    h8 hv;
+#pragma unroll
+                    for (int e = 0; e < 4; ++e) { hv[e] = (half_t)a0[e]; hv[e + 4] = (half_t)a1[e]; }
+                    if (sk.out) *reinterpret_cast<h8*>(sk.out + m * sk.ldo + c) = hv;
+                    v[k] = hv;
+                }
+            } else {
+                v[k] = ok ? *reinterpret_cast<const h8*>(src) : z;
+            }
+        } else {
+            v[k] = ok ? *reinterpret_cast<const h8*>(src) : z;
+        }
         if constexpr (HILO) {
             const half_t* srcl = c < c0 ? l0b + (long)pp * c0 + c : l1b + (long)pp * c1 + (c - c0);
             vl[k] = ok ? *reinterpret_cast<const h8*>(srcl) : z;
@@ -344,6 +394,46 @@
 }
 
 
+int g_gn_splitk_fuse = [] { const char* e = getenv("SDMI_GN_SPLITK_FUSE"); return e ? atoi(e) : 1; }();
+
+bool groupnorm_splitk_eligible(const SplitKDesc& d, const half_t* x1, int c1, int B, int HW, int groups) {
+    if (!g_gn_splitk_fuse || !g_gn_small || d.splitk <= 1 || !d.ws || !d.out) return false;
+    if (x1 == nullptr) c1 = 0;
+    const int c0 = d.N, C = c0 + c1;
+    if ((long)B * HW != d.M || d.rows_per_batch != HW || d.ldo != d.N || groups <= 0 || groups > 32) return false;
+    if (C % 8 || c0 % 8 || C > GN_MAX_C || C % groups || gn_bands(HW, C) != 1) return false;
+    const int cpg = C / groups;
+    if (cpg % 8 || (long)HW * (cpg / 8) > 12 * 256) return false;
+    auto al16 = [](const void* q) { return ((uintptr_t)q & 15) == 0; };
+    if (!al16(d.ws) || !al16(d.out) || !al16(d.bias) || !al16(d.rowbias) || !al16(d.resid) || !al16(x1)) return false;
+    if ((d.rowbias && d.ldrb % 4) || (d.resid && d.ldr % 8)) return false;
+    return true;
+}
+
+int launch_groupnorm_splitk(const SplitKDesc& d_in, bool keep, const half_t* x1, int c1, const float* gamma, const float* beta, half_t* out, int B,
+                            int HW, int groups, float eps, bool silu, hipStream_t s) {
+    SDMI_REQUIRE(groupnorm_splitk_eligible(d_in, x1, c1, B, HW, groups), "launch_groupnorm_splitk: not eligible (the caller runs the reduce pass and launch_groupnorm)");
+    SplitKDesc d = d_in;
+    const half_t* x0 = d.out;
+    if (!keep) d.out = nullptr;
+    if (x1 == nullptr) c1 = 0;
+    const int c0 = d.N, C = c0 + c1;
+    const long nv = (long)HW * (C / groups / 8);
+    char pname[64];
+    snprintf(pname, sizeof pname, "splitk_reduce_groupnorm B%d HW%d C%d", B, HW, C);
+    ProfScope ps(pname, 0.0, (double)B * HW * ((double)c0 * (4.0 * d.splitk + (keep ? 2.0 : 0.0)) + (double)c1 * 2.0 + (double)C * 2.0), s);
+    const dim3 grid(groups, B);
+    const int xcd_group = (g_gn_splitk_fuse == 1 && (groups * B) % 8 == 0) ? 1 : 0;
+    if (nv <= 4 * 256)
+        hipLaunchKernelGGL((gn_fused_small_kernel<4, false, true>), grid, dim3(256), 0, s, x0, x1, c0, c1, HW, groups, gamma, beta, out, eps, silu ? 1 : 0,
+                           (const half_t*)nullptr, (const half_t*)nullptr, d, xcd_group);
+    else
+        hipLaunchKernelGGL((gn_fused_small_kernel<12, false, true>), grid, dim3(256), 0, s, x0, x1, c0, c1, HW, groups, gamma, beta, out, eps, silu ? 1 : 0,
+                           (const half_t*)nullptr, (const half_t*)nullptr, d, xcd_group);
+    SDMI_CHECK_HIP(hipGetLastError());
+    return 0;
+}
+
 int launch_groupnorm(const half_t* x0, const half_t* x1, int c0, int c1, const float* gamma, const float* beta,
                      half_t* out, int B, int HW, int groups, float eps, bool silu, float* ws, hipStream_t s, int pre_nchunk,
                      const half_t* x0_lo, const half_t* x1_lo) {
@@ -365,7 +455,7 @@
             snprintf(pname, sizeof pname, "groupnorm_silu_fused B%d HW%d C%d", B, HW, C);
             ProfScope ps(pname, 0.0, (hilo ? 3.0 : 2.0) * B * (double)HW * C * 2.0, s);
             const dim3 grid(groups, B);
-#define SDMI_GNS(NVT, HL) hipLaunchKernelGGL((gn_fused_small_kernel<NVT, HL>), grid, dim3(256), 0, s, x0, x1, c0, c1, HW, groups, gamma, beta, out, eps, silu ? 1 : 0, x0_lo, x1_lo)
+#define SDMI_GNS(NVT, HL) hipLaunchKernelGGL((gn_fused_small_kernel<NVT, HL>), grid, dim3(256), 0, s, x0, x1, c0, c1, HW, groups, gamma, beta, out, eps, silu ? 1 : 0, x0_lo, x1_lo, 0, 0)
             if (hilo) { if (nv <= 2 * 256) SDMI_GNS(2, true); else SDMI_GNS(6, true); }
             else if (nv <= 4 * 256) SDMI_GNS(4, false);
             else SDMI_GNS(12, false);
diff --git a/stable-diffusion-webui_amd/ops.py b/stable-diffusion-webui_amd/ops.py
--- a/stable-diffusion-webui_amd/ops.py
+++ b/stable-diffusion-webui_amd/ops.py
@@ -136,6 +136,42 @@
     return out
 
 
+def conv_gemm_groupnorm(a0: torch.Tensor, w_packed: torch.Tensor, gamma, beta, *, x1: Optional[torch.Tensor] = None, bias=None, rowbias=None,
+                        resid=None, taps: int = 9, keep: bool = False, groups: int = 32, eps: float = 1e-5, silu: bool = True,
+                        pre: Optional[torch.Tensor] = None):
+    _lib.require_device()
+    assert a0.dtype == torch.float16 and a0.is_contiguous()
+    b, hi, wi, c0 = a0.shape
+    n = w_packed.shape[0]
+    c1 = x1.shape[3] if x1 is not None else 0
+    d = ConvDesc()
+    d.a0, d.w = a0.data_ptr(), w_packed.data_ptr()
+    d.bias = bias.data_ptr() if bias is not None else None
+    d.rowbias = rowbias.data_ptr() if rowbias is not None else None
+    d.resid = resid.data_ptr() if resid is not None else None
+    d.c0, d.lda0 = c0, c0
+    d.B, d.Hi, d.Wi, d.Ho, d.Wo = b, hi, wi, hi, wi
+    d.taps, d.stride, d.pad, d.up = taps, 1, 1 if taps == 9 else 0, 0
+    d.N, d.ldo = n, n
+    d.ldr = resid.shape[-1] if resid is not None else 0
+    d.alpha, d.batch = 1.0, 1
+    if keep and pre is None:
+        pre = torch.empty((b, hi, wi, n), dtype=torch.float16, device=a0.device)
+    assert pre is None or (keep and pre.dtype == torch.float16 and pre.is_contiguous() and tuple(pre.shape) == (b, hi, wi, n))
+    d.out = pre.data_ptr() if keep else None
+    y = torch.empty((b, hi, wi, n + c1), dtype=torch.float16, device=a0.device) if gamma is not None else None
+    wsb = lib.sdmi_conv_gemm_groupnorm_workspace_bytes(b * hi * wi, n, b, hi * wi, groups)
+    ws = torch.empty(wsb, dtype=torch.uint8, device=a0.device)
+    fused = C.c_int(-1)
+    gm = gamma.float().contiguous() if gamma is not None else None
+    bt = beta.float().contiguous() if gamma is not None else None
+    check(lib.sdmi_conv_gemm_groupnorm(C.byref(d), ptr(x1), c1, ptr(gm), ptr(bt), groups, float(eps), 1 if silu else 0, ptr(y), ptr(ws), wsb,
+                                       C.byref(fused), stream_ptr()), "sdmi_conv_gemm_groupnorm")
+    if gamma is None:
+        conv_gemm_groupnorm.pending_ws = ws
+    return y, pre, fused.value
+
+
 def groupnorm(x0: torch.Tensor, gamma: torch.Tensor, beta: torch.Tensor, *, x1: Optional[torch.Tensor] = None,
               groups: int = 32, eps: float = 1e-5, silu: bool = True) -> torch.Tensor:
     _lib.require_device()
```

Result: no change. 21.79, median of 5 (+0.3%).
